# jac99/Egonn

Measured on AMD Instinct MI355X. Metric: LiDAR scans/sec (descriptor extraction), 50k-pt clouds @ 0.1m voxel, higher is better.
Workload: dtype f32

## Files before the change

egonn_amd/_lib.py:

```python
from __future__ import annotations

import ctypes as C
import os
from typing import List, Optional, Sequence

import numpy as np
import torch

_HERE = os.path.dirname(os.path.abspath(__file__))
LIB_PATH = os.path.join(_HERE, "lib", "libegonn_hip.so")

QUANT_CARTESIAN, QUANT_POLAR = 0, 1
FLAG_DISABLE_GLOBAL, FLAG_DISABLE_LOCAL, FLAG_IGNORE_KP_REGRESSOR, FLAG_BF16 = 1, 2, 4, 8
FLAG_POOL_SPOC, FLAG_POOL_MAC = 16, 32
MINKFPN_SPLIT_TOPDOWN = 1
MINKFPN_BLOCKS = {'BasicBlock': 0, 'ECABasicBlock': 1}
MINKFPN_POOLING = {None: 0, 'GeM': 1, 'MAC': 2, 'SPoC': 3}

_P = C.c_void_p
_SIGS = [
    ("egonn_ctx_create", C.c_int, [C.POINTER(_P), C.c_int, C.c_int]),
    ("egonn_ctx_destroy", None, [_P]),
    ("egonn_last_error", C.c_char_p, []),
    ("egonn_debug_set_naive_conv", C.c_int, [_P, C.c_int]),
    ("egonn_debug_set_ksplit", C.c_int, [_P, C.c_int, C.c_int, C.c_int, C.c_int, C.c_int]),
    ("egonn_debug_set_resident", C.c_int, [_P, C.c_int, C.c_int]),
    ("egonn_debug_keep_level_features", C.c_int, [_P, C.c_int]),
    ("egonn_debug_set_trace", C.c_int, [_P]),
    ("egonn_prepare_maps", C.c_int, [_P, C.c_int, _P]),
    ("egonn_debug_rowgroup_tables", C.c_int, [_P, C.c_int, C.c_int, _P, _P, C.c_int64, C.POINTER(C.c_int64), _P]),
    ("egonn_debug_rowgroup_perm", C.c_int, [_P, C.c_int, C.c_int, _P, C.c_int64, C.POINTER(C.c_int64), _P]),
    ("egonn_debug_radix_sort_scratch_bytes", C.c_int64, [C.c_int64, C.c_int]),
    ("egonn_debug_radix_sort", C.c_int, [_P, _P, _P, _P, C.c_int64, C.c_int, _P, _P, C.c_int, C.c_int, C.c_int,
                                         C.POINTER(C.c_int32), _P, C.c_int64, _P]),
    ("egonn_debug_dense_group3", C.c_int, [_P, _P, _P, _P, _P, _P, _P]),
    ("egonn_debug_global_tail_scratch_bytes", C.c_int64, [C.c_int64]),
    ("egonn_debug_global_tail", C.c_int, [_P, _P, C.c_int, C.c_int64, _P, _P, _P, _P, _P, _P, C.c_int, C.c_int, _P, _P, _P, C.c_int64, _P]),
    ("egonn_voxelize", C.c_int, [_P, _P, C.POINTER(C.c_int64), C.c_int, C.c_int, C.POINTER(C.c_float), _P]),
    ("egonn_ctx_reserve", C.c_int, [_P, C.c_int64, C.c_int, C.POINTER(C.c_int64)]),
    ("egonn_voxelize_device", C.c_int, [_P, _P, C.c_int64, _P, C.c_int, C.c_int, C.POINTER(C.c_float), _P]),
    ("egonn_plan_status", C.c_int, [_P, _P]),
    ("egonn_ctx_set_exact_fp32", C.c_int, [_P, C.c_int]),
    ("egonn_ctx_set_operand_autoscale", C.c_int, [_P, C.c_int]),
    ("egonn_level_capacity", C.c_int, [_P, C.c_int, C.POINTER(C.c_int64)]),
    ("egonn_graph_begin", C.c_int, [_P]),
    ("egonn_graph_end", C.c_int, [_P, C.POINTER(_P)]),
    ("egonn_graph_launch", C.c_int, [_P, _P]),
    ("egonn_graph_destroy", None, [_P]),
    ("egonn_coords_set", C.c_int, [_P, _P, C.c_int64, C.c_int, _P]),
    ("egonn_level_count", C.c_int, [_P, C.c_int, C.POINTER(C.c_int64)]),
    ("egonn_level_batch_offsets", C.c_int, [_P, C.c_int, C.POINTER(C.c_int64)]),
    ("egonn_level_coords", C.c_int, [_P, C.c_int, _P, _P]),
    ("egonn_input_index", C.c_int, [_P, _P, _P]),
    ("egonn_conv", C.c_int, [_P, C.c_int, C.c_int, C.c_int, _P, C.c_int, _P, C.c_int, _P, _P, C.c_int, _P, _P]),
    ("egonn_conv_transpose", C.c_int, [_P, C.c_int, _P, C.c_int, _P, C.c_int, _P, _P]),
    ("egonn_sparse_conv", C.c_int, [_P, C.c_int, C.c_int, _P, C.c_int, _P, C.c_int, C.c_int, _P, _P, C.c_int, _P, _P, _P]),
    ("egonn_map_groups", C.c_int, [_P, C.c_int, C.c_int, C.POINTER(C.c_int64), C.POINTER(C.c_int64), _P]),
    ("egonn_global_avg_pool", C.c_int, [_P, C.c_int, _P, C.c_int, _P, _P]),
    ("egonn_bn_fold", C.c_int, [_P, _P, _P, _P, C.c_float, C.c_int, _P, _P, _P]),
    ("egonn_block_tail", C.c_int, [_P, C.c_int, _P, _P, C.c_int, _P, C.c_int, _P, _P]),
    ("egonn_gem", C.c_int, [_P, C.c_int, _P, C.c_int, _P, _P, _P]),
    ("egonn_global_max_pool", C.c_int, [_P, C.c_int, _P, C.c_int, _P, _P]),
    ("egonn_netvlad", C.c_int, [_P, C.c_int, _P, C.c_int, _P, _P, _P, _P, _P, _P, _P, _P, _P, _P, C.c_int, C.c_int, _P, _P]),
    ("egonn_netvlad_train_forward", C.c_int, [_P, C.c_int, _P, C.c_int, C.c_int, _P, _P, _P, _P, C.c_float, C.c_float, _P, _P,
                                              _P, C.c_int, _P, _P, _P, _P, _P, _P, _P]),
    ("egonn_netvlad_train_backward", C.c_int, [_P, C.c_int, _P, C.c_int, C.c_int, _P, _P, _P, _P, C.c_int, _P, _P, _P, _P, _P,
                                               _P, _P, _P, _P, _P, _P, _P]),
    ("egonn_global_max_pool_argmax", C.c_int, [_P, C.c_int, _P, C.c_int, _P, _P, _P]),
    ("egonn_global_max_pool_backward", C.c_int, [_P, C.c_int, _P, _P, C.c_int, _P, _P]),
    ("egonn_sigmoid_gate", C.c_int, [_P, _P, _P, C.c_int64, _P, _P, _P, _P]),
    ("egonn_add", C.c_int, [_P, _P, C.c_int64, _P, _P]),
    ("egonn_gather_input", C.c_int, [_P, _P, C.c_int, _P, _P]),
    ("egonn_model_create", C.c_int, [C.POINTER(_P)]),
    ("egonn_model_destroy", None, [_P]),
    ("egonn_model_set_tensor", C.c_int, [_P, C.c_char_p, _P, C.c_int, C.POINTER(C.c_int64)]),
    ("egonn_model_finalize", C.c_int, [_P, _P]),
    ("egonn_forward", C.c_int, [_P, _P, _P, C.c_int, C.POINTER(C.c_float), C.c_int, _P, _P, _P, _P, _P]),
    ("egonn_forward_level_features", C.c_int, [_P, C.c_int, _P, C.c_int, _P]),
    ("egonn_minkfpn_finalize", C.c_int, [_P, C.c_int, C.POINTER(C.c_int), C.POINTER(C.c_int), C.c_int, C.c_int, C.c_int, C.c_int, _P]),
    ("egonn_minkfpn_out_level", C.c_int, [C.c_int, C.c_int, C.POINTER(C.c_int)]),
    ("egonn_minkfpn_forward", C.c_int, [_P, _P, C.c_int, _P, _P, _P]),
    ("egonn_topdown_step", C.c_int, [_P, C.c_int, _P, _P, _P, _P, C.c_int, C.c_int, _P, _P]),
    ("egonn_select_keypoints", C.c_int, [_P, _P, _P, _P, C.c_int, _P, _P, _P, _P, _P]),
    ("egonn_topk_rows", C.c_int, [_P, _P, C.c_int, C.c_int, _P, _P, _P]),
    ("egonn_triplet_loss_scratch_floats", C.c_int64, [C.c_int]),
    ("egonn_triplet_loss", C.c_int, [_P, C.c_int, C.c_int, _P, _P, C.c_float, _P, _P, _P, _P, _P]),
    ("egonn_nn_search", C.c_int, [_P, C.c_int64, _P, _P, C.c_int64, _P, _P, _P]),
    ("egonn_matrix_min", C.c_int, [_P, C.c_int64, C.c_int64, _P, _P, _P, _P, _P]),
    ("egonn_softmax_cross_entropy", C.c_int, [_P, C.c_int64, C.c_int64, _P, _P, _P, _P, _P]),
    ("egonn_local_loss_scratch_bytes", C.c_int64, [C.c_int, C.c_int64, C.c_int64, C.c_int]),
    ("egonn_local_loss", C.c_int, [C.c_int, C.c_int64, C.c_int64, C.c_int64, C.c_int64, C.c_int] + [_P] * 13 +
                                  [C.POINTER(C.c_float)] + [_P] * 9 + [C.c_int64, _P]),
    ("egonn_dense", C.c_int, [_P, C.c_int64, C.c_int, _P, C.c_int, _P, C.c_int, C.c_int, _P, _P]),
    ("egonn_dense_pack_fragments", C.c_int, [_P, C.c_int, C.c_int, C.c_int, _P, _P]),
    ("egonn_dense_pack_fragments_host", C.c_int, [_P, C.c_int, C.c_int, C.c_int, _P]),
    ("egonn_debug_dense", C.c_int, [_P, C.c_int, C.c_int64, _P, C.c_int, C.c_int, _P, C.c_int, _P, _P, _P, _P, C.c_int, _P, C.c_int,
                                    _P, _P, C.c_int, _P, C.c_int, C.c_int, _P]),
    ("egonn_debug_dense_route", C.c_int, [C.c_int64, C.c_int, C.c_int, C.c_int, C.c_int, C.POINTER(C.c_int32)]),
    ("egonn_debug_sconv_choice", C.c_int, [C.POINTER(C.c_int32), C.c_int64, C.POINTER(C.c_int32)]),
    ("egonn_dense_backward_weight", C.c_int, [_P, C.c_int, _P, C.c_int, C.c_int64, _P, _P, C.c_int64, _P]),
    ("egonn_conv_backward_weight", C.c_int, [_P, C.c_int, C.c_int, C.c_int, C.c_int, _P, C.c_int, _P, C.c_int, _P, _P,
                                             C.c_int64, _P]),
    ("egonn_col_stats", C.c_int, [C.c_int, _P, _P, _P, _P, C.c_int64, C.c_int, _P, _P, C.c_int64, _P]),
    ("egonn_bn_train_finalize", C.c_int, [_P, _P, C.c_double, C.c_int, _P, _P, C.c_float, C.c_float, _P, _P, _P, _P]),
    ("egonn_bn_backward_finalize", C.c_int, [_P, _P, C.c_double, C.c_int, _P, _P, _P, _P, _P]),
    ("egonn_affine_act", C.c_int, [_P, _P, _P, C.c_int64, C.c_int, C.c_int, _P, _P]),
    ("egonn_affine3", C.c_int, [_P, _P, _P, _P, _P, _P, C.c_int64, C.c_int, _P, _P]),
    ("egonn_relu_backward", C.c_int, [_P, _P, C.c_int64, C.c_int, _P, _P]),
    ("egonn_contrastive_loss_scratch_floats", C.c_int64, [C.c_int]),
    ("egonn_contrastive_loss", C.c_int, [_P, C.c_int, C.c_int, _P, _P, C.c_float, C.c_float, _P, _P, _P, _P, _P]),
    ("egonn_se_gate", C.c_int, [_P, _P, _P, _P, _P, C.c_int, C.c_int, C.c_int, _P, _P, _P]),
    ("egonn_se_gate_backward", C.c_int, [_P, _P, _P, _P, _P, _P, C.c_int, C.c_int, C.c_int, _P, _P, _P, _P, _P, _P]),
    ("egonn_eca_gate", C.c_int, [_P, _P, C.c_int, C.c_int, C.c_int, _P, _P]),
    ("egonn_eca_gate_backward", C.c_int, [_P, _P, _P, _P, C.c_int, C.c_int, C.c_int, _P, _P, _P]),
    ("egonn_act_backward", C.c_int, [C.c_int, _P, _P, C.c_int64, C.c_int, _P, _P]),
    ("egonn_l2_normalize", C.c_int, [_P, _P, C.c_int64, C.c_int, _P, _P]),
    ("egonn_gate_residual", C.c_int, [_P, C.c_int, _P, _P, _P, C.c_int, C.c_int, _P, _P]),
    ("egonn_gate_residual_backward", C.c_int, [_P, C.c_int, _P, _P, _P, C.c_int, _P, _P, _P]),
    ("egonn_segment_sums", C.c_int, [_P, C.c_int, C.c_int, _P, _P, _P, _P, C.c_int, _P, _P, C.c_int64, _P]),
    ("egonn_segment_broadcast", C.c_int, [_P, C.c_int, _P, C.c_int, C.c_int, _P, _P]),
    ("egonn_gem_backward", C.c_int, [_P, C.c_int, _P, _P, _P, C.c_int, _P, _P]),
    ("egonn_filter_points_scratch_ints", C.c_int64, [C.c_int64]),
    ("egonn_filter_points", C.c_int, [_P, C.c_int64, C.c_int, _P, C.c_int, C.c_int, C.c_int, C.c_float, _P, _P, _P,
                                      C.c_int64, _P]),
    ("egonn_knn", C.c_int, [_P, C.c_int64, _P, C.c_int64, C.c_int, C.c_int, _P, _P, _P, C.c_int64, _P]),
    ("egonn_recall_counts", C.c_int, [_P, _P, _P, C.c_int64, C.c_int, C.c_int, _P, C.c_int, _P, _P]),
    ("egonn_registration_scratch_bytes", C.c_int64, [C.c_int, C.c_int, C.c_int]),
    ("egonn_match_mutual_scratch_bytes", C.c_int64, [C.c_int, C.c_int]),
    ("egonn_match_mutual", C.c_int, [_P, _P, _P, _P, C.c_int, C.c_int, C.c_int, _P, _P, _P, C.c_int64, _P]),
    ("egonn_ransac_pairs", C.c_int, [_P, _P, _P, _P, _P, _P, _P, C.c_int, C.c_int, C.c_int, C.c_uint64, C.c_double, _P,
                                     C.c_int64, _P, _P, _P]),
    ("egonn_registration_finish", C.c_int, [_P, _P, _P, _P, _P, _P, _P, C.c_int, C.c_int, C.c_int, C.c_uint64, C.c_double, _P,
                                            C.c_int64, _P, C.c_double, _P, _P, _P, _P, _P, _P, _P, _P, _P, _P, _P, _P]),
    ("egonn_voxel_downsample_scratch_bytes", C.c_int64, [C.c_int64, C.c_int]),
    ("egonn_voxel_downsample", C.c_int, [_P, C.c_int64, _P, C.c_int, C.c_double, C.POINTER(C.c_float), _P, _P, _P, _P, _P,
                                         C.c_int64, _P]),
    ("egonn_icp_scratch_bytes", C.c_int64, [C.c_int64, C.c_int64, C.c_int]),
    ("egonn_icp_pairs", C.c_int, [_P, C.c_int64, _P, _P, C.c_int64, _P, C.c_int, _P, C.c_double, C.c_int, C.c_double, C.c_double,
                                  _P, _P, _P, _P, _P, _P, _P, _P, _P, C.c_int64, _P]),
    ("egonn_estimate_normals_scratch_bytes", C.c_int64, [C.c_int64, C.c_int]),
    ("egonn_estimate_normals", C.c_int, [_P, C.c_int64, _P, C.c_int, C.c_int, _P, _P, _P, _P, _P, C.c_int64, _P]),
    ("egonn_icp_plane_scratch_bytes", C.c_int64, [C.c_int64, C.c_int64, C.c_int]),
    ("egonn_icp_plane_pairs", C.c_int, [_P, C.c_int64, _P, _P, C.c_int64, _P, _P, C.c_int, _P, C.c_double, C.c_int, C.c_double,
                                        C.c_double, _P, _P, _P, _P, _P, _P, _P, _P, _P, C.c_int64, _P]),
    ("egonn_augment_scratch_bytes", C.c_int64, [C.c_int64, C.c_int]),
    ("egonn_augment_points", C.c_int, [_P, C.c_int64, _P, C.c_int, _P, _P, _P, _P, _P, _P, _P, _P, _P, C.c_int64, _P]),
    ("egonn_scan_context", C.c_int, [_P, C.c_int64, _P, C.c_int, C.c_int, C.c_int, C.c_double, C.c_double, _P, _P, _P]),
    ("egonn_scan_context_ringkey", C.c_int, [_P, C.c_int64, C.c_int, C.c_int, _P, _P]),
    ("egonn_scan_context_distance", C.c_int, [_P, C.c_int64, _P, C.c_int64, C.c_int, C.c_int, _P, C.c_int, _P, _P, _P]),
    ("egonn_scan_context_rerank", C.c_int, [_P, _P, _P, C.c_int64, C.c_int, _P, _P, _P, _P]),
    ("egonn_radius_count", C.c_int, [_P, C.c_int64, _P, C.c_int64, C.POINTER(C.c_double), C.c_int, C.c_int, _P, _P]),
    ("egonn_radius_fill", C.c_int, [_P, C.c_int64, _P, C.c_int64, C.c_double, C.c_int, _P, _P, C.c_int64, _P, _P]),
    ("egonn_pair_masks", C.c_int, [_P, C.c_int, _P, _P, C.c_int64, _P, _P, C.c_int64, C.c_int64, _P, _P, _P, _P]),
    ("egonn_relative_poses", C.c_int, [_P, C.c_int64, _P, _P, C.c_int64, C.c_int, _P, _P, _P]),
    ("egonn_gather_clouds", C.c_int, [_P, C.c_int64, _P, C.c_int64, _P, C.c_int, _P, C.c_int64, _P, _P, _P]),
    ("egonn_match_candidates_scratch_bytes", C.c_int64, [C.c_int, C.c_int, C.c_int]),
    ("egonn_match_candidates", C.c_int, [_P, _P, _P, _P, _P, C.c_int, C.c_int, C.c_int, C.c_int, C.c_int, _P, _P, _P, _P,
                                         C.c_int64, _P]),
    ("egonn_gather_candidates", C.c_int, [_P, _P, _P, _P, _P, _P, C.c_int, C.c_int, C.c_int, C.c_int, _P, _P, _P, _P, _P, _P]),
    ("egonn_pick_candidates", C.c_int, [_P, C.c_int, C.c_int, C.c_int, _P, _P, _P, _P, _P, _P, _P, _P, C.c_int] + [_P] * 12),
    ("egonn_profile_enable", C.c_int, [_P, C.c_int, C.c_char_p]),
    ("egonn_profile_fetch", C.c_int, [_P, C.c_int, C.POINTER(C.c_int), C.c_char_p, C.POINTER(C.c_float),
                                      C.POINTER(C.c_double), C.POINTER(C.c_double), _P]),
]
EXPORTED_SYMBOLS = [s[0] for s in _SIGS]

_lib = None


def load() -> C.CDLL:
    global _lib
    if _lib is not None:
        return _lib
    if not os.path.exists(LIB_PATH):
        raise RuntimeError(
            f"egonn_amd: HIP library not found at {LIB_PATH}. Build it with "
            f"`python -c 'import __graft_entry__ as g; g.build()'` (hipcc --offload-arch=gfx950). "
            f"There is no CPU fallback.")
    lib = C.CDLL(LIB_PATH)
    for name, res, args in _SIGS:
        fn = getattr(lib, name)
        fn.restype = res
        fn.argtypes = args
    _lib = lib
    return lib


def _err(lib) -> str:
    msg = lib.egonn_last_error()
    return msg.decode() if msg else "unknown error"


class EgonnError(RuntimeError):

    def __init__(self, msg: str, code: int):
        super().__init__(msg)
        self.code = int(code)


class CapacityError(EgonnError):
    """status 5: the batch did not fit the capacities of egonn_ctx_reserve (the exact-size eager path still works)"""


class Fp16RangeError(EgonnError):
    """status 6: a kernel on the fp16-split pipe (fp32 sparse convolution or local heads) met an operand fp16 cannot hold
    (|x| >= 65520) or a non-finite input: the batch's outputs are invalid; Context.set_exact_fp32(True) and run it again
    (on the same plan: every forward clears this flag)"""


def check(rc: int):
    if rc != 0:
        cls = CapacityError if rc == 5 else (Fp16RangeError if rc == 6 else EgonnError)
        raise cls(f"libegonn_hip: {_err(load())} (code {rc})", rc)


def _stream() -> int:
    return torch.cuda.current_stream().cuda_stream


def _ptr(t: Optional[torch.Tensor]) -> Optional[int]:
    return None if t is None else t.data_ptr()


def call(device: torch.device, fn, *args):
    idx = device.index
    if idx is None or torch.cuda.current_device() == idx:
        rc = fn(*args, _stream())
    else:
        with torch.cuda.device(device):
            rc = fn(*args, _stream())
    if rc != 0:
        check(rc)


def _dev_f32(t: torch.Tensor, device) -> torch.Tensor:
    return t.to(device=device, dtype=torch.float32).contiguous()


def as_dev(x, dev, dtype) -> torch.Tensor:
    return torch.as_tensor(x).to(device=dev, dtype=dtype).contiguous()


def scratch(nbytes: int, dev) -> torch.Tensor:
    return torch.empty((max(int(nbytes), 8) + 7) // 8, dtype=torch.int64, device=dev)


def check_cloud(name, x):
    shape = tuple(getattr(x, "shape", ()))
    if len(shape) != 2 or shape[1] != 3:
        raise ValueError(f"{name}: expected (n, 3) points, got shape {shape}")


def check_offsets(name, off) -> int:
    shape = tuple(getattr(off, "shape", (len(off),) if hasattr(off, "__len__") else ()))
    if len(shape) != 1 or shape[0] < 2:
        raise ValueError(f"{name}: offsets must be a 1-D sequence of n_clouds + 1 entries, got shape {shape}")
    return shape[0] - 1


def concat_clouds(clouds, dev):
    ts = [torch.as_tensor(c) for c in clouds]
    for c in ts:
        check_cloud("cloud", c)
    off = [0]
    for c in ts:
        off.append(off[-1] + c.shape[0])
    pts = torch.cat([c.to(device=dev, dtype=torch.float32) for c in ts]) if ts else torch.zeros((0, 3), device=dev)
    return pts, torch.tensor(off, dtype=torch.int64, device=dev)


def dense_pack_fragments(weight, out_in: bool):
    lib = load()
    co, ci = (weight.shape if out_in else weight.shape[::-1])
    if isinstance(weight, np.ndarray):
        w = np.ascontiguousarray(weight, dtype=np.float32)
        out = np.empty(ci * co, dtype=np.float32)
        check(lib.egonn_dense_pack_fragments_host(w.ctypes.data, int(bool(out_in)), int(ci), int(co), out.ctypes.data))
        return out
    w = weight.contiguous()
    out = torch.empty(ci * co, dtype=torch.float32, device=w.device)
    call(w.device, lib.egonn_dense_pack_fragments, w.data_ptr(), int(bool(out_in)), int(ci), int(co), out.data_ptr())
    return out


def debug_dense(x, weight, out_in: bool, out, form: int, n_dev=None, packed=None, bias=None, scale=None, shift=None, act: int = 0,
                residual=None, gate=None, boff=None):
    lib = load()
    cap, cin = x.shape
    cout = out.shape[1]
    B = 0 if boff is None else boff.numel() - 1
    bf = lambda t: int(t is not None and t.dtype == torch.bfloat16)
    call(x.device, lib.egonn_debug_dense, x.data_ptr(), bf(x), int(cap), _ptr(n_dev), int(cin), int(cout), weight.data_ptr(),
         int(bool(out_in)), _ptr(packed), _ptr(bias), _ptr(scale), _ptr(shift), int(act), _ptr(residual), bf(residual), _ptr(gate),
         _ptr(boff), B, out.data_ptr(), bf(out), int(form))
    return out


CONV_PRODUCT, CONV_PLAIN, CONV_RING, CONV_COOP, CONV_RING2, CONV_DMA, CONV_DMA3, CONV_TRACED = 0, 1, 2, 4, 8, 16, 32, 128
CONV_SPLIT = 1000
CFG_NW4, CFG_NW8, CFG_RESIDENT = 142, 182, 183
CFG_PARTS, CFG_TRACED = 400, 9000
SCONV_ROUTES = ("plain", "split", "tail_split", "wg", "dma", "rg")
SCONV_CHOICE_FIELDS = ("route", "kernel", "NW", "NSW", "KW", "KS", "GATED", "TRACE", "resident", "KSP", "D", "G", "SPLIT", "PIPE",
                       "gx", "gy", "gz", "block", "lds", "kparts")


def debug_sconv_choice(kind: int, level: int, cin: int, cout: int, cap_groups: int, *, code: int = 0, bf16: int = 0, gated: int = 0,
                       split_io: int = 0, residual: int = 0, split_max_level: int = 5, autoscale: int = 0, resident_mask: int = -1,
                       max_workgroups: int = 0, kparts: int = -1, kw: int = -1, col_parts: int = -1) -> dict:
    arg = (C.c_int32 * 16)(int(code), kind, level, cin, cout, int(bf16), int(gated), split_io, int(residual), split_max_level,
                           int(autoscale), resident_mask, max_workgroups, kparts, kw, col_parts)
    out = (C.c_int32 * 20)()
    check(load().egonn_debug_sconv_choice(arg, int(cap_groups), out))
    d = dict(zip(SCONV_CHOICE_FIELDS, out))
    d["route"], d["kernel"] = SCONV_ROUTES[d["route"]], SCONV_ROUTES[d["kernel"]]
    return d


DENSE_ROUTES = ("none", "stream", "lds", "small", "tile", "plain")


def debug_dense_route(rows: int, cin: int, cout: int, form: int = -1, gate_scans: int = 0):
    out = (C.c_int32 * 5)()
    check(load().egonn_debug_dense_route(int(rows), int(cin), int(cout), int(form), int(gate_scans), out))
    return (DENSE_ROUTES[out[0]],) + tuple(out[1:])


def debug_radix_sort(keys_in, vals_in, keys_out, vals_out, n: int, nbits: int, n_dev=None, seg_offsets=None, idx_bits: int = 0,
                     either_pair: bool = False, scratch_buf=None, scratch_bytes: Optional[int] = None) -> int:
    lib = load()
    B = 0 if seg_offsets is None else seg_offsets.numel() - 1
    need = lib.egonn_debug_radix_sort_scratch_bytes(int(n), B)
    if scratch_buf is None:
        scratch_buf = scratch(need, keys_in.device)
    pair = C.c_int32(-1)
    call(keys_in.device, lib.egonn_debug_radix_sort, keys_in.data_ptr(), vals_in.data_ptr(), keys_out.data_ptr(),
         vals_out.data_ptr(), int(n), int(nbits), _ptr(n_dev), _ptr(seg_offsets), B, int(idx_bits), int(bool(either_pair)),
         C.byref(pair), scratch_buf.data_ptr(), need if scratch_bytes is None else int(scratch_bytes))
    return pair.value


def debug_dense_group3(xs, capacities, counts, ws, packed: bool):
    lib = load()
    dev = xs[0].device
    arr = lambda ptrs: (C.c_void_p * 3)(*ptrs)
    nds = [torch.tensor([int(c)], dtype=torch.int32, device=dev) for c in counts]
    pks = [dense_pack_fragments(w, False) for w in ws] if packed else [None] * 3
    bufs = [torch.full((max(int(c), 1), 128), -12345.0, dtype=torch.float32, device=dev) for c in capacities]
    call(dev, lib.egonn_debug_dense_group3, arr([x.data_ptr() for x in xs]), (C.c_int64 * 3)(*[int(c) for c in capacities]),
         arr([n.data_ptr() for n in nds]), arr([w.data_ptr() for w in ws]), arr([_ptr(p) for p in pks]),
         arr([b.data_ptr() for b in bufs]))
    return [b[:int(c)] for b, c in zip(bufs, capacities)]


GLOBAL_TAIL_POOLING = {"GeM": 1, "MAC": 2, "SPoC": 3}


def debug_global_tail(g5, row_offsets, n_dev, w0, b0, w1, b1, p, pooling: str, form: int):
    lib = load()
    B = row_offsets.numel() - 1
    cap = g5.shape[0]
    need = lib.egonn_debug_global_tail_scratch_bytes(int(cap))
    buf = scratch(need, g5.device)
    partial = torch.empty((B, 32, 256), dtype=torch.float32, device=g5.device)
    out = torch.empty((B, 256), dtype=torch.float32, device=g5.device)
    call(g5.device, lib.egonn_debug_global_tail, g5.data_ptr(), row_offsets.data_ptr(), B, int(cap), n_dev.data_ptr(), w0.data_ptr(),
         b0.data_ptr(), w1.data_ptr(), b1.data_ptr(), _ptr(p), GLOBAL_TAIL_POOLING[pooling], int(form), partial.data_ptr(),
         out.data_ptr(), buf.data_ptr(), need)
    return partial, out


def require_gpu() -> torch.device:
    if not torch.cuda.is_available():
        raise RuntimeError("egonn_amd: no HIP device visible (torch.cuda.is_available() is False); "
                           "the descriptor-extraction path runs on MI355X only — there is no CPU fallback.")
    return torch.device("cuda", torch.cuda.current_device())


class Context:

    def __init__(self, device: Optional[torch.device] = None, coord_bits: int = 16):
        self.lib = load()
        self.device = torch.device(device) if device is not None else require_gpu()
        if self.device.type != "cuda":
            raise RuntimeError(f"egonn_amd: device {self.device} is not a HIP device; there is no CPU fallback.")
        if self.device.index is None:
            self.device = torch.device("cuda", torch.cuda.current_device())
        h = _P()
        check(self.lib.egonn_ctx_create(C.byref(h), self.device.index, coord_bits))
        self.h = h
        self.batch_size = 0
        self._keep = []

    def __del__(self):
        try:
            if getattr(self, "h", None):
                self.lib.egonn_ctx_destroy(self.h)
                self.h = None
        except Exception:
            pass

    def voxelize(self, points: torch.Tensor, scan_offsets: Sequence[int], mode: int, step: Sequence[float]):
        assert points.is_cuda and points.dtype == torch.float32 and points.is_contiguous()
        assert points.dim() == 2 and points.shape[1] == 3
        B = len(scan_offsets) - 1
        off = (C.c_int64 * (B + 1))(*[int(o) for o in scan_offsets])
        st = (C.c_float * 3)(*([float(s) for s in step] + [0.0, 0.0])[:3])
        self._call(self.lib.egonn_voxelize, self.h, points.data_ptr(), off, B, mode, st)
        self.batch_size = B

    def reserve(self, max_points: int, batch_size: int, level_capacity: Optional[Sequence[int]] = None):
        caps = None
        if level_capacity is not None:
            assert len(level_capacity) == 8
            caps = (C.c_int64 * 8)(*[int(v) for v in level_capacity])
        with torch.cuda.device(self.device):
            check(self.lib.egonn_ctx_reserve(self.h, int(max_points), int(batch_size), caps))
        self.batch_size = int(batch_size)

    def voxelize_device(self, points: torch.Tensor, scan_offsets: torch.Tensor, batch_size: int, mode: int,
                        step: Sequence[float]):
        assert points.is_cuda and points.dtype == torch.float32 and points.is_contiguous() and points.shape[1] == 3
        assert scan_offsets.is_cuda and scan_offsets.dtype == torch.int64 and scan_offsets.numel() == batch_size + 1
        st = (C.c_float * 3)(*([float(s) for s in step] + [0.0, 0.0])[:3])
        self._call(self.lib.egonn_voxelize_device, self.h, points.data_ptr(), points.shape[0], scan_offsets.data_ptr(),
                   int(batch_size), mode, st)
        self.batch_size = int(batch_size)

    def plan_status(self):
        self._call(self.lib.egonn_plan_status, self.h)

    def level_capacity(self, level: int) -> int:
        n = C.c_int64()
        check(self.lib.egonn_level_capacity(self.h, level, C.byref(n)))
        return n.value

    def coords_set(self, coords: torch.Tensor, batch_size: int):
        assert coords.is_cuda and coords.dtype == torch.int32 and coords.is_contiguous()
        assert coords.dim() == 2 and coords.shape[1] == 4
        self._call(self.lib.egonn_coords_set, self.h, coords.data_ptr(), coords.shape[0], int(batch_size))
        self.batch_size = int(batch_size)

    def level_count(self, level: int) -> int:
        n = C.c_int64()
        check(self.lib.egonn_level_count(self.h, level, C.byref(n)))
        return n.value

    def level_batch_offsets(self, level: int) -> List[int]:
        off = (C.c_int64 * (self.batch_size + 1))()
        check(self.lib.egonn_level_batch_offsets(self.h, level, off))
        return list(off)

    def level_coords(self, level: int) -> torch.Tensor:
        out = torch.empty((self.level_count(level), 4), dtype=torch.int32, device=self.device)
        self._call(self.lib.egonn_level_coords, self.h, level, out.data_ptr())
        return out

    def input_index(self) -> torch.Tensor:
        out = torch.empty((self.level_count(0),), dtype=torch.int64, device=self.device)
        self._call(self.lib.egonn_input_index, self.h, out.data_ptr())
        return out

    def conv(self, level_in: int, level_out: int, kernel_size: int, x: torch.Tensor, kernel: torch.Tensor,
             scale: Optional[torch.Tensor] = None, shift: Optional[torch.Tensor] = None, relu: bool = False):
        kernel = _dev_f32(kernel, self.device)
        cin, cout = kernel.shape[-2], kernel.shape[-1]
        if x is None:
            assert kernel_size == 5 and cin == 1, "x=None (all-ones features) is the k=5 input layer only"
        else:
            x = _dev_f32(x, self.device)
            assert x.shape == (self.level_count(level_in), cin), (x.shape, self.level_count(level_in), cin)
        out = torch.empty((self.level_count(level_out), cout), dtype=torch.float32, device=self.device)
        sc = None if scale is None else _dev_f32(scale, self.device)
        sh = None if shift is None else _dev_f32(shift, self.device)
        self._call(self.lib.egonn_conv, self.h, level_in, level_out, kernel_size, _ptr(x), cin, kernel.data_ptr(), cout,
                   _ptr(sc), _ptr(sh), int(relu), out.data_ptr())
        return out

    def conv_transpose(self, level_in: int, x: torch.Tensor, kernel: torch.Tensor):
        x = _dev_f32(x, self.device)
        kernel = _dev_f32(kernel, self.device)
        cin, cout = kernel.shape[-2], kernel.shape[-1]
        assert x.shape == (self.level_count(level_in), cin)
        out = torch.empty((self.level_count(level_in - 1), cout), dtype=torch.float32, device=self.device)
        self._call(self.lib.egonn_conv_transpose, self.h, level_in, x.data_ptr(), cin, kernel.data_ptr(), cout, out.data_ptr())
        return out

    def sparse_conv(self, map_kind: int, level_out: int, x: torch.Tensor, kernel: torch.Tensor, scale=None, shift=None,
                    relu: bool = False, group_sums: bool = False):
        assert x.is_cuda and x.dtype in (torch.float32, torch.bfloat16) and x.is_contiguous()
        kernel = _dev_f32(kernel, self.device)
        cin, cout = kernel.shape[-2], kernel.shape[-1]
        assert x.shape[1] == cin
        out = torch.empty((self.level_count(level_out), cout), dtype=x.dtype, device=self.device)
        sc = None if scale is None else _dev_f32(scale, self.device)
        sh = None if shift is None else _dev_f32(shift, self.device)
        sums = None
        if group_sums:
            sums = torch.zeros((self.map_groups(map_kind, level_out)[0], cout), dtype=torch.float32, device=self.device)
        self._call(self.lib.egonn_sparse_conv, self.h, map_kind, level_out, x.data_ptr(), cin, kernel.data_ptr(), cout,
                   int(x.dtype == torch.bfloat16), _ptr(sc), _ptr(sh), int(relu), out.data_ptr(), _ptr(sums))
        return (out, sums) if group_sums else out

    def prepare_maps(self, with_level0_transpose: bool = False):
        self._call(self.lib.egonn_prepare_maps, self.h, int(with_level0_transpose))

    def map_groups(self, map_kind: int, level_out: int):
        n = C.c_int64()
        first = (C.c_int64 * (self.batch_size + 1))()
        self._call(self.lib.egonn_map_groups, self.h, map_kind, level_out, C.byref(n), first)
        return n.value, list(first)

    def rowgroup_tables(self, map_kind: int, level_out: int, with_rows: bool = True):
        ng, _ = self.map_groups(map_kind, level_out)
        K = 27 if map_kind == 0 else 8
        gm = torch.empty(ng, dtype=torch.int32, device=self.device)
        sn = torch.empty((ng, K, 16), dtype=torch.int32, device=self.device) if with_rows else None
        n = C.c_int64()
        self._call(self.lib.egonn_debug_rowgroup_tables, self.h, map_kind, level_out, gm.data_ptr(),
                   sn.data_ptr() if with_rows else None, ng, C.byref(n))
        return gm, sn

    def rowgroup_perm(self, map_kind: int, level_out: int):
        ng, _ = self.map_groups(map_kind, level_out)
        pm = torch.empty((ng, 16), dtype=torch.int32, device=self.device)
        n = C.c_int64()
        self._call(self.lib.egonn_debug_rowgroup_perm, self.h, map_kind, level_out, pm.data_ptr(), ng, C.byref(n))
        return pm

    def set_naive_conv(self, on):
        check(self.lib.egonn_debug_set_naive_conv(self.h, int(on)))

    def keep_level_features(self, on: bool):
        check(self.lib.egonn_debug_keep_level_features(self.h, int(bool(on))))

    def set_exact_fp32(self, on: bool):
        check(self.lib.egonn_ctx_set_exact_fp32(self.h, int(bool(on))))

    def set_operand_autoscale(self, on: bool):
        check(self.lib.egonn_ctx_set_operand_autoscale(self.h, int(bool(on))))

    def set_ksplit(self, map_class: int, level: int, kparts: int = -1, kw: int = -1, col_parts: int = -1):
        check(self.lib.egonn_debug_set_ksplit(self.h, int(map_class), int(level), int(kparts), int(kw), int(col_parts)))

    def set_resident(self, mask: int = -1, max_workgroups: int = 0):
        check(self.lib.egonn_debug_set_resident(self.h, int(mask), int(max_workgroups)))

    def global_avg_pool(self, level: int, x: torch.Tensor):
        x = _dev_f32(x, self.device)
        out = torch.empty((self.batch_size, x.shape[1]), dtype=torch.float32, device=self.device)
        self._call(self.lib.egonn_global_avg_pool, self.h, level, x.data_ptr(), x.shape[1], out.data_ptr())
        return out

    def bn_fold(self, bn: torch.nn.BatchNorm1d):
        c = bn.num_features
        w, b, rm, rv = (_dev_f32(t.detach(), self.device) for t in (bn.weight, bn.bias, bn.running_mean, bn.running_var))
        scale = torch.empty(c, dtype=torch.float32, device=self.device)
        shift = torch.empty(c, dtype=torch.float32, device=self.device)
        self._call(self.lib.egonn_bn_fold, w.data_ptr(), b.data_ptr(), rm.data_ptr(), rv.data_ptr(), float(bn.eps), c,
                   scale.data_ptr(), shift.data_ptr())
        return scale, shift

    def block_tail(self, level: int, x: torch.Tensor, residual: torch.Tensor, eca_weight: Optional[torch.Tensor] = None):
        x, residual = _dev_f32(x, self.device), _dev_f32(residual, self.device)
        assert x.shape == residual.shape == (self.level_count(level), x.shape[1])
        out = torch.empty_like(x)
        ew = None if eca_weight is None else _dev_f32(eca_weight.detach().reshape(-1), self.device)
        self._call(self.lib.egonn_block_tail, self.h, level, x.data_ptr(), residual.data_ptr(), x.shape[1], _ptr(ew),
                   0 if ew is None else ew.numel(), out.data_ptr())
        return out

    def se_gate(self, mean: torch.Tensor, w1, b1, w2, b2, want_hidden: bool = False):
        mean = _dev_f32(mean, self.device)
        w1, b1, w2, b2 = (_dev_f32(t.detach(), self.device) for t in (w1, b1, w2, b2))
        B, c = mean.shape
        h = w1.shape[0]
        assert w1.shape == (h, c) and w2.shape == (c, h) and b1.shape == (h,) and b2.shape == (c,)
        gate = torch.empty_like(mean)
        hid = torch.empty((B, h), dtype=torch.float32, device=self.device) if want_hidden else None
        self._call(self.lib.egonn_se_gate, mean.data_ptr(), w1.data_ptr(), b1.data_ptr(), w2.data_ptr(), b2.data_ptr(), B, c, h,
                   gate.data_ptr(), _ptr(hid))
        return (gate, hid) if want_hidden else gate

    def add(self, a: torch.Tensor, b: torch.Tensor):
        a, b = _dev_f32(a, self.device), _dev_f32(b, self.device)
        assert a.shape == b.shape
        out = torch.empty_like(a)
        self._call(self.lib.egonn_add, a.data_ptr(), b.data_ptr(), a.numel(), out.data_ptr())
        return out

    def topdown_step(self, level_out: int, x_coarse: torch.Tensor, w_tconv: torch.Tensor, x_lateral: Optional[torch.Tensor] = None,
                     w_lateral: Optional[torch.Tensor] = None, rows: Optional[int] = None):
        x_coarse, w_tconv = _dev_f32(x_coarse, self.device), _dev_f32(w_tconv, self.device)
        c = w_tconv.shape[-1]
        cl = 0
        if x_lateral is not None:
            x_lateral, w_lateral = _dev_f32(x_lateral, self.device), _dev_f32(w_lateral, self.device)
            cl = w_lateral.shape[0]
        n = self.level_count(level_out) if rows is None else int(rows)
        out = torch.empty((n, c), dtype=torch.float32, device=self.device)
        self._call(self.lib.egonn_topdown_step, self.h, level_out, x_coarse.data_ptr(), w_tconv.data_ptr(), _ptr(x_lateral),
                   _ptr(w_lateral), c, cl, out.data_ptr())
        return out

    def gather_input(self, feats: torch.Tensor):
        feats = _dev_f32(feats, self.device)
        out = torch.empty((self.level_count(0), feats.shape[1]), dtype=torch.float32, device=self.device)
        self._call(self.lib.egonn_gather_input, self.h, feats.data_ptr(), feats.shape[1], out.data_ptr())
        return out

    def gem(self, level: int, x: torch.Tensor, p: torch.Tensor):
        x = _dev_f32(x, self.device)
        pp = _dev_f32(p.detach().reshape(-1), self.device)
        out = torch.empty((self.batch_size, x.shape[1]), dtype=torch.float32, device=self.device)
        self._call(self.lib.egonn_gem, self.h, level, x.data_ptr(), x.shape[1], pp.data_ptr(), out.data_ptr())
        return out

    def global_max_pool(self, level: int, x: torch.Tensor):
        x = _dev_f32(x, self.device)
        out = torch.empty((self.batch_size, x.shape[1]), dtype=torch.float32, device=self.device)
        self._call(self.lib.egonn_global_max_pool, self.h, level, x.data_ptr(), x.shape[1], out.data_ptr())
        return out

    def netvlad(self, level: int, x: torch.Tensor, cluster_weights: torch.Tensor, cluster_weights2: torch.Tensor,
                bn1: torch.nn.BatchNorm1d, hidden1_weights: torch.Tensor, bn2: torch.nn.BatchNorm1d,
                gating_weights: Optional[torch.Tensor] = None, gate_bn: Optional[torch.nn.BatchNorm1d] = None):
        x = _dev_f32(x, self.device)
        assert x.dim() == 2 and x.shape[0] >= self.level_count(level), "netvlad: x must hold every row of the level"
        w = [_dev_f32(t.detach(), self.device) for t in (cluster_weights, cluster_weights2, hidden1_weights)]
        d = w[2].shape[-1]
        sc1, sh1 = self.bn_fold(bn1)
        sc2, sh2 = self.bn_fold(bn2)
        gating = gating_weights is not None
        gw = scg = shg = None
        if gating:
            gw = _dev_f32(gating_weights.detach(), self.device)
            scg, shg = self.bn_fold(gate_bn)
        out = torch.empty((self.batch_size, d), dtype=torch.float32, device=self.device)
        self._call(self.lib.egonn_netvlad, self.h, level, x.data_ptr(), x.shape[1], w[0].data_ptr(), w[1].data_ptr(),
                   sc1.data_ptr(), sh1.data_ptr(), w[2].data_ptr(), sc2.data_ptr(), sh2.data_ptr(), _ptr(gw), _ptr(scg),
                   _ptr(shg), d, int(gating), out.data_ptr())
        return out

    def scratch(self, nfloats: int) -> torch.Tensor:
        buf = getattr(self, "_scratch", None)
        if buf is None or buf.numel() < nfloats:
            buf = torch.empty(max(int(nfloats), 1 << 24), dtype=torch.float32, device=self.device)
            self._scratch = buf
        return buf

    def _call(self, fn, *args):
        call(self.device, fn, *args)

    def dense(self, x, weight, out_in: bool, bias=None, act: int = 0):
        x, weight = _dev_f32(x, self.device), _dev_f32(weight, self.device)
        cin, cout = (weight.shape[1], weight.shape[0]) if out_in else (weight.shape[0], weight.shape[1])
        assert x.dim() == 2 and x.shape[1] == cin, (x.shape, weight.shape, out_in)
        b = None if bias is None else _dev_f32(bias, self.device)
        out = torch.empty((x.shape[0], cout), dtype=torch.float32, device=self.device)
        self._call(self.lib.egonn_dense, x.data_ptr(), x.shape[0], cin, weight.data_ptr(), int(out_in), _ptr(b), cout,
                   act, out.data_ptr())
        return out

    def netvlad_train_forward(self, level: int, x: torch.Tensor, nmax: int, cluster_weights, cluster_weights2,
                              bn1: torch.nn.BatchNorm1d, hidden1_weights):
        x = _dev_f32(x, self.device)
        n, c = x.shape
        assert n == self.level_count(level), "netvlad: x must hold exactly the rows of the level"
        B, d = self.batch_size, hidden1_weights.shape[-1]
        f = dict(dtype=torch.float32, device=self.device)
        out = torch.empty((B, d), **f)
        saved = (torch.empty((n, 64), **f), torch.empty((4, 64), **f), torch.empty((B, c, 64), **f),
                 torch.empty((B, c // 16, 64), **f), torch.empty((B, 64), **f))
        mom = bn1.momentum if bn1.momentum is not None else 1.0 / float(int(bn1.num_batches_tracked) + 1)
# ... 259 lines not shown
```

egonn_amd/csrc/common.h:

```cpp
#pragma once
#include <hip/hip_runtime.h>
#include <atomic>
#include <stdint.h>
#include <stdio.h>
#include <string.h>
#include <string>
#include <vector>

#define EGONN_MAX_LEVELS 10
#define EGONN_NUM_LEVELS 8
#define EGONN_MAX_BATCH 4096

#define API extern "C" __attribute__((visibility("default")))

namespace egonn {

void set_error(const char* fmt, ...);
#define EGONN_OK 0
#define EGONN_ERR_INVALID 1
#define EGONN_ERR_HIP 2
#define EGONN_ERR_RANGE 3
#define EGONN_ERR_STATE 4
#define EGONN_ERR_CAPACITY 5
#define EGONN_ERR_FP16_RANGE 6

#define HIP_CHECK(expr)                                                                   \
  do {                                                                                    \
    hipError_t _e = (expr);                                                               \
    if (_e != hipSuccess) {                                                               \
      ::egonn::set_error("%s:%d: %s failed: %s", __FILE__, __LINE__, #expr,               \
                         hipGetErrorString(_e));                                          \
      return EGONN_ERR_HIP;                                                               \
    }                                                                                     \
  } while (0)

#define EGONN_REQUIRE(cond, code, ...)                                                    \
  do {                                                                                    \
    if (!(cond)) {                                                                        \
      ::egonn::set_error(__VA_ARGS__);                                                    \
      return (code);                                                                      \
    }                                                                                     \
  } while (0)

#define EGONN_TRY(expr)                                                                   \
  do {                                                                                    \
    int _rc = (expr);                                                                     \
    if (_rc != EGONN_OK) return _rc;                                                      \
  } while (0)

static inline int64_t cdiv(int64_t a, int64_t b) { return (a + b - 1) / b; }
__host__ __device__ static inline int clipi(int v, int hi) { return v < 0 ? 0 : (v > hi ? hi : v); }
__host__ __device__ static inline int64_t clipi(int64_t v, int64_t hi) { return v < 0 ? 0 : (v > hi ? hi : v); }

struct AttrOnce {
  std::atomic<uint64_t> done{0};
  static int dev() { int d = 0; (void)hipGetDevice(&d); return d & 63; }
  bool need() const { return !((done.load(std::memory_order_acquire) >> dev()) & 1ull); }
  void mark() { done.fetch_or(1ull << dev(), std::memory_order_release); }
};
static inline size_t align_up(size_t v, size_t a) { return (v + a - 1) / a * a; }

struct Arena {
  char* base = nullptr;
  size_t cap = 0;
  size_t off = 0;
  bool borrowed = false;
  static Arena view(void* span, size_t bytes) {
    Arena a;
    a.base = static_cast<char*>(span);
    a.cap = bytes;
    a.borrowed = true;
    return a;
  }
  int ensure(size_t bytes) {
    if (bytes <= cap) return EGONN_OK;
    EGONN_REQUIRE(!borrowed, EGONN_ERR_INVALID, "scratch span of %zu bytes is %zu bytes short of the %zu needed", cap, bytes - cap,
                  bytes);
    size_t want = align_up(bytes + bytes / 4, size_t(1) << 20);
    if (base) {
      HIP_CHECK(hipDeviceSynchronize());
      HIP_CHECK(hipFree(base));
      base = nullptr;
      cap = 0;
    }
    HIP_CHECK(hipMalloc(reinterpret_cast<void**>(&base), want));
    cap = want;
    off = 0;
    return EGONN_OK;
  }
  void reset() { off = 0; }
  template <typename T>
  T* alloc(size_t n) {
    size_t o = align_up(off, 256);
    size_t end = o + n * sizeof(T);
    if (end > cap) return nullptr;
    off = end;
    return reinterpret_cast<T*>(base + o);
  }
  void release() {
    if (borrowed) return;
    if (base) (void)hipFree(base);
    base = nullptr;
    cap = off = 0;
  }
};

__host__ __device__ static inline uint64_t part1by2(uint32_t v) {
  uint64_t x = v & 0xFFFFull;
  x = (x | (x << 16)) & 0x0000FF0000FFull;
  x = (x | (x << 8)) & 0x00F00F00F00Full;
  x = (x | (x << 4)) & 0x0C30C30C30C3ull;
  x = (x | (x << 2)) & 0x249249249249ull;
  return x;
}
__host__ __device__ static inline uint32_t compact1by2(uint64_t x) {
  x &= 0x249249249249ull;
  x = (x | (x >> 2)) & 0x0C30C30C30C3ull;
  x = (x | (x >> 4)) & 0x00F00F00F00Full;
  x = (x | (x >> 8)) & 0x0000FF0000FFull;
  x = (x | (x >> 16)) & 0xFFFFull;
  return (uint32_t)x;
}
__host__ __device__ static inline uint64_t morton3(uint32_t x, uint32_t y, uint32_t z) {
  return part1by2(x) | (part1by2(y) << 1) | (part1by2(z) << 2);
}

static constexpr int RG_MAX_JOBS = 24;
static constexpr int RG_MAX_WIN = 512;
struct RowGroups {
  int K = 0;
  int win = 0;
  int cap_groups = 0;
  int32_t* perm = nullptr;
  int32_t* snbr = nullptr;
  uint32_t* gmask = nullptr;
  int32_t* meta = nullptr;
  int32_t* order4 = nullptr;
  bool built = false;
};
struct RGBuild {
  RowGroups* rg;
  const int32_t* nbr;
  const int32_t* n_dev;
  const int32_t* boff;
  int32_t cap_rows = 0;
};
int rowgroup_build(const RGBuild* jobs, int njobs, int B, hipStream_t stream);

struct Level {
  int64_t n = 0;
  uint64_t* keys = nullptr;
  int32_t* parent = nullptr;
  int32_t* cstart = nullptr;
  uint64_t* mask = nullptr;
  int32_t* bstart = nullptr;
  int32_t* boff = nullptr;
  int32_t* nbr27 = nullptr;
  int32_t* nbr8 = nullptr;
  int32_t* nbrT = nullptr;
  RowGroups rg27, rg8, rgT;
};

struct Plan {
  bool valid = false;
  bool built_reserved = false;
  bool exact = false;
  int64_t cap_points = 0;
  int64_t* scan_off = nullptr;
  int batch = 0;
  int coord_bits = 16;
  int64_t n_input = 0;
  Level lv[EGONN_MAX_LEVELS];
  int64_t cap[EGONN_MAX_LEVELS] = {};
  int32_t* perm0 = nullptr;
  int32_t* g0 = nullptr;
  uint64_t* t2m = nullptr;
  int32_t* t2s = nullptr;
  std::vector<int32_t> boff_host[EGONN_NUM_LEVELS];
};

enum ProfKind { PK_CONV0 = 0, PK_K3 = 1, PK_K2S2 = 2, PK_TCONV = 3, PK_OTHER = 4 };
struct ProfRec {
  char name[64];
  int kind, level, K, cin, cout;
  int es;
  hipEvent_t e0, e1;
};
struct Profiler {
  int mode = 0;
  char filter[64] = "";
  std::vector<ProfRec> recs;
  std::vector<ProfRec> graph_recs;
  std::vector<hipEvent_t> pool;
  hipEvent_t get();
};

struct Switches {
  bool debug_sync;
  bool no_presplit;
  bool no_fused_down;
  bool no_fused_lateral;
  bool no_gated_k2s2;
  bool no_fused_ghead;
  bool no_fused_gtail;
  bool no_packed_laterals;
  bool no_split_heads;
  bool no_tail_split;
  bool no_task_order;
  bool flat_sort, sort_pairs;
  bool no_search67;
  bool no_dense_stream;
  int split_max_level;
  int split_max_level_k8;
  int split_cfg;
  int rg_first_pass;
  const char* ksplit[5];
};
const Switches& switches();

struct KsRule {
  int8_t kparts[2][EGONN_NUM_LEVELS];
  int8_t kw[2][EGONN_NUM_LEVELS];
  int8_t col_parts[EGONN_NUM_LEVELS];
};

static constexpr int SCONV_RESIDENT_DEFAULT = 6;

enum SconvFamily {
  SCONV_AUTO = 0,
  SCONV_PLAIN,
  SCONV_RING,
  SCONV_RING2,
  SCONV_COOP,
  SCONV_DMA,
  SCONV_DMA3,
  SCONV_TRACED
};
struct SplitCfg {
  int code = 0;
  int nw = 0;
  int parts_sel = 0;
  bool trace = false;
  bool resident = false;
};
struct SconvSetting {
  SconvFamily family = SCONV_AUTO;
  bool split = false;
  SplitCfg cfg;
  bool product() const { return family == SCONV_AUTO && !split; }
};
struct SconvSettings {
  SconvSetting set;
  int split_max_level = 5;
  int operand_autoscale = 0;
  int resident_mask = SCONV_RESIDENT_DEFAULT;
  int resident_wgs = 0;
  KsRule ks_rule;
};

struct Ctx {
  Profiler prof;
  SconvSettings sconv;
  uint16_t* conv0_lut = nullptr;
  unsigned long long* dev_pairs = nullptr;
  int device = 0;
  int coord_bits = 16;
  float* ks_part = nullptr;
  size_t ks_part_floats = 0;
  const void* sort_prezeroed = nullptr;
  int keep_level_features = 0;
  Arena plan_arena;
  Arena work_arena;
  Arena sort_arena;
  Plan plan;
  int32_t* host_counts = nullptr;
  int32_t* dev_counts = nullptr;
  int32_t* dev_flags = nullptr;
  int32_t* dev_fp16_flag = nullptr;
  bool reserved = false;
  int64_t reserve_points = 0;
  int reserve_batch = 0;
  int64_t reserve_cap[EGONN_MAX_LEVELS] = {};
  hipEvent_t ev0 = nullptr, ev1 = nullptr;
};

hipEvent_t* prof_kernel_events();
struct ProfScope {
  Ctx* ctx;
  hipStream_t st;
  int idx = -1;
  bool exact = false;
  bool in_graph = false;
  ProfScope(Ctx* c, hipStream_t s, const char* name, int kind, int level, int K, int cin, int cout, int es);
  ~ProfScope();
};

int ensure_level0_parent_table(Ctx* ctx, hipStream_t stream);
int ensure_rowgroups(Ctx* ctx, const int* kinds, const int* levels, int count, hipStream_t stream);
int rowgroup_cap_groups(const Plan& P, int level);

static constexpr int KP_MAX_N = 256;
static constexpr int KP_MAX_D = 256;
static constexpr int KP_MAX_PAIRS = 1 << 20;
static constexpr int REL_MAX_K = 1024;
int reg_check_shape(const char* who, int P, int n_max);
int rel_check_shape(const char* who, int Q, int k, int M, int n_max);

int radix_sort_pairs(Arena& ws, uint64_t* keys_in, uint32_t* vals_in, uint64_t* keys_out, uint32_t* vals_out,
                     int64_t n, int nbits, hipStream_t stream, const int64_t* n_dev = nullptr, uint64_t** keys_res = nullptr,
                     uint32_t** vals_res = nullptr);
size_t radix_sort_scratch_bytes(int64_t n);
int radix_sort_segments(Arena& ws, uint64_t* keys_in, uint32_t* vals_in, uint64_t* keys_out, uint32_t* vals_out, int64_t n,
                        const int64_t* off_dev, int B, int nbits, hipStream_t stream, uint64_t** keys_res, uint32_t** vals_res,
                        int idx_bits = 0, const void* prezeroed = nullptr);
size_t radix_sort_segments_scratch_bytes(int64_t n, int B);
int radix_sort_segments_layout(Arena& ws, int64_t n, int B, int32_t** tilehist, int32_t** scanhist);
int radix_sort_segments_passes(int nbits);
int radix_sort_segments_digits();

int plan_from_points(Ctx* ctx, const float* points, const int64_t* scan_offsets, int64_t n_cap, int offsets_on_device,
                     int B, int mode, const float* step, hipStream_t stream);
int plan_reserve(Ctx* ctx, int64_t max_points, int B, const int64_t* level_caps);
int plan_sync(Ctx* ctx, hipStream_t stream);
int plan_from_coords(Ctx* ctx, const int32_t* coords, int64_t n, int B, hipStream_t stream);
int plan_level_coords(Ctx* ctx, int level, int32_t* out, hipStream_t stream);
int count_map_pairs(Ctx* ctx, hipStream_t stream);

}
```

egonn_amd/csrc/coords.hip:

```cpp
#include "common.h"

#include <algorithm>
#include <stdarg.h>

namespace egonn {

static thread_local char g_err[1024] = "";
void set_error(const char* fmt, ...) {
  va_list ap;
  va_start(ap, fmt);
  vsnprintf(g_err, sizeof(g_err), fmt, ap);
  va_end(ap);
}
const char* last_error() { return g_err; }

const Switches& switches() {
  static const Switches sw = [] {
    auto on = [](const char* name) { return getenv(name) != nullptr; };
    auto num = [](const char* name, int unset) { const char* e = getenv(name); return e ? atoi(e) : unset; };
    const char* ds = getenv("EGONN_DEBUG_SYNC");
    return Switches{.debug_sync = ds && ds[0] == '1', .no_presplit = on("EGONN_NO_PRESPLIT"), .no_fused_down = on("EGONN_NO_FUSED_DOWN"),
                    .no_fused_lateral = on("EGONN_NO_FUSED_LATERAL"), .no_gated_k2s2 = on("EGONN_NO_GATED_K2S2"),
                    .no_fused_ghead = on("EGONN_NO_FUSED_GHEAD"), .no_fused_gtail = on("EGONN_NO_FUSED_GTAIL"),
                    .no_packed_laterals = on("EGONN_NO_PACKED_LATERALS"), .no_split_heads = on("EGONN_NO_SPLIT_HEADS"),
                    .no_tail_split = on("EGONN_NO_TAIL_SPLIT"), .no_task_order = on("EGONN_NO_TASK_ORDER"),
                    .flat_sort = on("EGONN_FLAT_SORT"), .sort_pairs = on("EGONN_SORT_PAIRS"), .no_search67 = on("EGONN_NO_SEARCH67"),
                    .no_dense_stream = on("EGONN_NO_DENSE_STREAM"),
                    .split_max_level = num("EGONN_SPLIT_MAX_LEVEL", -1), .split_max_level_k8 = num("EGONN_SPLIT_MAX_LEVEL_K8", -1),
                    .split_cfg = num("EGONN_SPLIT_CFG", 0), .rg_first_pass = num("EGONN_RG_FIRST_PASS", 0),
                    .ksplit = {getenv("EGONN_KSPLIT"), getenv("EGONN_KSPLIT8"), getenv("EGONN_KSPLIT_KW"), getenv("EGONN_KSPLIT_KW8"),
                               getenv("EGONN_KSPLIT_PARTS")}};
  }();
  return sw;
}

hipEvent_t Profiler::get() {
  if (!pool.empty()) {
    hipEvent_t e = pool.back();
    pool.pop_back();
    return e;
  }
  hipEvent_t e = nullptr;
  (void)hipEventCreate(&e);
  return e;
}
ProfScope::ProfScope(Ctx* c, hipStream_t s, const char* name, int kind, int level, int K, int cin, int cout, int es)
    : ctx(c), st(s) {
  if (!c || c->prof.mode == 0) return;
  if (c->prof.mode >= 2 && !strstr(name, c->prof.filter)) return;
  hipStreamCaptureStatus cs = hipStreamCaptureStatusNone;
  (void)hipStreamIsCapturing(s, &cs);
  in_graph = cs == hipStreamCaptureStatusActive;
  if (in_graph && c->prof.mode != 3) return;
  ProfRec r;
  snprintf(r.name, sizeof(r.name), "%s", name);
  r.kind = kind; r.level = level; r.K = K; r.cin = cin; r.cout = cout; r.es = es;
  r.e0 = c->prof.get();
  r.e1 = c->prof.get();
  exact = c->prof.mode == 2 && (kind == PK_K3 || kind == PK_K2S2 || kind == PK_TCONV);
  if (exact) {
    prof_kernel_events()[0] = r.e0;
    prof_kernel_events()[1] = r.e1;
  } else {
    (void)hipEventRecord(r.e0, s);
  }
  std::vector<ProfRec>& dst = in_graph ? c->prof.graph_recs : c->prof.recs;
  idx = (int)dst.size();
  dst.push_back(r);
}
ProfScope::~ProfScope() {
  if (idx < 0) return;
  if (exact) {
    prof_kernel_events()[0] = prof_kernel_events()[1] = nullptr;
  } else {
    (void)hipEventRecord((in_graph ? ctx->prof.graph_recs : ctx->prof.recs)[idx].e1, st);
  }
}
hipEvent_t* prof_kernel_events() {
  static thread_local hipEvent_t ev[2] = {nullptr, nullptr};
  return ev;
}

struct QuantParams {
  int mode;
  float s0, s1, s2;
};

__device__ static inline void quantize_point(const QuantParams& qp, float x, float y, float z, int32_t& cx,
                                             int32_t& cy, int32_t& cz) {
  if (qp.mode == 0) {
    cx = (int32_t)floorf(qp.s0 == 1.0f ? x : __fdiv_rn(x, qp.s0));
    cy = (int32_t)floorf(qp.s0 == 1.0f ? y : __fdiv_rn(y, qp.s0));
    cz = (int32_t)floorf(qp.s0 == 1.0f ? z : __fdiv_rn(z, qp.s0));
  } else {
    const float at = (float)atan2((double)y, (double)x);
    const float theta = __fadd_rn(180.0f, __fdiv_rn(__fmul_rn(at, 180.0f), 3.14159265358979323846f));
    const float dist = sqrtf(__fadd_rn(__fmul_rn(x, x), __fmul_rn(y, y)));
    cx = (int32_t)floorf(__fdiv_rn(theta, qp.s0));
    cy = (int32_t)floorf(__fdiv_rn(dist, qp.s1));
    cz = (int32_t)floorf(__fdiv_rn(z, qp.s2));
  }
}

__device__ static inline bool encode_key(int32_t b, int32_t cx, int32_t cy, int32_t cz, int cb, uint64_t& key) {
  const int32_t bias = 1 << (cb - 1);
  const int32_t lim = 1 << cb;
  const int32_t ux = cx + bias, uy = cy + bias, uz = cz + bias;
  const bool ok = (ux >= 0) & (ux < lim) & (uy >= 0) & (uy < lim) & (uz >= 0) & (uz < lim) & (b >= 0);
  key = ((uint64_t)(uint32_t)b << (3 * cb)) | morton3((uint32_t)ux, (uint32_t)uy, (uint32_t)uz);
  return ok;
}

__global__ void points_to_keys_kernel(const float* __restrict__ pts, int64_t n_cap, const int64_t* __restrict__ scan_off,
                                      int B, QuantParams qp, int cb, uint64_t* __restrict__ keys,
                                      uint32_t* __restrict__ vals, int32_t* __restrict__ flags, int idx_bits,
                                      int64_t* __restrict__ off_copy, int32_t* __restrict__ zero_ptr, int zero_words) {
  const int64_t i = (int64_t)blockIdx.x * blockDim.x + threadIdx.x;
  const int64_t stride = (int64_t)gridDim.x * blockDim.x;
  if (off_copy)
    for (int64_t b = i; b <= B; b += stride) off_copy[b] = scan_off[b];
  for (int64_t w = i; w < zero_words; w += stride) zero_ptr[w] = 0;
  const int64_t nn = scan_off[B];
  if (i == 0 && nn > n_cap) atomicOr(flags, 2);
  for (int64_t b = i; b <= B; b += stride)
    if ((b == 0 && scan_off[0] != 0) || (b > 0 && scan_off[b] < scan_off[b - 1])) atomicOr(flags, 1);
  if (i >= (nn < n_cap ? nn : n_cap)) return;
  int lo = 0, hi = B;
  while (hi - lo > 1) {
    const int mid = (lo + hi) >> 1;
    if (scan_off[mid] <= i) lo = mid; else hi = mid;
  }
  const float x = pts[3 * i + 0], y = pts[3 * i + 1], z = pts[3 * i + 2];
  int32_t cx, cy, cz;
  quantize_point(qp, x, y, z, cx, cy, cz);
  uint64_t key;
  const bool finite = isfinite(x) & isfinite(y) & isfinite(z);
  if (!encode_key(lo, cx, cy, cz, cb, key) || !finite) {
    atomicOr(flags, 1);
    const int32_t hi = (1 << (cb - 1)) - 1, lo_c = -(1 << (cb - 1));
    const int32_t qx = finite ? min(max(cx, lo_c), hi) : 0, qy = finite ? min(max(cy, lo_c), hi) : 0,
                  qz = finite ? min(max(cz, lo_c), hi) : 0;
    encode_key(lo, qx, qy, qz, cb, key);
  }
  if (idx_bits > 0) {
    keys[i] = ((key & ((1ull << (3 * cb)) - 1)) << idx_bits) | (uint64_t)(i - scan_off[lo]);
  } else {
    keys[i] = key;
    vals[i] = (uint32_t)i;
  }
}

__global__ void coords_to_keys_kernel(const int32_t* __restrict__ c4, int64_t n, int cb, int Bmax,
                                      uint64_t* __restrict__ keys, uint32_t* __restrict__ vals,
                                      int32_t* __restrict__ flags) {
  const int64_t i = (int64_t)blockIdx.x * blockDim.x + threadIdx.x;
  if (i >= n) return;
  const int4 c = reinterpret_cast<const int4*>(c4)[i];
  uint64_t key;
  if (!encode_key(c.x, c.y, c.z, c.w, cb, key) || c.x >= Bmax) {
    atomicOr(flags, 1);
    key = ~0ull >> 1;
  }
  keys[i] = key;
  vals[i] = (uint32_t)i;
}

static constexpr int PYR_BLOCK = 256;
static constexpr int PYR_ROUNDS = 4;
static constexpr int PYR_TILE = PYR_BLOCK * PYR_ROUNDS;
static constexpr int NL = EGONN_MAX_LEVELS;

__device__ static inline int head_levels(const uint64_t* __restrict__ keys, int64_t i) {
  if (i == 0) return NL;
  const uint64_t d = keys[i] ^ keys[i - 1];
  if (d == 0) return 0;
  const int t = (63 - __clzll(d)) / 3;
  return (t >= NL - 1) ? NL : t + 1;
}

__device__ static inline int64_t clip_count(int64_t cap, const int64_t* __restrict__ n_dev) {
  if (!n_dev) return cap;
  const int64_t v = *n_dev;
  return v < cap ? v : cap;
}
__global__ __launch_bounds__(PYR_BLOCK) void pyramid_count_kernel(const uint64_t* __restrict__ keys, int64_t n_cap,
                                                                  const int64_t* __restrict__ n_dev,
                                                                  int32_t* __restrict__ tilecnt) {
  __shared__ int32_t cnt[PYR_BLOCK / 64][NL];
  const int64_t n = clip_count(n_cap, n_dev);
  const int tid = threadIdx.x, lane = tid & 63, wave = tid >> 6;
  const int64_t wbase = (int64_t)blockIdx.x * PYR_TILE + (int64_t)wave * 64 * PYR_ROUNDS;
  int32_t c[NL];
#pragma unroll
  for (int l = 0; l < NL; ++l) c[l] = 0;
  for (int r = 0; r < PYR_ROUNDS; ++r) {
    const int64_t i = wbase + r * 64 + lane;
    const int h = (i < n) ? head_levels(keys, i) : 0;
#pragma unroll
    for (int l = 0; l < NL; ++l) c[l] += __popcll(__ballot(h > l));
  }
  if (lane == 0) {
#pragma unroll
    for (int l = 0; l < NL; ++l) cnt[wave][l] = c[l];
  }
  __syncthreads();
  if (tid < NL) {
    int32_t s = 0;
    for (int w = 0; w < PYR_BLOCK / 64; ++w) s += cnt[w][tid];
    tilecnt[(int64_t)blockIdx.x * NL + tid] = s;
  }
}

struct PyramidOut {
  uint64_t* keys[NL];
  int32_t* parent[NL];
  int32_t* cstart[NL];
  int32_t* boff[EGONN_NUM_LEVELS];
  int32_t* perm0;
  int32_t* counts;
  int32_t* flags;
  int32_t cap[NL];
};

__global__ __launch_bounds__(PYR_BLOCK) void pyramid_apply_kernel(const uint64_t* __restrict__ keys,
                                                                  const uint32_t* __restrict__ vals, int64_t n_cap,
                                                                  const int64_t* __restrict__ n_dev,
                                                                  const int32_t* __restrict__ tilecnt, int ntiles,
                                                                  int cb, int B, PyramidOut out) {
  __shared__ int32_t red[PYR_BLOCK / 64][NL];
  const int64_t n = clip_count(n_cap, n_dev);
  __shared__ int32_t tilebase[NL];
  __shared__ int32_t wavecnt[PYR_BLOCK / 64][NL];
  const int tid = threadIdx.x, lane = tid & 63, wave = tid >> 6;
  const int tile = blockIdx.x;

  {
    int32_t p[NL];
#pragma unroll
    for (int l = 0; l < NL; ++l) p[l] = 0;
    for (int t = tid; t < tile; t += PYR_BLOCK) {
#pragma unroll
      for (int l = 0; l < NL; ++l) p[l] += tilecnt[(int64_t)t * NL + l];
    }
#pragma unroll
    for (int l = 0; l < NL; ++l) {
      int32_t v = p[l];
#pragma unroll
      for (int o = 32; o > 0; o >>= 1) v += __shfl_down(v, o, 64);
      if (lane == 0) red[wave][l] = v;
    }
    __syncthreads();
    if (tid < NL) {
      int32_t s = 0;
      for (int w = 0; w < PYR_BLOCK / 64; ++w) s += red[w][tid];
      tilebase[tid] = s;
    }
  }

  const int64_t wbase = (int64_t)tile * PYR_TILE + (int64_t)wave * 64 * PYR_ROUNDS;
  int hreg[PYR_ROUNDS];
  int32_t wc[NL];
#pragma unroll
  for (int l = 0; l < NL; ++l) wc[l] = 0;
#pragma unroll
  for (int r = 0; r < PYR_ROUNDS; ++r) {
    const int64_t i = wbase + r * 64 + lane;
    hreg[r] = (i < n) ? head_levels(keys, i) : 0;
#pragma unroll
    for (int l = 0; l < NL; ++l) wc[l] += __popcll(__ballot(hreg[r] > l));
  }
  if (lane == 0) {
#pragma unroll
    for (int l = 0; l < NL; ++l) wavecnt[wave][l] = wc[l];
  }
  __syncthreads();
  int32_t run[NL];
#pragma unroll
  for (int l = 0; l < NL; ++l) {
    int32_t s = tilebase[l];
    for (int w = 0; w < wave; ++w) s += wavecnt[w][l];
    run[l] = s;
  }

  const uint64_t lt = (lane == 0) ? 0ull : (~0ull >> (64 - lane));
  const int bshift = 3 * cb;
#pragma unroll
  for (int r = 0; r < PYR_ROUNDS; ++r) {
    const int64_t i = wbase + r * 64 + lane;
    const int h = hreg[r];
    const uint64_t key = (i < n) ? keys[i] : 0ull;
    int32_t excl[NL];
#pragma unroll
    for (int l = 0; l < NL; ++l) {
      const uint64_t m = __ballot(h > l);
      excl[l] = run[l] + __popcll(m & lt);
      run[l] += __popcll(m);
    }
    if (i < n && h > 0) {
      if (excl[0] < out.cap[0]) out.perm0[excl[0]] = (int32_t)vals[i];
#pragma unroll
      for (int l = 0; l < NL; ++l) {
        if (l < h && excl[l] < out.cap[l]) {
          out.keys[l][excl[l]] = key >> (3 * l);
          if (l >= 1) out.cstart[l][excl[l]] = min(excl[l - 1], out.cap[l - 1]);
          if (l + 1 < NL) {
            const int32_t g = (l + 1 < h) ? excl[l + 1] : excl[l + 1] - 1;
            out.parent[l][excl[l]] = min(g, out.cap[l + 1] - 1);
          }
        }
      }
      const int32_t b = (int32_t)(key >> bshift);
      const int32_t bprev = (i == 0) ? -1 : (int32_t)(keys[i - 1] >> bshift);
      if (b != bprev) {
        for (int32_t bb = bprev + 1; bb <= b && bb <= B; ++bb) {
#pragma unroll
          for (int l = 0; l < EGONN_NUM_LEVELS; ++l) out.boff[l][bb] = min(excl[l], out.cap[l]);
        }
      }
    }
    if (i == n - 1) {
      const int32_t blast = (int32_t)(key >> bshift);
#pragma unroll
      for (int l = 0; l < NL; ++l) {
        const int32_t total = excl[l] + (h > l ? 1 : 0);
        out.counts[l] = total;
        if (total > out.cap[l]) atomicOr(out.flags, 2);
        if (l >= 1) {
          const int32_t below = excl[l - 1] + (h > l - 1 ? 1 : 0);
          out.cstart[l][min(total, out.cap[l])] = min(below, out.cap[l - 1]);
        }
        if (l < EGONN_NUM_LEVELS) {
          for (int32_t bb = blast + 1; bb <= B; ++bb) out.boff[l][bb] = min(total, out.cap[l]);
// ... 747 lines not shown
```

egonn_amd/csrc/global_tail.hip:

```cpp
#include "common.h"
#include "kernels.h"
#include "rowmath.h"

namespace egonn {

constexpr int GT_KS0 = GTAIL_CIN / 16, GT_KS1 = GTAIL_MID / 16;
constexpr int GT_NT0 = GTAIL_MID / 16 / 4, GT_NT1 = GTAIL_OUT / 16 / 4;
constexpr int GT_HS = GTAIL_MID + 4, GT_OS = GTAIL_OUT + 4;

__global__ __launch_bounds__(256, 2) void global_tail_kernel(const float* __restrict__ g5, int64_t ncap, const int32_t* __restrict__ boff,
                                                             const f32x4* __restrict__ wf0, const float* __restrict__ b0,
                                                             const f32x4* __restrict__ wf1, const float* __restrict__ b1, int pow_mode,
                                                             const float* __restrict__ pexp, float* __restrict__ partial) {
  __shared__ __attribute__((aligned(16))) float s_hid[16 * GT_HS];
  __shared__ __attribute__((aligned(16))) float s_out[16 * GT_OS];
  const int b = blockIdx.y, ch = blockIdx.x;
  const int32_t s = boff[b], e = boff[b + 1];
  const int64_t len = e - s;
  const int32_t r0 = s + (int32_t)(len * ch / SEG_CHUNKS);
  const int32_t r1 = ncap > 0 ? s + (int32_t)(len * (ch + 1) / SEG_CHUNKS) : r0;
  const int tid = threadIdx.x, lane = tid & 63, wave = tid >> 6;
  const int l15 = lane & 15, g4 = lane >> 4;
  const float p = pow_mode == 1 ? pexp[0] : 1.f;
  float run = pow_mode == 2 ? -INFINITY : 0.f;
#pragma unroll 1
  for (int32_t base = r0; base < r1; base += 16) {
    int zero = 0;
    asm volatile("" : "+s"(zero));
    const f32x4* const w0p = wf0 + (int64_t)wave * GT_NT0 * GT_KS0 * 64 + lane + zero;
    const f32x4* const w1p = wf1 + (int64_t)wave * GT_NT1 * GT_KS1 * 64 + lane + zero;
    const int64_t row = max(min((int64_t)min(base + l15, r1 - 1), ncap - 1), (int64_t)0);
    f32x4 a[GT_KS0], w0[GT_NT0][GT_KS0], w1[2][GT_KS1];
    float bh[GT_NT0];
#pragma unroll
    for (int t = 0; t < GT_KS0; ++t) a[t] = *reinterpret_cast<const f32x4*>(g5 + row * GTAIL_CIN + 16 * t + 4 * g4);
#pragma unroll
    for (int j = 0; j < GT_NT0; ++j) {
#pragma unroll
      for (int t = 0; t < GT_KS0; ++t) w0[j][t] = w0p[(j * GT_KS0 + t) * 64];
      bh[j] = b0[16 * (wave * GT_NT0 + j) + l15];
    }
#pragma unroll
    for (int t = 0; t < GT_KS1; ++t) w1[0][t] = w1p[t * 64];
    __builtin_amdgcn_sched_barrier(0);
#pragma unroll
    for (int j = 0; j < GT_NT0; ++j) {
      f32x4 acc = {0.f, 0.f, 0.f, 0.f};
#pragma unroll
      for (int t = 0; t < GT_KS0; ++t) {
#pragma unroll
        for (int u = 0; u < 4; ++u) acc = __builtin_amdgcn_mfma_f32_16x16x4f32(a[t][u], w0[j][t][u], acc, 0, 0, 0);
      }
#pragma unroll
      for (int r = 0; r < 4; ++r) s_hid[(4 * g4 + r) * GT_HS + 16 * (wave * GT_NT0 + j) + l15] = fmaxf(acc[r] + bh[j], 0.f);
      __builtin_amdgcn_sched_barrier(0);
    }
    __syncthreads();
    f32x4 h[GT_KS1];
#pragma unroll
    for (int t = 0; t < GT_KS1; ++t) h[t] = *reinterpret_cast<const f32x4*>(s_hid + l15 * GT_HS + 16 * t + 4 * g4);
    __builtin_amdgcn_sched_barrier(0);
#pragma unroll
    for (int j = 0; j < GT_NT1; ++j) {
      const int c0 = 16 * (wave * GT_NT1 + j) + 4 * g4;
      const f32x4 bo = *reinterpret_cast<const f32x4*>(b1 + c0);
      if (j + 1 < GT_NT1) {
#pragma unroll
        for (int t = 0; t < GT_KS1; ++t) w1[(j + 1) & 1][t] = w1p[((j + 1) * GT_KS1 + t) * 64];
      }
      f32x4 acc = {0.f, 0.f, 0.f, 0.f};
#pragma unroll
      for (int t = 0; t < GT_KS1; ++t) {
#pragma unroll
        for (int u = 0; u < 4; ++u) acc = __builtin_amdgcn_mfma_f32_16x16x4f32(w1[j & 1][t][u], h[t][u], acc, 0, 0, 0);
      }
      f32x4 v = acc + bo;
      v = v * 1.f + 0.f;
      *reinterpret_cast<f32x4*>(s_out + l15 * GT_OS + c0) = v;
      __builtin_amdgcn_sched_barrier(0);
    }
    __syncthreads();
    const int nrows = min(16, r1 - base);
    for (int r = 0; r < nrows; ++r) {
      float v = s_out[r * GT_OS + tid];
      if (pow_mode == 1) v = powf(fmaxf(v, 1e-6f), p);
      run = pow_mode == 2 ? fmaxf(run, v) : run + v;
    }
  }
  float sum = pow_mode == 2 ? -INFINITY : 0.f;
  sum = pow_mode == 2 ? fmaxf(sum, run) : sum + run;
  partial[((int64_t)b * SEG_CHUNKS + ch) * GTAIL_OUT + tid] = sum;
}

int global_tail_fused(const float* g5, int64_t ncap, const int32_t* boff, int B, const float* wf0, const float* b0, const float* wf1,
                      const float* b1, int pow_mode, const float* p, float* partial, hipStream_t stream) {
  EGONN_REQUIRE(g5 && boff && wf0 && b0 && wf1 && b1 && partial && B >= 1 && ncap >= 0 && pow_mode >= 0 && pow_mode <= 2 &&
                    (pow_mode != 1 || p),
                EGONN_ERR_INVALID, "global tail: bad arguments");
  hipLaunchKernelGGL(global_tail_kernel, dim3(SEG_CHUNKS, B), dim3(256), 0, stream, g5, ncap, boff, reinterpret_cast<const f32x4*>(wf0),
                     b0, reinterpret_cast<const f32x4*>(wf1), b1, pow_mode, p, partial);
  HIP_CHECK(hipGetLastError());
  return EGONN_OK;
}

}
```

egonn_amd/csrc/kernels.h:

```cpp
#pragma once
#include "common.h"

namespace egonn {

const char* last_error();

bool sconv_rg_supported(int cin, int cout);
int pack_rg_weights(const float* W, int K, int cin, int cout, int bf16, int flip, int transpose, void* out,
                    hipStream_t stream);
extern unsigned long long* g_sconv_trace;
struct PackedKernel {
  const void* rg32 = nullptr;
  const void* rg16 = nullptr;
  const void* split = nullptr;
};
struct ConvCall {
  int kind = 0, level = 0;
  const void* in = nullptr; void* out = nullptr;
  int cin = 0, cout = 0, bf16 = 0;
  const float *scale = nullptr, *shift = nullptr;
  int relu = 0;
  float* psum = nullptr;
  const PackedKernel* packed = nullptr;
  const float* W = nullptr; float* scratch = nullptr; size_t scratch_floats = 0;
  int split_io = 0;
  const float *in2 = nullptr, *gate = nullptr;
  const float* residual = nullptr;
};
enum SconvRoute {
  ROUTE_PLAIN,
  ROUTE_SPLIT,
  ROUTE_TAIL_SPLIT,
  ROUTE_WG,
  ROUTE_DMA,
  ROUTE_RG
};
struct SconvLayer {
  int kind = 0, level = 0, cin = 0, cout = 0, bf16 = 0;
  bool gated = false;
  int split_io = 0;
  bool residual = false;
};
struct SconvChoice {
  SconvRoute route = ROUTE_RG;
  SconvRoute kernel = ROUTE_RG;
  int NW = 0, NSW = 0, KW = 0, KS = 0, GATED = 0, TRACE = 0, resident = 0;
  int KSP = 0, D = 0, G = 0, SPLIT = 0, PIPE = 0;
  unsigned gx = 0, gy = 1, gz = 1, block = 0;
  size_t lds = 0;
  int kparts = 1;
  int err = 0;
};
template <auto Kernel, class Args>
static int launch_sconv(const SconvChoice& ch, hipStream_t stream, const Args& a, hipEvent_t* stop_later = nullptr) {
  static AttrOnce attr_done;
  if (ch.lds > 48 * 1024 && attr_done.need()) {
    HIP_CHECK(hipFuncSetAttribute(reinterpret_cast<const void*>(Kernel), hipFuncAttributeMaxDynamicSharedMemorySize, 160 * 1024));
    attr_done.mark();
  }
  const dim3 grid(ch.gx, ch.gy, ch.gz), block(ch.block);
  hipEvent_t* pev = prof_kernel_events();
  if (pev[0]) {
    if (stop_later) *stop_later = pev[1];
    hipExtLaunchKernelGGL(Kernel, grid, block, ch.lds, stream, pev[0], stop_later ? nullptr : pev[1], 0, a);
    pev[0] = pev[1] = nullptr;
  } else {
    hipLaunchKernelGGL(Kernel, grid, block, ch.lds, stream, a);
  }
  HIP_CHECK(hipGetLastError());
  return EGONN_OK;
}
SconvChoice sconv_choose(const SconvSettings& s, const SconvLayer& l, int64_t cap_groups);
SconvSetting sconv_decode(int code);
SplitCfg sconv_decode_cfg(int cfg);
SconvRoute sconv_route(const Ctx* ctx, int kind, int level, int cin, int cout, int bf16);
bool sconv_split_arithmetic(const Ctx* ctx);
const char* sconv_kernel_name(const Ctx* ctx, int kind, int level, int cin, int cout, int bf16);
struct SconvLaunch {
  SconvChoice ch;
  const RowGroups* rg = nullptr;
  int64_t n_in_cap = 0;
  const void* Wp = nullptr;
  int32_t* flags = nullptr;
  int B = 0;
  float* part = nullptr; size_t part_floats = 0;
  uint32_t* in_absmax = nullptr; int64_t in_elems = 0;
};
int sconv_rg_forward(const ConvCall& c, const SconvLaunch& l, hipStream_t stream);
int sconv_map(Ctx* ctx, const ConvCall& c, hipStream_t stream);
bool sconv_split_supported(int cin, int cout);
int pack_split_weights(const float* W, int K, int cin, int cout, int flip, int transpose, void* out, hipStream_t stream);
size_t split_weights_bytes(int K, int cin, int cout);
int sconv_split_forward(const ConvCall& c, const SconvLaunch& l, hipStream_t stream);
size_t sconv_split_part_floats(const RowGroups& rg, int cout, int kparts);
struct KsChoice { int kparts, col_parts, kw; };
KsChoice sconv_ksplit_rule(const KsRule& rule, int kind, int level);
void sconv_ksplit_defaults(KsRule* r);
size_t sconv_ksplit_scratch_floats(const Ctx* ctx);
static constexpr size_t SCONV_SCRATCH_FLOATS = (size_t)2 << 20;
int sconv_naive(const float* in, const int32_t* nbr, const float* W, const float* scale, const float* shift, int relu,
                float* out, int64_t n_out, int K, int cin, int cout, hipStream_t stream);
int conv0_lut_init(Ctx* ctx);
int conv0_k5_forward(Ctx* ctx, const float* feat, const float* W, int cout, const float* scale,
                     const float* shift, int relu, void* out, int out_bf16, hipStream_t stream, const void* wpk = nullptr);
int conv0_pack_unit(const float* W, void* wpk, hipStream_t stream);

enum Act { ACT_NONE = 0, ACT_RELU = 1, ACT_TANH = 2, ACT_SOFTPLUS = 3, ACT_SIGMOID = 4 };
struct DenseCall {
  const void* in = nullptr; int in_bf16 = 0;
  int64_t n = 0;
  const int32_t* n_dev = nullptr;
  int cin = 0, cout = 0;
  const float* W = nullptr;
  int w_out_in = 0;
  const float* wfrag = nullptr;
  const float* bias = nullptr;
  const float *scale = nullptr, *shift = nullptr;
  int act = 0;
  const void* residual = nullptr; int res_bf16 = 0;
  const float* gate = nullptr;
  const int32_t* boff = nullptr;
  int B = 0;
  void* out = nullptr; int out_bf16 = 0;
  int form = -1;
};
enum DenseRoute {
  DENSE_INVALID = -1,
  DENSE_NONE = 0,
  DENSE_STREAM,
  DENSE_LDS,
  DENSE_SMALL,
  DENSE_TILE,
  DENSE_PLAIN
};
struct DenseLaunch {
  DenseRoute route = DENSE_NONE;
  unsigned gx = 0, gy = 0;
  size_t lds = 0;
  int colblk = 0;
};
DenseRoute dense_route(int64_t n, int cin, int cout, int form);
DenseLaunch dense_launch(int64_t n, int cin, int cout, int form, int gate_scans);
int dense_forward(const DenseCall& c, hipStream_t stream);
bool dense_gate_fusable(int64_t n, int cin, int cout);
bool dense_group3_rows(int64_t n);
int dense_small_group3(const float* const* in, const int64_t* n, const int32_t* const* n_dev, const float* const* W,
                       const float* const* wfrag, float* const* out, hipStream_t stream);
int dense_pack_frags(const float* W, int w_out_in, int cin, int cout, float* out, hipStream_t stream);

constexpr int GTAIL_CIN = 128, GTAIL_MID = 192, GTAIL_OUT = 256;
int global_tail_fused(const float* g5, int64_t ncap, const int32_t* boff, int B, const float* wf0, const float* b0, const float* wf1,
                      const float* b1, int pow_mode, const float* p, float* partial, hipStream_t stream);

int bn_fold(const float* w, const float* b, const float* rm, const float* rv, float eps, int c, float* scale,
            float* shift, hipStream_t stream);
int gather_rows(const float* in, const int32_t* perm, int64_t n, int c, float* out, hipStream_t stream,
                const int32_t* n_dev = nullptr);
static constexpr int SEG_CHUNKS = 32;
int segment_partial_sums(const float* in, const int32_t* boff, int B, int c, int pow_mode, const float* p,
                         float* partial, hipStream_t stream);
int eca_apply(const float* x, const float* res, const float* partial, const int32_t* boff, int B, int64_t n, int c,
              const float* wconv, int ksize, float* out, hipStream_t stream);
int eca_gate_groups(const float* psum, const RowGroups& rg, const int32_t* boff, int B, int c, const float* wconv, int ksize,
                    float* gate, hipStream_t stream);
int eca_apply_gate(const void* x, const void* res, const float* gate, const int32_t* boff, int B, int64_t n, int c,
                   void* out, int bf16, hipStream_t stream);
int convert_bf16_to_f32(const void* in, int64_t n, float* out, hipStream_t stream);
int gem_finish(const float* partial, const int32_t* boff, int B, int c, const float* p, float* out,
               hipStream_t stream);
int pool_finish(const float* partial, const int32_t* boff, int B, int c, int mode, float* out, hipStream_t stream);
int l2_normalize_rows(float* x, int64_t n, int c, hipStream_t stream, const int32_t* n_dev = nullptr);
int add_act(const float* a, const float* b, int64_t n, int relu, float* out, hipStream_t stream);

constexpr int LH_WAVES = 8;
int keypoint_positions(const uint64_t* keys, int64_t n, int level, int cb, const float* offsets, int mode,
                       const float* step, int ignore_offsets, float* out, hipStream_t stream, const int32_t* n_dev = nullptr);
int local_heads_forward(const float* x, int64_t n, const int32_t* n_dev, const float* const* w, const uint64_t* keys,
                        int level, int cb, int mode, const float* step, int ignore_offsets, float* out_desc, float* out_kp,
                        float* out_sigma, hipStream_t stream, const float* lateral_w = nullptr, const float* lateral_res = nullptr,
                        int in_bf16 = 0, const void* split_pack = nullptr, int32_t* flags = nullptr);
size_t local_heads_pack_bytes();
int local_heads_pack(const float* const* w6_dev, void* out, hipStream_t stream);
int select_topk(const float* sigma, const int32_t* boff_dev, int B, int k, const float* kp, const float* desc, int dc,
                int32_t* sel_rows , int32_t* sel_count , float* out_kp, float* out_desc, hipStream_t stream);

static constexpr int NV_K = 64;
static constexpr int NV_MAX_CHUNKS = 32;
static constexpr int NV_CHUNK_ROWS = 128;
__host__ __device__ static inline int nv_chunks(int32_t len) {
  if (len <= 0) return 0;
  const int n = (len + NV_CHUNK_ROWS - 1) / NV_CHUNK_ROWS;
  return n < NV_MAX_CHUNKS ? n : NV_MAX_CHUNKS;
}
size_t netvlad_workspace_floats(int B, int C, int D);
void netvlad_workspace_carve(float* ws, int B, int C, float** part, float** vraw, float** sq, float** pp);
int netvlad_forward(const float* x, const int32_t* boff, int B, int C, const float* wc, const float* w2, const float* sc1,
                    const float* sh1, const float* H, int D, const float* sc2, const float* sh2, const float* wg,
                    const float* scg, const float* shg, int gating, float* out, float* ws, hipStream_t stream);

constexpr int LL_CLOUD_CHUNK = 1024;
constexpr int LL_STATS = 16;

}
```

egonn_amd/csrc/model.h:

```cpp
#pragma once
#include <map>
#include <string>
#include <vector>

#include "../../include/egonn_hip.h"
#include "common.h"
#include "kernels.h"

struct egonn_ctx : public egonn::Ctx {
  hipStream_t plan_stream = nullptr;

  void* level_feat[EGONN_NUM_LEVELS] = {};
  int level_ch[EGONN_NUM_LEVELS] = {};
  int level_bf16 = 0;
  bool from_points = false;
};

#define REQUIRE_PLAN(c)                                                                               \
  EGONN_REQUIRE((c) && (c)->plan.valid, EGONN_ERR_STATE, "no coordinate plan (call egonn_voxelize / " \
                                                         "egonn_coords_set first)")
#define REQUIRE_LEVEL(c, level)                                                                              \
  REQUIRE_PLAN(c);                                                                                           \
  HIP_CHECK(hipSetDevice((c)->device));                                                                      \
  EGONN_REQUIRE((level) >= 0 && (level) < EGONN_NUM_LEVELS, EGONN_ERR_INVALID, "level %d out of range", (level))

#define DBG_SYNC(...)                                                 \
  do {                                                                \
    if (switches().debug_sync) {                                      \
      fprintf(stderr, "[egonn] " __VA_ARGS__);                        \
      fprintf(stderr, "\n");                                          \
      fflush(stderr);                                                 \
      HIP_CHECK(hipStreamSynchronize(st));                            \
    }                                                                 \
  } while (0)

#define WALLOC(T, var, count)                                                      \
  T* var = A->alloc<T>((size_t)(count));                                           \
  EGONN_REQUIRE(var != nullptr, EGONN_ERR_STATE, "work arena too small (" #var ")")

namespace egonn {

int claim_work(egonn_ctx* c, size_t bytes, bool with_ksplit, Arena** A);

struct TensorRef {
  const float* p = nullptr;
  std::vector<int64_t> shape;
};

struct BnRef {
  const float *w = nullptr, *b = nullptr, *rm = nullptr, *rv = nullptr;
  float *scale = nullptr, *shift = nullptr;
  int c = 0;
};

struct BlockRef {
  const float *conv1 = nullptr, *conv2 = nullptr, *down = nullptr, *eca = nullptr;
  BnRef n1, n2, dn;
  int cin = 0, cout = 0, eca_k = 0;
};

struct MlpRef {
  const float *w0 = nullptr, *b0 = nullptr, *w1 = nullptr, *b1 = nullptr;
  int cin = 0, mid = 0, cout = 0;
};

struct ModelStore {
  enum Form { RG32, RG16, SPLIT, DENSE, DENSE_OI };
  struct Pack { Form form; const float* w; int K, ci, co; size_t off; const void** dst; };
  std::vector<BnRef*> bns;
  std::vector<Pack> packs;
  size_t bn_bytes = 0, pack_bytes = 0;
  char *folded = nullptr, *packed = nullptr;
  size_t folded_cap = 0, packed_cap = 0;

  void begin();
  void add_bn(BnRef* bn);
  void add_pack(Form form, const float* w, int K, int ci, int co, const void** dst);
  void add_kernel(const float* w, int K, int ci, int co, bool bf16, PackedKernel* dst);
  int commit(hipStream_t st);
  void release();
};

struct MinkFpnModel;
void minkfpn_model_free(MinkFpnModel* f);
void minkfpn_model_invalidate(MinkFpnModel* f);

}

struct egonn_model {
  std::map<std::string, egonn::TensorRef> t;
  bool ready = false;
  egonn::ModelStore store;
  const float* conv0 = nullptr;
  egonn::BnRef bn[8];
  const float* convs[8] = {};
  egonn::BlockRef blk[8];
  const float *g1x1[8] = {}, *gt[8] = {}, *l1x1[8] = {}, *lt[8] = {};
  const float* gem_p = nullptr;
  egonn::MlpRef gdec, ldec, kp, sg;
  void* conv0_unit = nullptr;
  void* lh_pack = nullptr;
  const float** lh_ptrs = nullptr;
  egonn::PackedKernel pk_convs[8], pk_c1[8], pk_c2[8], pk_gt[8], pk_lt[8];
  const void *pk_down[8] = {}, *pk_l1x1[8] = {};
  const void *pk_g1x1[8] = {}, *pk_gdec[2] = {};
  egonn::MinkFpnModel* fpn = nullptr;
};

namespace egonn {

int get_tensor(egonn_model* m, const std::string& key, std::initializer_list<int64_t> want, const float** out);
int get_bn(egonn_model* m, const std::string& prefix, int c, BnRef* bn, ModelStore* store);
int get_block(egonn_model* m, const std::string& prefix, int ci, int co, bool eca, BlockRef* b, ModelStore* store);
int eca_ksize(int c);
int conv_layer(egonn_ctx* c, hipStream_t st, const ConvCall& cc, const char* what);
ConvCall conv_call(int kind, int level, const void* in, const PackedKernel& pk, int cin, int cout, int bf16, const BnRef* bn, int relu,
                   void* out);
int ensure_graph_rowgroups(egonn_ctx* c, int L, const int* tlevels, int nt, hipStream_t st);
int block_convs(egonn_ctx* c, hipStream_t st, Arena* A, int level, const BlockRef& b, const PackedKernel& pk1, const PackedKernel& pk2,
                int bf16, const void* in, float* psum, void** t2);
DenseCall down_call(const BlockRef& b, const void* in, int bf16, int64_t n, const int32_t* n_dev, const void* wfrag);
int block_tail(const float* x, const float* res, const int32_t* boff, int B, int64_t n, int ch, const float* eca, int eca_k,
               float* partial, float* out, hipStream_t st);
enum Pooling { POOL_GEM = 1, POOL_MAC = 2, POOL_SPOC = 3 };
int global_pool(Pooling method, const float* x, const int32_t* boff, int B, int C, const float* p, float* partial, float* out,
                hipStream_t st);
bool global_tail_fusable(const MlpRef& r);
int global_tail(const MlpRef& r, const void* const* pk, const float* g5, int64_t ncap, const int32_t* n_dev, const int32_t* boff, int B,
                Pooling method, const float* p, bool fused, float* gh, float* gd, float* partial, float* out, hipStream_t st);

bool topdown_split_supported(int C, int Cl);
int topdown_split_forward(Ctx* ctx, int level_out, const float* x_coarse, const void* sp_tconv, const float* x_lateral,
                          const void* sp_lateral, int C, int Cl, float* out, hipStream_t stream);

}
```

egonn_amd/csrc/model.hip:

```cpp
#include "model.h"

using namespace egonn;

namespace {

const int PLANES[7] = {32, 64, 64, 128, 128, 128, 128};
const int GLOBAL_CH = 128, GLOBAL_DIM = 256, LOCAL_CH = 64, LOCAL_DIM = 128;

}

API const char* egonn_last_error(void) { return last_error(); }

API int egonn_debug_set_naive_conv(egonn_ctx* c, int on) {
  EGONN_REQUIRE(c, EGONN_ERR_INVALID, "debug_set_naive_conv: null context");
  c->sconv.set = sconv_decode(on);
  return EGONN_OK;
}

API int egonn_debug_set_ksplit(egonn_ctx* c, int map_class, int level, int kparts, int kw, int col_parts) {
  EGONN_REQUIRE(c && (map_class == 0 || map_class == 1) && level >= 0 && level < EGONN_NUM_LEVELS, EGONN_ERR_INVALID,
                "debug_set_ksplit: bad argument");
  EGONN_REQUIRE(kparts <= 27 && kw <= 4 && col_parts <= 4, EGONN_ERR_INVALID, "debug_set_ksplit: kparts <= 27, kw <= 4, col_parts <= 4");
  if (kparts >= 0) c->sconv.ks_rule.kparts[map_class][level] = (int8_t)std::max(kparts, 1);
  if (kw >= 0) c->sconv.ks_rule.kw[map_class][level] = (int8_t)kw;
// ... 448 lines not shown
API int egonn_model_set_tensor(egonn_model* m, const char* key, const float* data, int ndim, const int64_t* shape) {
  EGONN_REQUIRE(m && key && data && ndim >= 0 && ndim <= 4, EGONN_ERR_INVALID, "model_set_tensor: bad argument");
  TensorRef r;
  r.p = data;
  r.shape.assign(shape, shape + ndim);
  m->t[key] = r;
  m->ready = false;
  if (m->fpn) minkfpn_model_invalidate(m->fpn);
  return EGONN_OK;
}

namespace egonn {

int get_tensor(egonn_model* m, const std::string& key, std::initializer_list<int64_t> want, const float** out) {
  auto it = m->t.find(key);
  EGONN_REQUIRE(it != m->t.end(), EGONN_ERR_STATE, "model: missing state_dict tensor '%s'", key.c_str());
  const std::vector<int64_t>& s = it->second.shape;
  bool ok = s.size() == want.size();
  size_t i = 0;
  for (int64_t w : want) {
    if (ok && s[i] != w) ok = false;
    ++i;
  }
  if (!ok) {
    std::string got = "(", exp = "(";
    for (int64_t v : s) got += std::to_string(v) + ",";
    for (int64_t v : want) exp += std::to_string(v) + ",";
    set_error("model: tensor '%s' has shape %s), expected %s)", key.c_str(), got.c_str(), exp.c_str());
    return EGONN_ERR_INVALID;
  }
  *out = it->second.p;
  return EGONN_OK;
}

int get_bn(egonn_model* m, const std::string& prefix, int c, BnRef* bn, ModelStore* store) {
  bn->c = c;
  EGONN_TRY(get_tensor(m, prefix + ".bn.weight", {c}, &bn->w));
  EGONN_TRY(get_tensor(m, prefix + ".bn.bias", {c}, &bn->b));
  EGONN_TRY(get_tensor(m, prefix + ".bn.running_mean", {c}, &bn->rm));
  EGONN_TRY(get_tensor(m, prefix + ".bn.running_var", {c}, &bn->rv));
  store->add_bn(bn);
  return EGONN_OK;
}

int eca_ksize(int c) {
  int lg = 0;
  while ((1 << lg) < c) ++lg;
  const int t = (lg + 1) / 2;
  return (t % 2) ? t : t + 1;
}

int get_block(egonn_model* m, const std::string& prefix, int ci, int co, bool eca, BlockRef* b, ModelStore* store) {
  *b = BlockRef();
  b->cin = ci;
  b->cout = co;
  EGONN_TRY(get_tensor(m, prefix + ".conv1.kernel", {27, ci, co}, &b->conv1));
  EGONN_TRY(get_bn(m, prefix + ".norm1", co, &b->n1, store));
  EGONN_TRY(get_tensor(m, prefix + ".conv2.kernel", {27, co, co}, &b->conv2));
  EGONN_TRY(get_bn(m, prefix + ".norm2", co, &b->n2, store));
  if (ci != co) {
    EGONN_TRY(get_tensor(m, prefix + ".downsample.0.kernel", {ci, co}, &b->down));
    EGONN_TRY(get_bn(m, prefix + ".downsample.1", co, &b->dn, store));
  }
  if (eca) {
    b->eca_k = eca_ksize(co);
    EGONN_TRY(get_tensor(m, prefix + ".eca.conv.weight", {1, 1, b->eca_k}, &b->eca));
  }
  return EGONN_OK;
}

void ModelStore::begin() {
  bns.clear();
  packs.clear();
  bn_bytes = pack_bytes = 0;
}
void ModelStore::add_bn(BnRef* bn) {
  bns.push_back(bn);
  bn_bytes += align_up((size_t)2 * bn->c * sizeof(float), 256);
}
void ModelStore::add_pack(Form form, const float* w, int K, int ci, int co, const void** dst) {
  packs.push_back({form, w, K, ci, co, pack_bytes, dst});
  const size_t n = (size_t)K * ci * co;
  pack_bytes += align_up(form == SPLIT ? split_weights_bytes(K, ci, co) : form == RG16 ? n * 2 : n * 4, 256);
}
void ModelStore::add_kernel(const float* w, int K, int ci, int co, bool bf16, PackedKernel* dst) {
  *dst = PackedKernel();
  add_pack(RG32, w, K, ci, co, &dst->rg32);
  if (bf16) add_pack(RG16, w, K, ci, co, &dst->rg16);
  if (sconv_split_supported(ci, co)) add_pack(SPLIT, w, K, ci, co, &dst->split);
}
int ModelStore::commit(hipStream_t st) {
  auto grow = [](char** buf, size_t* cap, size_t need) -> int {
    if (*cap >= need) return EGONN_OK;
    if (*buf) HIP_CHECK(hipFree(*buf));
    *buf = nullptr;
    *cap = 0;
    HIP_CHECK(hipMalloc(reinterpret_cast<void**>(buf), need));
    *cap = need;
    return EGONN_OK;
  };
  EGONN_TRY(grow(&folded, &folded_cap, bn_bytes));
  EGONN_TRY(grow(&packed, &packed_cap, pack_bytes));
  for (const Pack& k : packs) {
    char* out = packed + k.off;
    switch (k.form) {
      case RG32: EGONN_TRY(pack_rg_weights(k.w, k.K, k.ci, k.co, 0, 0, 0, out, st)); break;
      case RG16: EGONN_TRY(pack_rg_weights(k.w, k.K, k.ci, k.co, 1, 0, 0, out, st)); break;
      case SPLIT: EGONN_TRY(pack_split_weights(k.w, k.K, k.ci, k.co, 0, 0, out, st)); break;
      case DENSE: EGONN_TRY(dense_pack_frags(k.w, 0, k.ci, k.co, reinterpret_cast<float*>(out), st)); break;
      case DENSE_OI: EGONN_TRY(dense_pack_frags(k.w, 1, k.ci, k.co, reinterpret_cast<float*>(out), st)); break;
    }
    *k.dst = out;
  }
  char* cur = folded;
  for (BnRef* bn : bns) {
    bn->scale = reinterpret_cast<float*>(cur);
    bn->shift = bn->scale + bn->c;
    cur += align_up((size_t)2 * bn->c * sizeof(float), 256);
    EGONN_TRY(bn_fold(bn->w, bn->b, bn->rm, bn->rv, 1e-5f, bn->c, bn->scale, bn->shift, st));
  }
  return EGONN_OK;
}
void ModelStore::release() {
  if (folded) (void)hipFree(folded);
  if (packed) (void)hipFree(packed);
  folded = packed = nullptr;
  folded_cap = packed_cap = 0;
}

}

namespace {

int get_mlp(egonn_model* m, const std::string& prefix, int cin, int mid, int cout, MlpRef* r) {
  r->cin = cin; r->mid = mid; r->cout = cout;
  EGONN_TRY(get_tensor(m, prefix + ".net.0.linear.weight", {mid, cin}, &r->w0));
  EGONN_TRY(get_tensor(m, prefix + ".net.0.linear.bias", {mid}, &r->b0));
  EGONN_TRY(get_tensor(m, prefix + ".net.2.linear.weight", {cout, mid}, &r->w1));
  EGONN_TRY(get_tensor(m, prefix + ".net.2.linear.bias", {cout}, &r->b1));
  return EGONN_OK;
}

}

API int egonn_model_finalize(egonn_model* m, void* stream) {
  EGONN_REQUIRE(m, EGONN_ERR_INVALID, "model_finalize: null model");
  hipStream_t st = (hipStream_t)stream;
  ModelStore& S = m->store;
  S.begin();
  auto dense = [&](const float* w, int ci, int co, const void** dst, ModelStore::Form form = ModelStore::DENSE) {
    *dst = nullptr;
    if (ci % 16 == 0 && co % 16 == 0) S.add_pack(form, w, 1, ci, co, dst);
  };
  EGONN_TRY(get_tensor(m, "trunk.convs.0.kernel", {125, 1, 32}, &m->conv0));
  EGONN_TRY(get_bn(m, "trunk.bn.0", 32, &m->bn[0], &S));
  int inpl = PLANES[0];
  for (int i = 1; i <= 7; ++i) {
    const std::string si = std::to_string(i);
    const int cout = PLANES[i - 1];
    EGONN_TRY(get_tensor(m, "trunk.convs." + si + ".kernel", {8, inpl, inpl}, &m->convs[i]));
    EGONN_TRY(get_bn(m, "trunk.bn." + si, inpl, &m->bn[i], &S));
    BlockRef& b = m->blk[i];
    EGONN_TRY(get_block(m, "trunk.blocks." + si + ".0", inpl, cout, true, &b, &S));
    S.add_kernel(m->convs[i], 8, inpl, inpl, true, &m->pk_convs[i]);
    S.add_kernel(b.conv1, 27, inpl, cout, true, &m->pk_c1[i]);
    S.add_kernel(b.conv2, 27, cout, cout, true, &m->pk_c2[i]);
    m->pk_down[i] = nullptr;
    if (b.down) dense(b.down, inpl, cout, &m->pk_down[i]);
    inpl = cout;
  }
  for (int l : {5, 6, 7}) {
    EGONN_TRY(get_tensor(m, "global_head.conv1x1." + std::to_string(l) + ".kernel", {PLANES[l - 1], GLOBAL_CH}, &m->g1x1[l]));
    dense(m->g1x1[l], PLANES[l - 1], GLOBAL_CH, &m->pk_g1x1[l]);
  }
  for (int l : {6, 7}) {
    EGONN_TRY(get_tensor(m, "global_head.tconv." + std::to_string(l) + ".kernel", {8, GLOBAL_CH, GLOBAL_CH}, &m->gt[l]));
    S.add_kernel(m->gt[l], 8, GLOBAL_CH, GLOBAL_CH, true, &m->pk_gt[l]);
  }
  for (int l : {3, 4}) {
    EGONN_TRY(get_tensor(m, "local_head.conv1x1." + std::to_string(l) + ".kernel", {PLANES[l - 1], LOCAL_CH}, &m->l1x1[l]));
    dense(m->l1x1[l], PLANES[l - 1], LOCAL_CH, &m->pk_l1x1[l]);
  }
  EGONN_TRY(get_tensor(m, "local_head.tconv.4.kernel", {8, LOCAL_CH, LOCAL_CH}, &m->lt[4]));
  S.add_kernel(m->lt[4], 8, LOCAL_CH, LOCAL_CH, true, &m->pk_lt[4]);
  m->gem_p = nullptr;
  if (m->t.count("global_pooling.pooling.p")) EGONN_TRY(get_tensor(m, "global_pooling.pooling.p", {1}, &m->gem_p));
  EGONN_TRY(get_mlp(m, "global_descriptor_decoder", GLOBAL_CH, GLOBAL_DIM + (GLOBAL_CH - GLOBAL_DIM) / 2, GLOBAL_DIM, &m->gdec));
  m->pk_gdec[0] = m->pk_gdec[1] = nullptr;
  if (global_tail_fusable(m->gdec)) {
    dense(m->gdec.w0, m->gdec.cin, m->gdec.mid, &m->pk_gdec[0], ModelStore::DENSE_OI);
    dense(m->gdec.w1, m->gdec.mid, m->gdec.cout, &m->pk_gdec[1], ModelStore::DENSE_OI);
  }
  EGONN_TRY(get_mlp(m, "local_descriptor_decoder", LOCAL_CH, LOCAL_DIM + (LOCAL_CH - LOCAL_DIM) / 2, LOCAL_DIM, &m->ldec));
  EGONN_TRY(get_mlp(m, "local_keypoint_regressor", LOCAL_CH, LOCAL_CH / 2, 3, &m->kp));
  EGONN_TRY(get_mlp(m, "local_sigma_regressor", LOCAL_CH, LOCAL_CH / 2, 1, &m->sg));

  EGONN_TRY(S.commit(st));
  if (!m->conv0_unit) HIP_CHECK(hipMalloc(&m->conv0_unit, 2 * 4 * 3 * 64 * 16));
  EGONN_TRY(conv0_pack_unit(m->conv0, m->conv0_unit, st));
  if (m->ldec.cin == 64 && m->ldec.mid == 96 && m->ldec.cout == 128 && m->kp.mid == 32 && m->sg.mid == 32 && m->kp.cin == 64 &&
      m->sg.cin == 64) {
    if (!m->lh_pack) HIP_CHECK(hipMalloc(&m->lh_pack, local_heads_pack_bytes()));
    if (!m->lh_ptrs) HIP_CHECK(hipMalloc(reinterpret_cast<void**>(&m->lh_ptrs), 6 * sizeof(float*)));
    const float* hp[6] = {m->ldec.w0, m->ldec.w1, m->kp.w0, m->kp.w1, m->sg.w0, m->sg.w1};
    HIP_CHECK(hipMemcpyAsync(m->lh_ptrs, hp, sizeof(hp), hipMemcpyHostToDevice, st));
    HIP_CHECK(hipStreamSynchronize(st));
    EGONN_TRY(local_heads_pack(m->lh_ptrs, m->lh_pack, st));
  }
  m->ready = true;
  return EGONN_OK;
}

namespace {

int run_mlp(const MlpRef& r, const float* x, int64_t n, int act_out, float* hidden, float* out, hipStream_t st,
            const int32_t* n_dev) {
  EGONN_TRY(dense_forward({.in = x, .n = n, .n_dev = n_dev, .cin = r.cin, .cout = r.mid, .W = r.w0, .w_out_in = 1, .bias = r.b0,
                           .act = ACT_RELU, .out = hidden},
                          st));
  return dense_forward({.in = hidden, .n = n, .n_dev = n_dev, .cin = r.mid, .cout = r.cout, .W = r.w1, .w_out_in = 1, .bias = r.b1,
                        .act = act_out, .out = out},
                       st);
}

}

namespace egonn {

int claim_work(egonn_ctx* c, size_t bytes, bool with_ksplit, Arena** A) {
  for (int l = 0; l < EGONN_NUM_LEVELS; ++l) c->level_feat[l] = nullptr;
  c->ks_part = nullptr;
  c->ks_part_floats = 0;
  EGONN_TRY(c->work_arena.ensure(bytes));
  c->work_arena.reset();
  *A = &c->work_arena;
  const size_t ks = with_ksplit ? sconv_ksplit_scratch_floats(c) : 0;
  if (ks) {
    c->ks_part = (*A)->alloc<float>(ks);
    EGONN_REQUIRE(c->ks_part, EGONN_ERR_STATE, "work arena too small (ks_part)");
    c->ks_part_floats = ks;
  }
  return EGONN_OK;
}

int conv_layer(egonn_ctx* c, hipStream_t st, const ConvCall& cc, const char* what) {
  static const int pk[3] = {PK_K3, PK_K2S2, PK_TCONV};
  char tag[64];
  snprintf(tag, sizeof(tag), "%s<%d,%d>/L%d/%s", sconv_kernel_name(c, cc.kind, cc.level, cc.cin, cc.cout, cc.bf16), cc.cin, cc.cout,
           cc.level, what);
  ProfScope ps(c, st, tag, pk[cc.kind], cc.level, cc.kind == 0 ? 27 : 8, cc.cin, cc.cout, cc.bf16 ? 2 : 4);
  return sconv_map(c, cc, st);
}
ConvCall conv_call(int kind, int level, const void* in, const PackedKernel& pk, int cin, int cout, int bf16, const BnRef* bn, int relu,
                   void* out) {
  return ConvCall{.kind = kind, .level = level, .in = in, .out = out, .cin = cin, .cout = cout, .bf16 = bf16,
                  .scale = bn ? bn->scale : nullptr, .shift = bn ? bn->shift : nullptr, .relu = relu, .packed = &pk};
}

int ensure_graph_rowgroups(egonn_ctx* c, int L, const int* tlevels, int nt, hipStream_t st) {
  int kinds[RG_MAX_JOBS], levels[RG_MAX_JOBS], n = 0;
  for (int l = 1; l <= L; ++l) { kinds[n] = 0; levels[n++] = l; }
  for (int l = 1; l <= L; ++l) { kinds[n] = 1; levels[n++] = l; }
  for (int i = 0; i < nt; ++i) { kinds[n] = 2; levels[n++] = tlevels[i]; }
  return ensure_rowgroups(c, kinds, levels, n, st);
}

int block_convs(egonn_ctx* c, hipStream_t st, Arena* A, int level, const BlockRef& b, const PackedKernel& pk1, const PackedKernel& pk2,
                int bf16, const void* in, float* psum, void** t2_out) {
  const size_t bytes = (size_t)c->plan.cap[level] * b.cout * (bf16 ? 2 : 4);
  WALLOC(char, t1, bytes);
  WALLOC(char, t2, bytes);
  const bool t1_split = !switches().no_presplit && sconv_route(c, 0, level, b.cin, b.cout, bf16) == ROUTE_SPLIT &&
                        sconv_route(c, 0, level, b.cout, b.cout, bf16) == ROUTE_SPLIT;
  ConvCall c1 = conv_call(0, level, in, pk1, b.cin, b.cout, bf16, &b.n1, 1, t1);
  c1.split_io = t1_split ? 2 : 0;
  EGONN_TRY(conv_layer(c, st, c1, "k3.conv1"));
  ConvCall c2 = conv_call(0, level, t1, pk2, b.cout, b.cout, bf16, &b.n2, 0, t2);
  c2.split_io = t1_split ? 1 : 0;
  c2.psum = psum;
  EGONN_TRY(conv_layer(c, st, c2, "k3.conv2"));
  *t2_out = t2;
  return EGONN_OK;
}

DenseCall down_call(const BlockRef& b, const void* in, int bf16, int64_t n, const int32_t* n_dev, const void* wfrag) {
  return DenseCall{.in = in, .in_bf16 = bf16, .n = n, .n_dev = n_dev, .cin = b.cin, .cout = b.cout, .W = b.down,
                   .wfrag = static_cast<const float*>(wfrag), .scale = b.dn.scale, .shift = b.dn.shift, .out_bf16 = bf16};
}

static int pool_pow_mode(Pooling method) { return method == POOL_GEM ? 1 : method == POOL_MAC ? 2 : 0; }
static int global_pool_finish(Pooling method, const float* partial, const int32_t* boff, int B, int C, const float* p, float* out,
                              hipStream_t st) {
  if (method == POOL_GEM) return gem_finish(partial, boff, B, C, p, out, st);
  return pool_finish(partial, boff, B, C, pool_pow_mode(method), out, st);
}
int global_pool(Pooling method, const float* x, const int32_t* boff, int B, int C, const float* p, float* partial, float* out,
                hipStream_t st) {
  EGONN_TRY(segment_partial_sums(x, boff, B, C, pool_pow_mode(method), method == POOL_GEM ? p : nullptr, partial, st));
  return global_pool_finish(method, partial, boff, B, C, p, out, st);
}

bool global_tail_fusable(const MlpRef& r) { return r.cin == GTAIL_CIN && r.mid == GTAIL_MID && r.cout == GTAIL_OUT; }
int global_tail(const MlpRef& r, const void* const* pk, const float* g5, int64_t ncap, const int32_t* n_dev, const int32_t* boff, int B,
                Pooling method, const float* p, bool fused, float* gh, float* gd, float* partial, float* out, hipStream_t st) {
  if (fused) {
    EGONN_REQUIRE(global_tail_fusable(r) && pk && pk[0] && pk[1], EGONN_ERR_STATE, "global tail: no fused form for %d->%d->%d", r.cin,
                  r.mid, r.cout);
    EGONN_TRY(global_tail_fused(g5, ncap, boff, B, static_cast<const float*>(pk[0]), r.b0, static_cast<const float*>(pk[1]), r.b1,
                                pool_pow_mode(method), method == POOL_GEM ? p : nullptr, partial, st));
    return global_pool_finish(method, partial, boff, B, r.cout, p, out, st);
  }
  EGONN_TRY(run_mlp(r, g5, ncap, ACT_NONE, gh, gd, st, n_dev));
  return global_pool(method, gd, boff, B, r.cout, p, partial, out, st);
}

int block_tail(const float* x, const float* res, const int32_t* boff, int B, int64_t n, int ch, const float* eca, int eca_k,
               float* partial, float* out, hipStream_t st) {
  if (!eca) return add_act(x, res, n * ch, 1, out, st);
  EGONN_TRY(segment_partial_sums(x, boff, B, ch, 0, nullptr, partial, st));
  return eca_apply(x, res, partial, boff, B, n, ch, eca, eca_k, out, st);
}

}

API int egonn_forward(egonn_ctx* c, egonn_model* m, const float* features, int quant_mode, const float* step, int flags,
                      float* out_global, float* out_desc, float* out_kp, float* out_sigma, void* stream) {
  REQUIRE_PLAN(c);
  EGONN_REQUIRE(m && m->ready, EGONN_ERR_STATE, "model not finalized (call egonn_model_finalize)");
  EGONN_REQUIRE(step, EGONN_ERR_INVALID, "forward: null argument");
  HIP_CHECK(hipSetDevice(c->device));
  hipStream_t st = (hipStream_t)stream;
  Plan& P = c->plan;
  const int B = P.batch;
  const int32_t* cnt = c->dev_counts;
  const int bf16 = (flags & EGONN_FLAG_BF16) ? 1 : 0;
  const size_t es = bf16 ? 2 : 4;
  const bool do_global = !(flags & EGONN_FLAG_DISABLE_GLOBAL);
  const bool do_local = !(flags & EGONN_FLAG_DISABLE_LOCAL);
  EGONN_REQUIRE(!do_global || out_global, EGONN_ERR_INVALID, "forward: out_global is null");
  EGONN_REQUIRE(!do_local || (out_desc && out_kp && out_sigma), EGONN_ERR_INVALID, "forward: local outputs are null");
  HIP_CHECK(hipMemsetAsync(c->dev_fp16_flag, 0, sizeof(int32_t), st));

  {
    const int tlevels[3] = {6, 5, 3};
    EGONN_TRY(ensure_graph_rowgroups(c, 7, tlevels + (do_global ? 0 : 2), (do_global ? 2 : 0) + (do_local ? 1 : 0), st));
    DBG_SYNC("row groups");
  }

  size_t need = (size_t)P.cap[0] * (1 + 32) * 4;
  for (int i = 1; i <= 7; ++i) need += (size_t)P.cap[i] * 128 * 4 * 6 + (size_t)P.lv[i].rg27.cap_groups * 128 * 4;
  need += (size_t)P.cap[5] * (192 + 256 + 128 * 2) * 4 + (size_t)P.cap[3] * (96 + 32 + 32 + 3 + 64 * 2) * 4;
  need += (size_t)B * SEG_CHUNKS * 256 * 4 * 10 + (size_t)P.cap[3] * 32 + (4u << 20);
  need += sconv_ksplit_scratch_floats(c) * 4 + 4096;
  Arena* A;
  EGONN_TRY(claim_work(c, need, true, &A));

  const int64_t n0 = P.cap[0];
  const float* f0 = features;
  if (features && !c->from_points) {
    WALLOC(float, fg, n0);
    EGONN_TRY(gather_rows(features, P.perm0, n0, 1, fg, st, cnt));
    f0 = fg;
  }
  WALLOC(char, x0, n0 * 32 * es);
  {
    ProfScope ps(c, st, "conv0_k5_kernel/L0", PK_CONV0, 0, 125, 1, 32, (int)es);
    EGONN_TRY(conv0_k5_forward(c, f0, m->conv0, 32, m->bn[0].scale, m->bn[0].shift, 1, x0, bf16, st, m->conv0_unit));
  }
  DBG_SYNC("conv0");
  const void* x[8] = {x0};
  c->level_feat[0] = x0;
  c->level_ch[0] = 32;
  c->level_bf16 = bf16;
  auto local_head = [&](hipStream_t st) -> int {
    const int64_t n3 = P.cap[3], n4 = P.cap[4];
    WALLOC(char, l4, n4 * LOCAL_CH * es);
    EGONN_TRY(dense_forward({.in = x[4], .in_bf16 = bf16, .n = n4, .n_dev = cnt + 4, .cin = 128, .cout = LOCAL_CH, .W = m->l1x1[4],
                             .wfrag = static_cast<const float*>(m->pk_l1x1[4]), .out = l4, .out_bf16 = bf16},
                            st));
    WALLOC(char, u3, n3 * LOCAL_CH * es);
    EGONN_TRY(conv_layer(c, st, conv_call(2, 3, l4, m->pk_lt[4], LOCAL_CH, LOCAL_CH, bf16, nullptr, 0, u3), "tconv"));
    EGONN_REQUIRE(m->ldec.cin == 64 && m->ldec.mid == 96 && m->ldec.cout == 128 && m->kp.mid == 32 && m->sg.mid == 32,
                  EGONN_ERR_STATE, "local heads: unexpected layer sizes");
    const float* hw[12] = {m->ldec.w0, m->ldec.b0, m->ldec.w1, m->ldec.b1, m->kp.w0, m->kp.b0, m->kp.w1, m->kp.b1,
                           m->sg.w0, m->sg.b0, m->sg.w1, m->sg.b1};
    const void* lh_pack = (!switches().no_split_heads && sconv_split_arithmetic(c)) ? m->lh_pack : nullptr;
    if (!switches().no_fused_lateral && LOCAL_CH == 64) {
      EGONN_TRY(local_heads_forward(reinterpret_cast<const float*>(x[3]), n3, cnt + 3, hw, P.lv[3].keys, 3, P.coord_bits, quant_mode,
                                    step, (flags & EGONN_FLAG_IGNORE_KP_REGRESSOR) ? 1 : 0, out_desc, out_kp, out_sigma, st,
                                    m->l1x1[3], reinterpret_cast<const float*>(u3), bf16, lh_pack, c->dev_fp16_flag));
      return EGONN_OK;
    }
    WALLOC(float, l3, n3 * LOCAL_CH);
    EGONN_TRY(dense_forward({.in = x[3], .in_bf16 = bf16, .n = n3, .n_dev = cnt + 3, .cin = 64, .cout = LOCAL_CH, .W = m->l1x1[3],
                             .wfrag = static_cast<const float*>(m->pk_l1x1[3]), .residual = u3, .res_bf16 = bf16, .out = l3},
                            st));
    EGONN_TRY(local_heads_forward(l3, n3, cnt + 3, hw, P.lv[3].keys, 3, P.coord_bits, quant_mode, step,
                                  (flags & EGONN_FLAG_IGNORE_KP_REGRESSOR) ? 1 : 0, out_desc, out_kp, out_sigma, st, nullptr, nullptr, 0,
                                  lh_pack, c->dev_fp16_flag));
    return EGONN_OK;
  };
  const float *gated_t2 = nullptr, *gated_res = nullptr, *gated_gate = nullptr;
  for (int i = 1; i <= 7; ++i) {
    const BlockRef& b = m->blk[i];
    const Level& L = P.lv[i];
    const int64_t n = P.cap[i];
    WALLOC(char, y, n * b.cin * es);
    {
      ConvCall cc = conv_call(1, i, x[i - 1], m->pk_convs[i], b.cin, b.cin, bf16, &m->bn[i], 1, y);
      if (gated_t2 && i == 2) {
        cc.in = gated_t2;
        cc.in2 = gated_res;
        cc.gate = gated_gate;
      }
      EGONN_TRY(conv_layer(c, st, cc, "k2s2"));
    }
    DBG_SYNC("L%d k2s2", i);
    WALLOC(float, psum, (size_t)L.rg27.cap_groups * b.cout);
    void* t2 = nullptr;
    EGONN_TRY(block_convs(c, st, A, i, b, m->pk_c1[i], m->pk_c2[i], bf16, y, psum, &t2));
    WALLOC(float, gate, (size_t)B * b.cout);
    DBG_SYNC("L%d convs", i);
    EGONN_TRY(eca_gate_groups(psum, L.rg27, L.boff, B, b.cout, b.eca, b.eca_k, gate, st));
    DBG_SYNC("L%d eca gate", i);
    const void* res = y;
    if (i == 1 && !switches().no_gated_k2s2 && !c->keep_level_features && !bf16 && !b.down && c->sconv.set.product() && b.cout == 32 &&
        m->blk[2].cin == 32 && sconv_route(c, 1, 2, 32, 32, 0) == ROUTE_SPLIT) {
      gated_t2 = reinterpret_cast<const float*>(t2);
      gated_res = reinterpret_cast<const float*>(y);
      gated_gate = gate;
      x[i] = nullptr;
      c->level_feat[i] = nullptr;
      c->level_ch[i] = b.cout;
      continue;
    }
    WALLOC(char, xo, n * b.cout * es);
    const DenseCall down = down_call(b, y, bf16, n, cnt + i, m->pk_down[i]);
    if (b.down && !switches().no_fused_down && dense_gate_fusable(n, b.cin, b.cout)) {
      DenseCall dc = down;
      dc.residual = t2; dc.res_bf16 = bf16;
      dc.gate = gate; dc.boff = L.boff; dc.B = B;
      dc.out = xo;
      EGONN_TRY(dense_forward(dc, st));
    } else {
      if (b.down) {
        WALLOC(char, rd, n * b.cout * es);
        DenseCall dc = down;
        dc.out = rd;
        EGONN_TRY(dense_forward(dc, st));
        res = rd;
      }
      EGONN_TRY(eca_apply_gate(t2, res, gate, L.boff, B, n, b.cout, xo, bf16, st));
    }
    DBG_SYNC("L%d eca apply", i);
    x[i] = xo;
    c->level_feat[i] = xo;
    c->level_ch[i] = b.cout;
  }
  if (do_local) EGONN_TRY(local_head(st));
  DBG_SYNC("local head");

  void* g5_fused = nullptr;
  if (do_global && !switches().no_fused_ghead && !bf16 && c->sconv.set.product() && dense_group3_rows(P.cap[5]) &&
      dense_group3_rows(P.cap[6]) && dense_group3_rows(P.cap[7])) {
    WALLOC(float, l7, P.cap[7] * GLOBAL_CH);
    WALLOC(float, l6, P.cap[6] * GLOBAL_CH);
    WALLOC(float, l5, P.cap[5] * GLOBAL_CH);
    WALLOC(float, g6f, P.cap[6] * GLOBAL_CH);
    WALLOC(float, g5f, P.cap[5] * GLOBAL_CH);
    const float* gin[3] = {reinterpret_cast<const float*>(x[7]), reinterpret_cast<const float*>(x[6]), reinterpret_cast<const float*>(x[5])};
    const int64_t gn[3] = {P.cap[7], P.cap[6], P.cap[5]};
    const int32_t* gnd[3] = {cnt + 7, cnt + 6, cnt + 5};
    const float* gw[3] = {m->g1x1[7], m->g1x1[6], m->g1x1[5]};
    float* gout[3] = {l7, l6, l5};
    const float* gpk[3] = {static_cast<const float*>(m->pk_g1x1[7]), static_cast<const float*>(m->pk_g1x1[6]),
                           static_cast<const float*>(m->pk_g1x1[5])};
    EGONN_TRY(dense_small_group3(gin, gn, gnd, gw, switches().no_packed_laterals ? nullptr : gpk, gout, st));
    for (int lv = 6; lv >= 5; --lv) {
      ConvCall cc = conv_call(2, lv, lv == 6 ? l7 : g6f, m->pk_gt[lv + 1], GLOBAL_CH, GLOBAL_CH, 0, nullptr, 0, lv == 6 ? g6f : g5f);
      cc.residual = lv == 6 ? l6 : l5;
      EGONN_TRY(conv_layer(c, st, cc, "tconv"));
    }
    g5_fused = g5f;
    DBG_SYNC("global head (fused)");
  }
  if (do_global) {
    const float* g5 = reinterpret_cast<const float*>(g5_fused);
    if (!g5) {
    auto lateral = [&](int l, const void* up, void* out, int out_bf16) {
      return dense_forward({.in = x[l], .in_bf16 = bf16, .n = P.cap[l], .n_dev = cnt + l, .cin = 128, .cout = GLOBAL_CH, .W = m->g1x1[l],
                            .residual = up, .res_bf16 = up ? bf16 : 0, .out = out, .out_bf16 = out_bf16},
                           st);
    };
    WALLOC(char, g7, P.cap[7] * GLOBAL_CH * es);
    EGONN_TRY(lateral(7, nullptr, g7, bf16));
    WALLOC(char, u6, P.cap[6] * GLOBAL_CH * es);
    EGONN_TRY(conv_layer(c, st, conv_call(2, 6, g7, m->pk_gt[7], GLOBAL_CH, GLOBAL_CH, bf16, nullptr, 0, u6), "tconv"));
    WALLOC(char, g6, P.cap[6] * GLOBAL_CH * es);
    EGONN_TRY(lateral(6, u6, g6, bf16));
    WALLOC(char, u5, P.cap[5] * GLOBAL_CH * es);
    EGONN_TRY(conv_layer(c, st, conv_call(2, 5, g6, m->pk_gt[6], GLOBAL_CH, GLOBAL_CH, bf16, nullptr, 0, u5), "tconv"));
    WALLOC(float, g5u, P.cap[5] * GLOBAL_CH);
    EGONN_TRY(lateral(5, u5, g5u, 0));
    g5 = g5u;
    DBG_SYNC("global head");
    }
    WALLOC(float, gh, P.cap[5] * m->gdec.mid);
    WALLOC(float, gd, P.cap[5] * GLOBAL_DIM);
    WALLOC(float, gp, (size_t)B * SEG_CHUNKS * GLOBAL_DIM);
    const Pooling pool = (flags & EGONN_FLAG_POOL_MAC) ? POOL_MAC : (flags & EGONN_FLAG_POOL_SPOC) ? POOL_SPOC : POOL_GEM;
    EGONN_REQUIRE(pool != POOL_GEM || m->gem_p, EGONN_ERR_STATE, "forward: GeM pooling needs the tensor 'global_pooling.pooling.p'");
    const bool fused_tail = !switches().no_fused_gtail && global_tail_fusable(m->gdec) && m->pk_gdec[0] && m->pk_gdec[1];
    EGONN_TRY(global_tail(m->gdec, m->pk_gdec, g5, P.cap[5], cnt + 5, P.lv[5].boff, B, pool, m->gem_p, fused_tail, gh, gd, gp, out_global, st));
  }

  DBG_SYNC("global decoder + pooling");
  return EGONN_OK;
}

static size_t debug_tail_span(int64_t ncap) {
  return align_up((size_t)ncap * GTAIL_MID * 4, 256) + align_up((size_t)ncap * GTAIL_OUT * 4, 256) +
         align_up((size_t)GTAIL_CIN * GTAIL_MID * 4, 256) + align_up((size_t)GTAIL_MID * GTAIL_OUT * 4, 256) + 1024;
}
API int64_t egonn_debug_global_tail_scratch_bytes(int64_t rows_capacity) {
  if (rows_capacity < 0 || rows_capacity >= (1ll << 31) / GTAIL_OUT) return -1;
  return (int64_t)debug_tail_span(rows_capacity);
}
API int egonn_debug_global_tail(const float* g5, const int32_t* row_offsets, int batch_size, int64_t rows_capacity, const int32_t* n_dev,
                                const float* w0, const float* b0, const float* w1, const float* b1, const float* p, int pooling, int form,
                                float* partial, float* out, void* scratch, int64_t scratch_bytes, void* stream) {
  EGONN_REQUIRE(g5 && row_offsets && n_dev && w0 && b0 && w1 && b1 && partial && out && scratch, EGONN_ERR_INVALID,
                "debug_global_tail: null pointer");
  EGONN_REQUIRE(batch_size >= 1 && batch_size <= EGONN_MAX_BATCH, EGONN_ERR_INVALID, "debug_global_tail: batch_size=%d outside [1, %d]",
                batch_size, EGONN_MAX_BATCH);
  EGONN_REQUIRE(rows_capacity >= 0 && rows_capacity < (1ll << 31) / GTAIL_OUT, EGONN_ERR_INVALID,
                "debug_global_tail: rows_capacity=%lld outside [0, 2^31 / %d)", (long long)rows_capacity, GTAIL_OUT);
  EGONN_REQUIRE(pooling >= POOL_GEM && pooling <= POOL_SPOC && (pooling != POOL_GEM || p), EGONN_ERR_INVALID,
                "debug_global_tail: pooling=%d (1 GeM with its exponent, 2 MAC, 3 SPoC)", pooling);
  EGONN_REQUIRE(form == 0 || form == 1, EGONN_ERR_INVALID, "debug_global_tail: form=%d (0 three launches, 1 the fused launch)", form);
  const size_t need = debug_tail_span(rows_capacity);
  EGONN_REQUIRE(scratch_bytes >= (int64_t)need && ((uintptr_t)scratch & 255) == 0, EGONN_ERR_INVALID,
                "debug_global_tail: scratch needs %lld bytes, 256-byte aligned", (long long)need);
  hipStream_t st = (hipStream_t)stream;
  Arena ws = Arena::view(scratch, need);
  float* gh = ws.alloc<float>((size_t)rows_capacity * GTAIL_MID);
  float* gd = ws.alloc<float>((size_t)rows_capacity * GTAIL_OUT);
  float* pk0 = ws.alloc<float>((size_t)GTAIL_CIN * GTAIL_MID);
  float* pk1 = ws.alloc<float>((size_t)GTAIL_MID * GTAIL_OUT);
  EGONN_REQUIRE(gh && gd && pk0 && pk1, EGONN_ERR_STATE, "debug_global_tail: scratch span too small");
  const MlpRef r{.w0 = w0, .b0 = b0, .w1 = w1, .b1 = b1, .cin = GTAIL_CIN, .mid = GTAIL_MID, .cout = GTAIL_OUT};
  const void* pk[2] = {pk0, pk1};
  if (form == 1) {
    EGONN_TRY(dense_pack_frags(w0, 1, r.cin, r.mid, pk0, st));
    EGONN_TRY(dense_pack_frags(w1, 1, r.mid, r.cout, pk1, st));
  }
  return global_tail(r, pk, g5, rows_capacity, n_dev, row_offsets, batch_size, (Pooling)pooling, p, form == 1, gh, gd, partial, out, st);
}

API int egonn_forward_level_features(egonn_ctx* c, int level, float* out, int channels, void* stream) {
  REQUIRE_PLAN(c);
  EGONN_REQUIRE(level >= 0 && level < EGONN_NUM_LEVELS && c->level_feat[level], EGONN_ERR_STATE,
                "no features for level %d (run egonn_forward first; level 1 of fp32 maps is materialised only after "
                "egonn_debug_keep_level_features(ctx, 1))", level);
  EGONN_REQUIRE(channels == c->level_ch[level], EGONN_ERR_INVALID, "level %d has %d channels, caller expects %d", level,
                c->level_ch[level], channels);
  const int64_t cnt = c->plan.lv[level].n * channels;
  if (c->level_bf16) return convert_bf16_to_f32(c->level_feat[level], cnt, out, (hipStream_t)stream);
  HIP_CHECK(hipMemcpyAsync(out, c->level_feat[level], sizeof(float) * cnt, hipMemcpyDeviceToDevice, (hipStream_t)stream));
  return EGONN_OK;
}

API int egonn_select_keypoints(egonn_ctx* c, const float* sigma, const float* keypoints, const float* descriptors,
                               int n_k, float* sel_kp, float* sel_desc, int32_t* sel_rows, int32_t* sel_count,
                               void* stream) {
  REQUIRE_PLAN(c);
  EGONN_REQUIRE(sigma && keypoints && descriptors && sel_kp && sel_desc && sel_rows && sel_count, EGONN_ERR_INVALID,
                "select_keypoints: null argument");
  HIP_CHECK(hipSetDevice(c->device));
  return select_topk(sigma, c->plan.lv[3].boff, c->plan.batch, n_k, keypoints, descriptors, LOCAL_DIM, sel_rows, sel_count,
                     sel_kp, sel_desc, (hipStream_t)stream);
}


API int egonn_topk_rows(const float* sigma, const int32_t* row_offsets, int batch_size, int n_k, int32_t* sel_rows,
                        int32_t* sel_count, void* stream) {
  EGONN_REQUIRE(sigma && row_offsets && sel_rows && sel_count && batch_size >= 1, EGONN_ERR_INVALID, "topk_rows: bad argument");
  return select_topk(sigma, row_offsets, batch_size, n_k, nullptr, nullptr, 0, sel_rows, sel_count, nullptr, nullptr,
                     (hipStream_t)stream);
}

API int egonn_profile_enable(egonn_ctx* c, int mode, const char* filter) {
  EGONN_REQUIRE(c && mode >= 0 && mode <= 3, EGONN_ERR_INVALID, "profile_enable: bad argument");
  c->prof.mode = mode;
  snprintf(c->prof.filter, sizeof(c->prof.filter), "%s", filter ? filter : "");
  return EGONN_OK;
}

API int egonn_profile_fetch(egonn_ctx* c, int cap, int* n, char* names, float* ms, double* bytes, double* flops,
                            void* stream) {
  EGONN_REQUIRE(c && n && names && ms && bytes && flops, EGONN_ERR_INVALID, "profile_fetch: null argument");
  HIP_CHECK(hipSetDevice(c->device));
  Plan& P = c->plan;
  if (P.valid) {
    if (P.built_reserved) P.exact = false;
    EGONN_TRY(plan_sync(c, (hipStream_t)stream));
    EGONN_TRY(count_map_pairs(c, (hipStream_t)stream));
  }
  HIP_CHECK(hipStreamSynchronize((hipStream_t)stream));
  unsigned long long pairs[16];
  HIP_CHECK(hipMemcpy(pairs, c->dev_pairs, sizeof(pairs), hipMemcpyDeviceToHost));
  int w = 0;
  std::vector<ProfRec> all(c->prof.recs);
  all.insert(all.end(), c->prof.graph_recs.begin(), c->prof.graph_recs.end());
  const size_t n_plain = c->prof.recs.size();
  size_t ri = 0;
  for (auto& r : all) {
    const bool plain = ri++ < n_plain;
    float t = 0.f;
    if (hipEventSynchronize(r.e1) != hipSuccess || hipEventElapsedTime(&t, r.e0, r.e1) != hipSuccess) {
      (void)hipGetLastError();
      if (plain) { c->prof.pool.push_back(r.e0); c->prof.pool.push_back(r.e1); }
      continue;
    }
    if (w < cap) {
      const double n_out = (double)P.lv[r.level].n;
      double Pn = 0;
      switch (r.kind) {
        case PK_CONV0: Pn = (double)pairs[0]; break;
        case PK_K3: Pn = (double)pairs[r.level]; break;
        case PK_K2S2: Pn = (double)P.lv[r.level - 1].n; break;
        case PK_TCONV: Pn = n_out; break;
        default: Pn = n_out; break;
      }
      snprintf(names + (size_t)w * 64, 64, "%s", r.name);
      ms[w] = t;
      bytes[w] = Pn * r.cin * r.es + n_out * r.cout * r.es + (double)r.K * r.cin * r.cout * r.es + 8.0 * Pn;
      flops[w] = 2.0 * Pn * r.cin * r.cout;
      ++w;
    }
    if (plain) { c->prof.pool.push_back(r.e0); c->prof.pool.push_back(r.e1); }
  }
  c->prof.recs.clear();
  *n = w;
  return EGONN_OK;
}
```

egonn_amd/csrc/rowwise.hip:

```cpp
#include "common.h"
#include "kernels.h"
#include "rowmath.h"

namespace egonn {

__global__ void bn_fold_kernel(const float* __restrict__ w, const float* __restrict__ b,
                               const float* __restrict__ rm, const float* __restrict__ rv, float eps, int c,
                               float* __restrict__ scale, float* __restrict__ shift) {
  const int i = blockIdx.x * blockDim.x + threadIdx.x;
  if (i >= c) return;
  const float s = w[i] / sqrtf(rv[i] + eps);
  scale[i] = s;
  shift[i] = b[i] - rm[i] * s;
}
int bn_fold(const float* w, const float* b, const float* rm, const float* rv, float eps, int c, float* scale,
            float* shift, hipStream_t stream) {
  hipLaunchKernelGGL(bn_fold_kernel, dim3((unsigned)cdiv(c, 128)), dim3(128), 0, stream, w, b, rm, rv, eps, c, scale,
                     shift);
  HIP_CHECK(hipGetLastError());
  return EGONN_OK;
}

__global__ void gather_rows_kernel(const float* __restrict__ in, const int32_t* __restrict__ perm, int64_t n, int c,
                                   float* __restrict__ out, const int32_t* __restrict__ n_dev) {
  const int64_t t = (int64_t)blockIdx.x * blockDim.x + threadIdx.x;
  if (n_dev) n = min((int64_t)*n_dev, n);
  if (t >= n * c) return;
  const int64_t r = t / c;
  const int ch = (int)(t - r * c);
  out[t] = in[(int64_t)perm[r] * c + ch];
}
int gather_rows(const float* in, const int32_t* perm, int64_t n, int c, float* out, hipStream_t stream, const int32_t* n_dev) {
  if (n == 0) return EGONN_OK;
  hipLaunchKernelGGL(gather_rows_kernel, dim3((unsigned)cdiv(n * c, 256)), dim3(256), 0, stream, in, perm, n, c, out, n_dev);
  HIP_CHECK(hipGetLastError());
  return EGONN_OK;
}

__global__ __launch_bounds__(256) void segment_partial_kernel(const float* __restrict__ in,
                                                               const int32_t* __restrict__ boff, int c, int pow_mode,
                                                               const float* __restrict__ pexp,
                                                               float* __restrict__ partial) {
  __shared__ float red[256];
  const int b = blockIdx.y, ch = blockIdx.x;
  const int32_t s = boff[b], e = boff[b + 1];
  const int64_t len = e - s;
  const int32_t r0 = s + (int32_t)(len * ch / SEG_CHUNKS), r1 = s + (int32_t)(len * (ch + 1) / SEG_CHUNKS);
  const int tid = threadIdx.x;
  const float p = pow_mode == 1 ? pexp[0] : 1.f;
  const int rl = tid / c, cidx = tid - rl * c, nrl = 256 / c;
  float acc = pow_mode == 2 ? -INFINITY : 0.f;
  if (rl < nrl) {
    for (int32_t r = r0 + rl; r < r1; r += nrl) {
      float v = in[(int64_t)r * c + cidx];
      if (pow_mode == 1) v = powf(fmaxf(v, 1e-6f), p);
      acc = pow_mode == 2 ? fmaxf(acc, v) : acc + v;
    }
  }
  red[tid] = acc;
  __syncthreads();
  if (tid < c) {
    float sum = pow_mode == 2 ? -INFINITY : 0.f;
    for (int k = 0; k < nrl; ++k) sum = pow_mode == 2 ? fmaxf(sum, red[k * c + tid]) : sum + red[k * c + tid];
    partial[((int64_t)b * SEG_CHUNKS + ch) * c + tid] = sum;
  }
}
int segment_partial_sums(const float* in, const int32_t* boff, int B, int c, int pow_mode, const float* p,
                         float* partial, hipStream_t stream) {
  EGONN_REQUIRE(c >= 1 && c <= 256 && 256 % c == 0, EGONN_ERR_INVALID, "segment sums: %d channels unsupported", c);
  hipLaunchKernelGGL(segment_partial_kernel, dim3(SEG_CHUNKS, B), dim3(256), 0, stream, in, boff, c, pow_mode, p,
                     partial);
  HIP_CHECK(hipGetLastError());
  return EGONN_OK;
}

__global__ void eca_gate_kernel(const float* __restrict__ partial, const int32_t* __restrict__ boff, int c,
                                const float* __restrict__ wconv, int ksize, float* __restrict__ gate) {
  extern __shared__ float mean[];
  const int b = blockIdx.x, t = threadIdx.x;
  const int32_t cntr = boff[b + 1] - boff[b];
  if (t < c) {
    float s = 0.f;
    for (int ch = 0; ch < SEG_CHUNKS; ++ch) s += partial[((int64_t)b * SEG_CHUNKS + ch) * c + t];
    mean[t] = cntr > 0 ? s / (float)cntr : 0.f;
  }
  __syncthreads();
  if (t < c) {
    const int pad = (ksize - 1) / 2;
    float y = 0.f;
    for (int j = 0; j < ksize; ++j) {
      const int q = t + j - pad;
      if (q >= 0 && q < c) y += wconv[j] * mean[q];
    }
    gate[(int64_t)b * c + t] = 1.f / (1.f + expf(-y));
  }
}


template <bool BF16>
__global__ void eca_apply_kernel(const void* __restrict__ x, const void* __restrict__ res,
                                 const float* __restrict__ gate, const int32_t* __restrict__ boff, int B, int64_t n,
                                 int cq_shift, void* __restrict__ out) {
  constexpr int CPT = BF16 ? 8 : 4;
  const int64_t t = (int64_t)blockIdx.x * blockDim.x + threadIdx.x;
  n = min((int64_t)boff[B], n);
  if (t >= (n << cq_shift)) return;
  const int32_t r = (int32_t)(t >> cq_shift);
  const int q = (int)(t - ((int64_t)r << cq_shift));
  const int b = sample_of_row(boff, B, r);
  const float* gp = gate + (((int64_t)b << cq_shift) + q) * CPT;
  float xv[CPT], rv[CPT], g[CPT];
  if constexpr (BF16) {
    const uint4 xh = reinterpret_cast<const uint4*>(x)[t], rh = reinterpret_cast<const uint4*>(res)[t];
    const uint32_t xw[4] = {xh.x, xh.y, xh.z, xh.w}, rw[4] = {rh.x, rh.y, rh.z, rh.w};
#pragma unroll
    for (int i = 0; i < 4; ++i) {
      xv[2 * i] = bf2f(xw[i] & 0xFFFFu); xv[2 * i + 1] = bf2f(xw[i] >> 16);
      rv[2 * i] = bf2f(rw[i] & 0xFFFFu); rv[2 * i + 1] = bf2f(rw[i] >> 16);
    }
    const float4 g0 = reinterpret_cast<const float4*>(gp)[0], g1 = reinterpret_cast<const float4*>(gp)[1];
    g[0] = g0.x; g[1] = g0.y; g[2] = g0.z; g[3] = g0.w; g[4] = g1.x; g[5] = g1.y; g[6] = g1.z; g[7] = g1.w;
  } else {
    const float4 xf = reinterpret_cast<const float4*>(x)[t], rf = reinterpret_cast<const float4*>(res)[t];
    const float4 g0 = reinterpret_cast<const float4*>(gp)[0];
    xv[0] = xf.x; xv[1] = xf.y; xv[2] = xf.z; xv[3] = xf.w;
    rv[0] = rf.x; rv[1] = rf.y; rv[2] = rf.z; rv[3] = rf.w;
    g[0] = g0.x; g[1] = g0.y; g[2] = g0.z; g[3] = g0.w;
  }
  float o[CPT];
#pragma unroll
  for (int i = 0; i < CPT; ++i) o[i] = fmaxf(xv[i] * g[i] + rv[i], 0.f);
  if constexpr (BF16) {
    uint4 oh;
    oh.x = f2bf_rn(o[0]) | (f2bf_rn(o[1]) << 16);
    oh.y = f2bf_rn(o[2]) | (f2bf_rn(o[3]) << 16);
    oh.z = f2bf_rn(o[4]) | (f2bf_rn(o[5]) << 16);
    oh.w = f2bf_rn(o[6]) | (f2bf_rn(o[7]) << 16);
    reinterpret_cast<uint4*>(out)[t] = oh;
  } else {
    reinterpret_cast<float4*>(out)[t] = make_float4(o[0], o[1], o[2], o[3]);
  }
}
__global__ void bf16_to_f32_kernel(const uint16_t* __restrict__ in, int64_t n, float* __restrict__ out) {
  const int64_t t = (int64_t)blockIdx.x * blockDim.x + threadIdx.x;
  if (t < n) out[t] = bf2f(in[t]);
}
int convert_bf16_to_f32(const void* in, int64_t n, float* out, hipStream_t stream) {
  if (n == 0) return EGONN_OK;
  hipLaunchKernelGGL(bf16_to_f32_kernel, dim3((unsigned)cdiv(n, 256)), dim3(256), 0, stream,
                     reinterpret_cast<const uint16_t*>(in), n, out);
  HIP_CHECK(hipGetLastError());
  return EGONN_OK;
}

int eca_apply(const float* x, const float* res, const float* partial, const int32_t* boff, int B, int64_t n, int c,
              const float* wconv, int ksize, float* out, hipStream_t stream) {
  EGONN_REQUIRE(c >= 4 && c <= 256 && c % 4 == 0, EGONN_ERR_INVALID, "eca: %d channels unsupported (4..256, multiple of 4)", c);
  if (n == 0) return EGONN_OK;
  float* gate = const_cast<float*>(partial) + (int64_t)B * SEG_CHUNKS * c;
  hipLaunchKernelGGL(eca_gate_kernel, dim3(B), dim3(256), c * sizeof(float), stream, partial, boff, c, wconv, ksize,
                     gate);
  const int c4 = c / 4;
  EGONN_REQUIRE((c4 & (c4 - 1)) == 0, EGONN_ERR_INVALID, "eca_apply: %d channels (a power of two expected)", c);
  hipLaunchKernelGGL(eca_apply_kernel<false>, dim3((unsigned)cdiv(n * c4, 256)), dim3(256), 0, stream, x, res, gate, boff, B,
                     n, __builtin_ctz(c4), out);
  HIP_CHECK(hipGetLastError());
  return EGONN_OK;
}

__global__ __launch_bounds__(1024) void eca_gate_groups_kernel(const float* __restrict__ psum,
                                                                const uint32_t* __restrict__ gmask,
                                                                const int32_t* __restrict__ meta,
                                                                const int32_t* __restrict__ boff, int c,
                                                                const float* __restrict__ wconv, int ksize,
                                                                float* __restrict__ gate) {
  __shared__ float red[1024];
  __shared__ float mean[256];
  const int b = blockIdx.x, tid = threadIdx.x;
  const int g0 = meta[1 + b], g1 = meta[2 + b];
  const int32_t cntr = boff[b + 1] - boff[b];
  const int nsl = 1024 / c, sl = tid / c, ch = tid - sl * c;
  float acc = 0.f;
  {
    constexpr int U = 8;
    int g = g0 + sl;
    for (; g + (U - 1) * nsl < g1; g += U * nsl) {
      float v[U];
      uint32_t m[U];
#pragma unroll
      for (int u = 0; u < U; ++u) {
        m[u] = gmask[g + u * nsl];
        v[u] = psum[(int64_t)(g + u * nsl) * c + ch];
      }
#pragma unroll
      for (int u = 0; u < U; ++u) acc += (m[u] >> 31) ? v[u] : 0.f;
    }
    for (; g < g1; g += nsl) {
      const uint32_t m = gmask[g];
      const float v = psum[(int64_t)g * c + ch];
      acc += (m >> 31) ? v : 0.f;
    }
  }
  red[tid] = acc;
  __syncthreads();
  if (tid < c) {
    float s = 0.f;
    for (int k = 0; k < nsl; ++k) s += red[k * c + tid];
    mean[tid] = cntr > 0 ? s / (float)cntr : 0.f;
  }
  __syncthreads();
  if (tid < c) {
    const int pad = (ksize - 1) / 2;
    float y = 0.f;
    for (int j = 0; j < ksize; ++j) {
      const int q = tid + j - pad;
      if (q >= 0 && q < c) y += wconv[j] * mean[q];
    }
    gate[(int64_t)b * c + tid] = 1.f / (1.f + expf(-y));
  }
}
int eca_gate_groups(const float* psum, const RowGroups& rg, const int32_t* boff, int B, int c, const float* wconv, int ksize,
                    float* gate, hipStream_t stream) {
  EGONN_REQUIRE(c >= 32 && c <= 256 && 256 % c == 0, EGONN_ERR_INVALID, "eca gate: %d channels unsupported", c);
  hipLaunchKernelGGL(eca_gate_groups_kernel, dim3(B), dim3(1024), 0, stream, psum, rg.gmask, rg.meta, boff, c, wconv, ksize,
                     gate);
  HIP_CHECK(hipGetLastError());
  return EGONN_OK;
}
int eca_apply_gate(const void* x, const void* res, const float* gate, const int32_t* boff, int B, int64_t n, int c,
                   void* out, int bf16, hipStream_t stream) {
  if (n == 0) return EGONN_OK;
  const int cq = bf16 ? c / 8 : c / 4;
  EGONN_REQUIRE(cq >= 1 && (cq & (cq - 1)) == 0, EGONN_ERR_INVALID, "eca_apply: %d channels (a power of two expected)", c);
  if (bf16)
    hipLaunchKernelGGL(eca_apply_kernel<true>, dim3((unsigned)cdiv(n * cq, 256)), dim3(256), 0, stream, x, res, gate, boff, B, n,
                       __builtin_ctz(cq), out);
  else
    hipLaunchKernelGGL(eca_apply_kernel<false>, dim3((unsigned)cdiv(n * cq, 256)), dim3(256), 0, stream, x, res, gate, boff, B, n,
                       __builtin_ctz(cq), out);
  HIP_CHECK(hipGetLastError());
  return EGONN_OK;
}

__global__ void add_act_kernel(const float* __restrict__ a, const float* __restrict__ b, int64_t n, int relu,
                               float* __restrict__ out) {
  const int64_t t = (int64_t)blockIdx.x * blockDim.x + threadIdx.x;
  if (t >= n) return;
  const float v = a[t] + b[t];
  out[t] = relu ? fmaxf(v, 0.f) : v;
}
int add_act(const float* a, const float* b, int64_t n, int relu, float* out, hipStream_t stream) {
  if (n == 0) return EGONN_OK;
  hipLaunchKernelGGL(add_act_kernel, dim3((unsigned)cdiv(n, 256)), dim3(256), 0, stream, a, b, n, relu, out);
  HIP_CHECK(hipGetLastError());
  return EGONN_OK;
}

__global__ void gem_finish_kernel(const float* __restrict__ partial, const int32_t* __restrict__ boff, int c,
                                  const float* __restrict__ pexp, int mode, float* __restrict__ out) {
  const int b = blockIdx.x, t = threadIdx.x;
  if (t >= c) return;
  const int32_t cntr = boff[b + 1] - boff[b];
  if (mode == 2) {
    float s = -INFINITY;
    for (int ch = 0; ch < SEG_CHUNKS; ++ch) s = fmaxf(s, partial[((int64_t)b * SEG_CHUNKS + ch) * c + t]);
    out[(int64_t)b * c + t] = cntr > 0 ? s : 0.f;
    return;
  }
  float s = 0.f;
  for (int ch = 0; ch < SEG_CHUNKS; ++ch) s += partial[((int64_t)b * SEG_CHUNKS + ch) * c + t];
  const float m = cntr > 0 ? s / (float)cntr : 0.f;
  out[(int64_t)b * c + t] = pexp ? powf(m, 1.f / pexp[0]) : m;
}
int gem_finish(const float* partial, const int32_t* boff, int B, int c, const float* p, float* out,
               hipStream_t stream) {
  EGONN_REQUIRE(c >= 1 && c <= 256, EGONN_ERR_INVALID, "gem: %d channels unsupported (1..256)", c);
  hipLaunchKernelGGL(gem_finish_kernel, dim3(B), dim3(256), 0, stream, partial, boff, c, p, 0, out);
  HIP_CHECK(hipGetLastError());
  return EGONN_OK;
}

int pool_finish(const float* partial, const int32_t* boff, int B, int c, int mode, float* out, hipStream_t stream) {
  EGONN_REQUIRE(c >= 1 && c <= 256 && (mode == 0 || mode == 2), EGONN_ERR_INVALID, "pooling: bad arguments");
  hipLaunchKernelGGL(gem_finish_kernel, dim3(B), dim3(256), 0, stream, partial, boff, c, (const float*)nullptr, mode, out);
  HIP_CHECK(hipGetLastError());
  return EGONN_OK;
}

__global__ void l2norm_kernel(float* __restrict__ x, int64_t n, int c, const int32_t* __restrict__ n_dev) {
  const int lane = threadIdx.x & 63;
  const int64_t row = (int64_t)blockIdx.x * (blockDim.x >> 6) + (threadIdx.x >> 6);
  if (n_dev) n = min((int64_t)*n_dev, n);
  if (row >= n) return;
  float* p = x + row * c;
  float ss = 0.f;
  for (int i = lane; i < c; i += 64) ss += p[i] * p[i];
#pragma unroll
  for (int o = 32; o > 0; o >>= 1) ss += __shfl_xor(ss, o, 64);
  const float inv = 1.f / fmaxf(sqrtf(ss), 1e-12f);
  for (int i = lane; i < c; i += 64) p[i] *= inv;
}
int l2_normalize_rows(float* x, int64_t n, int c, hipStream_t stream, const int32_t* n_dev) {
  if (n == 0) return EGONN_OK;
  hipLaunchKernelGGL(l2norm_kernel, dim3((unsigned)cdiv(n, 4)), dim3(256), 0, stream, x, n, c, n_dev);
  HIP_CHECK(hipGetLastError());
  return EGONN_OK;
}

}
```

include/egonn_hip.h:

```cpp
#ifndef EGONN_HIP_H
#define EGONN_HIP_H

#include <stdint.h>

#ifdef __cplusplus
extern "C" {
#endif

typedef struct egonn_ctx egonn_ctx;
typedef struct egonn_model egonn_model;

enum { EGONN_QUANT_CARTESIAN = 0, EGONN_QUANT_POLAR = 1 };
enum { EGONN_STATUS_OK = 0, EGONN_STATUS_INVALID = 1, EGONN_STATUS_HIP = 2, EGONN_STATUS_RANGE = 3, EGONN_STATUS_STATE = 4,
       EGONN_STATUS_CAPACITY = 5,
       EGONN_STATUS_FP16_RANGE = 6 };
enum { EGONN_FLAG_DISABLE_GLOBAL = 1, EGONN_FLAG_DISABLE_LOCAL = 2, EGONN_FLAG_IGNORE_KP_REGRESSOR = 4,
       EGONN_FLAG_BF16 = 8,
       EGONN_FLAG_POOL_SPOC = 16, EGONN_FLAG_POOL_MAC = 32 };

int egonn_ctx_create(egonn_ctx** ctx, int device, int coord_bits);
void egonn_ctx_destroy(egonn_ctx* ctx);
const char* egonn_last_error(void);
int egonn_debug_set_naive_conv(egonn_ctx* ctx, int on);
int egonn_debug_set_ksplit(egonn_ctx* ctx, int map_class, int level, int kparts, int kw, int col_parts);
int egonn_debug_set_resident(egonn_ctx* ctx, int mask, int max_workgroups);
int egonn_debug_keep_level_features(egonn_ctx* ctx, int on);
int egonn_debug_set_trace(void* device_buffer);
int egonn_debug_rowgroup_tables(egonn_ctx* ctx, int map_kind, int level_out, uint32_t* gmask_out, int32_t* snbr_out,
                                int64_t capacity_groups, int64_t* n_groups, void* stream);
int egonn_debug_rowgroup_perm(egonn_ctx* ctx, int map_kind, int level_out, int32_t* perm_out, int64_t capacity_groups,
                              int64_t* n_groups, void* stream);
int64_t egonn_debug_radix_sort_scratch_bytes(int64_t n, int n_segments);
int egonn_debug_radix_sort(uint64_t* keys_in, uint32_t* vals_in, uint64_t* keys_out, uint32_t* vals_out, int64_t n, int nbits,
                           const int64_t* n_dev, const int64_t* seg_offsets, int n_segments, int idx_bits, int either_pair,
                           int32_t* result_pair, void* scratch, int64_t scratch_bytes, void* stream);
int egonn_debug_dense_group3(const float* const in[3], const int64_t rows_capacity[3], const int32_t* const n_dev[3],
                             const float* const weight[3], const float* const packed[3], float* const out[3], void* stream);
int64_t egonn_debug_global_tail_scratch_bytes(int64_t rows_capacity);
int egonn_debug_global_tail(const float* g5, const int32_t* row_offsets, int batch_size, int64_t rows_capacity, const int32_t* n_dev,
                            const float* w0, const float* b0, const float* w1, const float* b1, const float* p, int pooling, int form,
                            float* partial, float* out, void* scratch, int64_t scratch_bytes, void* stream);

int egonn_voxelize(egonn_ctx* ctx, const float* points, const int64_t* scan_offsets, int batch_size, int quant_mode,
                   const float* step, void* stream);
int egonn_ctx_reserve(egonn_ctx* ctx, int64_t max_points, int batch_size, const int64_t* level_capacity);
int egonn_voxelize_device(egonn_ctx* ctx, const float* points, int64_t n_rows, const int64_t* scan_offsets_dev,
                          int batch_size, int quant_mode, const float* step, void* stream);
int egonn_plan_status(egonn_ctx* ctx, void* stream);
int egonn_ctx_set_exact_fp32(egonn_ctx* ctx, int on);
int egonn_ctx_set_operand_autoscale(egonn_ctx* ctx, int on);
int egonn_level_capacity(egonn_ctx* ctx, int level, int64_t* capacity);
typedef struct egonn_graph egonn_graph;
int egonn_graph_begin(void* stream);
int egonn_graph_end(void* stream, egonn_graph** graph);
int egonn_graph_launch(egonn_graph* graph, void* stream);
void egonn_graph_destroy(egonn_graph* graph);
int egonn_coords_set(egonn_ctx* ctx, const int32_t* coords, int64_t n, int batch_size, void* stream);

int egonn_level_count(egonn_ctx* ctx, int level, int64_t* n_rows);
int egonn_level_batch_offsets(egonn_ctx* ctx, int level, int64_t* offsets );
int egonn_level_coords(egonn_ctx* ctx, int level, int32_t* out, void* stream);
int egonn_input_index(egonn_ctx* ctx, int64_t* out , void* stream);

int egonn_conv(egonn_ctx* ctx, int level_in, int level_out, int kernel_size, const float* in, int cin,
               const float* kernel, int cout, const float* scale, const float* shift, int relu, float* out,
               void* stream);
int egonn_conv_transpose(egonn_ctx* ctx, int level_in, const float* in, int cin, const float* kernel, int cout,
                         float* out, void* stream);
int egonn_sparse_conv(egonn_ctx* ctx, int map_kind, int level_out, const void* in, int cin, const float* kernel, int cout,
                      int bf16, const float* scale, const float* shift, int relu, void* out, float* group_sums,
                      void* stream);
int egonn_prepare_maps(egonn_ctx* ctx, int with_level0_transpose, void* stream);
int egonn_map_groups(egonn_ctx* ctx, int map_kind, int level_out, int64_t* n_groups, int64_t* first_group, void* stream);
int egonn_global_avg_pool(egonn_ctx* ctx, int level, const float* in, int channels, float* out, void* stream);

int egonn_bn_fold(const float* weight, const float* bias, const float* running_mean, const float* running_var,
                  float eps, int channels, float* scale, float* shift, void* stream);
int egonn_block_tail(egonn_ctx* ctx, int level, const float* x, const float* residual, int channels,
                     const float* eca_weight, int eca_ksize, float* out, void* stream);
int egonn_add(const float* a, const float* b, int64_t n, float* out, void* stream);
int egonn_gather_input(egonn_ctx* ctx, const float* features, int channels, float* out, void* stream);
int egonn_gem(egonn_ctx* ctx, int level, const float* x, int channels, const float* p, float* out, void* stream);
int egonn_global_max_pool(egonn_ctx* ctx, int level, const float* in, int channels, float* out, void* stream);
int egonn_netvlad(egonn_ctx* ctx, int level, const float* x, int channels, const float* cluster_weights,
                  const float* cluster_weights2, const float* bn1_scale, const float* bn1_shift,
                  const float* hidden1_weights, const float* bn2_scale, const float* bn2_shift,
                  const float* gating_weights, const float* gate_scale, const float* gate_shift, int out_dim, int gating,
                  float* out, void* stream);
int egonn_netvlad_train_forward(egonn_ctx* ctx, int level, const float* x, int channels, int nmax,
                                const float* cluster_weights, const float* cluster_weights2, const float* bn1_weight,
                                const float* bn1_bias, float bn1_eps, float bn1_momentum, float* bn1_running_mean,
                                float* bn1_running_var, const float* hidden1_weights, int out_dim, float* out, float* save_z,
                                float* save_bn1, float* save_v, float* save_sq, float* save_asum, void* stream);
int egonn_netvlad_train_backward(egonn_ctx* ctx, int level, const float* x, int channels, int nmax,
                                 const float* cluster_weights, const float* cluster_weights2, const float* bn1_weight,
                                 const float* hidden1_weights, int out_dim, const float* grad_out, const float* save_z,
                                 const float* save_bn1, const float* save_v, const float* save_sq, const float* save_asum,
                                 float* grad_x, float* grad_cluster_weights, float* grad_cluster_weights2, float* out_bn1,
                                 float* grad_hidden1_weights, void* stream);
int egonn_global_max_pool_argmax(egonn_ctx* ctx, int level, const float* in, int channels, float* out, int32_t* out_rows,
                                 void* stream);
int egonn_global_max_pool_backward(egonn_ctx* ctx, int level, const float* grad_out, const int32_t* rows, int channels,
                                   float* grad_in, void* stream);
int egonn_sigmoid_gate(const float* y, const float* t, const float* grad_out, int64_t n, float* out, float* grad_y,
                       float* grad_t, void* stream);

int egonn_model_create(egonn_model** model);
void egonn_model_destroy(egonn_model* model);
int egonn_model_set_tensor(egonn_model* model, const char* key, const float* data, int ndim, const int64_t* shape);
int egonn_model_finalize(egonn_model* model, void* stream);

int egonn_forward(egonn_ctx* ctx, egonn_model* model, const float* features, int quant_mode, const float* step,
                  int flags, float* out_global, float* out_descriptors, float* out_keypoints, float* out_sigma,
                  void* stream);
int egonn_forward_level_features(egonn_ctx* ctx, int level, float* out, int channels, void* stream);

int egonn_minkfpn_finalize(egonn_model* model, int n_levels, const int* planes, const int* layers, int num_top_down,
                           int feature_size, int block, int pooling, void* stream);
int egonn_minkfpn_out_level(int n_levels, int num_top_down, int* level);
enum { EGONN_MINKFPN_SPLIT_TOPDOWN = 1 };
int egonn_minkfpn_forward(egonn_ctx* ctx, egonn_model* model, int flags, float* out_global, float* out_map, void* stream);
int egonn_topdown_step(egonn_ctx* ctx, int level_out, const float* x_coarse, const float* w_tconv, const float* x_lateral,
                       const float* w_lateral, int C, int Cl, float* out, void* stream);

int egonn_select_keypoints(egonn_ctx* ctx, const float* sigma, const float* keypoints, const float* descriptors,
                           int n_k, float* sel_keypoints, float* sel_descriptors, int32_t* sel_rows,
                           int32_t* sel_count, void* stream);

int egonn_topk_rows(const float* sigma, const int32_t* row_offsets, int batch_size, int n_k, int32_t* sel_rows,
                    int32_t* sel_count, void* stream);

int64_t egonn_triplet_loss_scratch_floats(int n);
int egonn_triplet_loss(const float* embeddings, int n, int d, const uint8_t* positives_mask,
                       const uint8_t* negatives_mask, float margin, float* out_stats, int32_t* out_triplets,
                       float* out_grad, float* scratch, void* stream);

int64_t egonn_contrastive_loss_scratch_floats(int n);
int egonn_contrastive_loss(const float* embeddings, int n, int d, const uint8_t* positives_mask,
                           const uint8_t* negatives_mask, float pos_margin, float neg_margin, float* out_stats,
                           int32_t* out_triplets, float* out_grad, float* scratch, void* stream);

int egonn_nn_search(const float* a, int64_t n, const float* transform, const float* b, int64_t m, float* out_dist,
                    int32_t* out_index, void* stream);
int egonn_matrix_min(const float* d, int64_t n, int64_t m, float* row_min, int32_t* row_index, float* col_min,
                     int32_t* col_index, void* stream);
int egonn_softmax_cross_entropy(const float* logits, int64_t n, int64_t m, const int32_t* target, float* out_loss,
                                int32_t* out_argmax, float* out_dlogits, void* stream);

#define EGONN_LOCAL_LOSS_STATS 16
enum { EGONN_LL_LOSS = 0, EGONN_LL_KP_PER_CLOUD = 1, EGONN_LL_REPEATABILITY = 2, EGONN_LL_CHAMFER_PURE = 3,
       EGONN_LL_CHAMFER_WEIGHTED = 4, EGONN_LL_MEAN_SIGMA = 5, EGONN_LL_LOSS_CHAMFER = 6, EGONN_LL_LOSS_P2P = 7,
       EGONN_LL_KEYPOINT_LOSS = 8, EGONN_LL_CORRESPONDENCE_LOSS = 9, EGONN_LL_MATCHING_KEYPOINTS = 10,
       EGONN_LL_MATCHING_DESCRIPTORS = 11, EGONN_LL_POS_SIMILARITY = 12, EGONN_LL_NEG_SIMILARITY = 13  };
int64_t egonn_local_loss_scratch_bytes(int pairs, int64_t n_kp1, int64_t n_kp2, int dim);
int egonn_local_loss(int pairs, int64_t n_cloud1, int64_t n_cloud2, int64_t n_kp1, int64_t n_kp2, int dim,
                     const float* clouds1, const int32_t* cloud_off1, const float* clouds2, const int32_t* cloud_off2,
                     const float* kp1, const float* sigma1, const float* desc1, const int32_t* kp_off1,
                     const float* kp2, const float* sigma2, const float* desc2, const int32_t* kp_off2,
                     const float* transforms, const float* params, float* out_pair, float* out_batch,
                     float* g_kp1, float* g_sigma1, float* g_desc1, float* g_kp2, float* g_sigma2, float* g_desc2,
                     void* scratch, int64_t scratch_bytes, void* stream);

enum { EGONN_ACT_NONE = 0, EGONN_ACT_RELU = 1, EGONN_ACT_TANH = 2, EGONN_ACT_SOFTPLUS = 3, EGONN_ACT_SIGMOID = 4 };
int egonn_dense(const float* x, int64_t n, int cin, const float* weight, int weight_out_in, const float* bias, int cout,
                int act, float* out, void* stream);
int egonn_dense_pack_fragments(const float* weight, int weight_out_in, int cin, int cout, float* packed, void* stream);
int egonn_dense_pack_fragments_host(const float* weight, int weight_out_in, int cin, int cout, float* packed);
int egonn_debug_dense(const void* in, int in_bf16, int64_t rows_capacity, const int32_t* n_dev, int cin, int cout, const float* weight,
                      int weight_out_in, const float* packed, const float* bias, const float* scale, const float* shift, int act,
                      const void* residual, int res_bf16, const float* gate, const int32_t* boff, int B, void* out, int out_bf16,
                      int form, void* stream);
int egonn_debug_dense_route(int64_t rows, int cin, int cout, int form, int gate_scans, int32_t out[5]);
int egonn_debug_sconv_choice(const int32_t in[16], int64_t cap_groups, int32_t out[20]);
int egonn_dense_backward_weight(const float* a, int ca, const float* b, int cb, int64_t n, float* out, float* scratch,
                                int64_t scratch_floats, void* stream);
int egonn_conv_backward_weight(egonn_ctx* ctx, int level_in, int level_out, int kernel_size, int transposed,
                               const float* in, int cin, const float* grad_out, int cout, float* grad_kernel,
                               float* scratch, int64_t scratch_floats, void* stream);
int egonn_col_stats(int mode, const float* a, const float* b, const float* mask, const float* mean, int64_t n, int c,
                    double* out, float* scratch, int64_t scratch_floats, void* stream);
int egonn_bn_train_finalize(const double* sums, const float* shift_point, double count, int c, const float* weight,
                            const float* bias, float eps, float momentum, float* running_mean, float* running_var,
                            float* out_mean_invstd_scale_shift, void* stream);
int egonn_bn_backward_finalize(const double* local_sums, const double* global_sums, double count, int c, const float* weight,
                               const float* mean, const float* invstd, float* out_abc_dgamma_dbeta, void* stream);
int egonn_affine_act(const float* x, const float* scale, const float* shift, int64_t n, int c, int relu, float* out,
                     void* stream);
int egonn_affine3(const float* g, const float* mask, const float* x, const float* A, const float* B, const float* C,
                  int64_t n, int c, float* out, void* stream);
int egonn_relu_backward(const float* grad_out, const float* out, int64_t n, int c, float* grad_in, void* stream);
int egonn_act_backward(int act, const float* grad_out, const float* out, int64_t n, int c, float* grad_in, void* stream);
int egonn_l2_normalize(const float* x, const float* grad_out, int64_t n, int c, float* out, void* stream);
int egonn_eca_gate(const float* mean, const float* conv_weight, int kernel_size, int batch_size, int channels, float* gate,
                   void* stream);
int egonn_eca_gate_backward(const float* grad_gate, const float* gate, const float* mean, const float* conv_weight,
                            int kernel_size, int batch_size, int channels, float* grad_mean, float* grad_weight,
                            void* stream);
int egonn_se_gate(const float* mean, const float* w1, const float* b1, const float* w2, const float* b2, int batch_size,
                  int channels, int hidden, float* gate, float* hidden_out, void* stream);
int egonn_se_gate_backward(const float* grad_gate, const float* gate, const float* hidden_act, const float* mean,
                           const float* w1, const float* w2, int batch_size, int channels, int hidden, float* grad_mean,
                           float* grad_w1, float* grad_b1, float* grad_w2, float* grad_b2, void* stream);
int egonn_gate_residual(egonn_ctx* ctx, int level, const float* x, const float* gate, const float* residual, int channels,
                        int relu, float* out, void* stream);
int egonn_gate_residual_backward(egonn_ctx* ctx, int level, const float* grad_out, const float* out, const float* gate,
                                 int channels, float* grad_x, float* grad_residual, void* stream);
int egonn_segment_sums(egonn_ctx* ctx, int level, int mode, const float* a, const float* b, const float* x2,
                       const float* p, int channels, float* out, float* scratch, int64_t scratch_floats, void* stream);
int egonn_segment_broadcast(egonn_ctx* ctx, int level, const float* v, int channels, int mean, float* out, void* stream);
int egonn_gem_backward(egonn_ctx* ctx, int level, const float* x, const float* coef, const float* p, int channels,
                       float* grad_x, void* stream);

int64_t egonn_filter_points_scratch_ints(int64_t n);
int egonn_filter_points(const float* raw, int64_t n, int floats_per_point, const int64_t* scan_offsets, int batch_size,
                        int remove_zero_points, int remove_ground_plane, float ground_plane_level, float* out_points,
                        int64_t* out_scan_offsets, int32_t* scratch, int64_t scratch_ints, void* stream);

int egonn_knn(const float* query, int64_t n_query, const float* database, int64_t n_database, int dim, int k,
              int32_t* out_index, float* out_distance, float* scratch, int64_t scratch_floats, void* stream);
int egonn_recall_counts(const int32_t* nn_index, const float* query_positions, const float* map_positions,
                        int64_t n_query, int k, int position_dim, const float* radius, int n_radius,
                        int32_t* out_true_positives, void* stream);

enum { EGONN_REG_STATUS_CLIPPED = 1,
       EGONN_REG_STATUS_FEW_CORR = 2,
       EGONN_REG_STATUS_NO_MODEL = 4,
       EGONN_REG_STATUS_BAD_INDEX = 8 };
int64_t egonn_registration_scratch_bytes(int n_pairs, int n_max, int n_hypotheses);
int64_t egonn_match_mutual_scratch_bytes(int n_pairs, int n_max);
int egonn_match_mutual(const float* feat1, const float* feat2, const int32_t* n1, const int32_t* n2, int n_pairs, int n_max,
                       int dim, int32_t* corr, int32_t* n_corr, void* scratch, int64_t scratch_bytes, void* stream);
int egonn_ransac_pairs(const float* kp1, const float* kp2, const int32_t* n1, const int32_t* n2, const int32_t* corr,
                       const int32_t* n_corr, const int32_t* pair_id, int n_pairs, int n_max, int n_hypotheses, uint64_t seed,
                       double dist_th, void* scratch, int64_t scratch_bytes, int32_t* hyp_count, double* hyp_err2, void* stream);
int egonn_registration_finish(const float* kp1, const float* kp2, const int32_t* n1, const int32_t* n2, const int32_t* corr,
                              const int32_t* n_corr, const int32_t* pair_id, int n_pairs, int n_max, int n_hypotheses,
                              uint64_t seed, double dist_th, const void* scratch, int64_t scratch_bytes, const double* T_gt,
                              double repeat_th, double* T, int32_t* inliers, double* fitness, double* inlier_rmse,
                              int32_t* corr_set, int32_t* best_t, double* rte, double* rre, int32_t* success,
                              double* repeatability, int32_t* status, void* stream);

enum { EGONN_ICP_STATUS_FEW_CORR = 1,
       EGONN_ICP_STATUS_MAX_ITER = 2,
       EGONN_ICP_STATUS_EMPTY = 4,
       EGONN_ICP_STATUS_RANGE = 8 };
int64_t egonn_voxel_downsample_scratch_bytes(int64_t n, int n_clouds);
int egonn_voxel_downsample(const float* points, int64_t n, const int64_t* offsets, int n_clouds, double voxel_size,
                           const float* crop, double* out_points, int64_t* out_offsets, int32_t* out_counts, int32_t* status,
                           void* scratch, int64_t scratch_bytes, void* stream);
int64_t egonn_icp_scratch_bytes(int64_t n_src, int64_t n_tgt, int n_pairs);
int egonn_icp_pairs(const double* src, int64_t n_src, const int64_t* src_offsets, const double* tgt, int64_t n_tgt,
                    const int64_t* tgt_offsets, int n_pairs, const double* T_init, double max_dist, int max_iteration,
                    double eps_fitness, double eps_rmse, double* T, double* fitness, double* inlier_rmse, int32_t* iterations,
                    int32_t* status, double* T_trace, double* eval_trace, int32_t* corr, void* scratch, int64_t scratch_bytes,
                    void* stream);

enum { EGONN_ICP_STATUS_SINGULAR = 16 };
enum { EGONN_NORMALS_STATUS_FEW_POINTS = 1,
       EGONN_NORMALS_STATUS_RANGE = 2 };
int64_t egonn_estimate_normals_scratch_bytes(int64_t n, int n_clouds);
int egonn_estimate_normals(const double* points, int64_t n, const int64_t* offsets, int n_clouds, int knn, double* normals,
                           int32_t* status, int32_t* neighbors, double* eigenvalues, void* scratch, int64_t scratch_bytes,
                           void* stream);
int64_t egonn_icp_plane_scratch_bytes(int64_t n_src, int64_t n_tgt, int n_pairs);
int egonn_icp_plane_pairs(const double* src, int64_t n_src, const int64_t* src_offsets, const double* tgt, int64_t n_tgt,
                          const int64_t* tgt_offsets, const double* tgt_normals, int n_pairs, const double* T_init, double max_dist,
                          int max_iteration, double eps_fitness, double eps_rmse, double* T, double* fitness, double* inlier_rmse,
                          int32_t* iterations, int32_t* status, double* T_trace, double* eval_trace, int32_t* corr, void* scratch,
                          int64_t scratch_bytes, void* stream);

enum { EGONN_AUG_JITTER = 1, EGONN_AUG_REMOVE_POINTS = 2, EGONN_AUG_TRANSLATE = 4, EGONN_AUG_ROTATE = 8, EGONN_AUG_BLOCK = 16,
       EGONN_AUG_SET_ROTATE = 32, EGONN_AUG_FLIP = 64, EGONN_AUG_RIGID = 128, EGONN_AUG_JITTER_CLIP = 256, EGONN_AUG_ALL = 511 };
enum { EGONN_AUG_STATUS_BAD_ID = 1 };
typedef struct egonn_augment_params {
  uint64_t seed;
  uint32_t draw;
  uint32_t set_id;
  uint32_t stages;
  uint32_t reserved;
  double sigma, clip;
  double r_min, r_max;
  double max_delta;
  double max_theta;
  double block_p, scale_lo, scale_hi, ratio_lo, ratio_hi;
  double set_max_theta;
  double flip_cum[3];
  double rot_max, trans_max;
} egonn_augment_params;
int64_t egonn_augment_scratch_bytes(int64_t n, int batch_size);
int egonn_augment_points(const float* points, int64_t n, const int64_t* scan_offsets, int batch_size, const int32_t* scan_ids,
                         const egonn_augment_params* params, const float* T_in, float* out_points, float* T_out,
                         int32_t* rec_i, double* rec_d, uint8_t* flags, void* scratch, int64_t scratch_bytes, void* stream);

int egonn_scan_context(const float* points, int64_t n, const int64_t* scan_offsets, int batch_size, int num_sector,
                       int num_ring, double max_length, double lidar_height, float* out_sc, float* out_ringkey, void* stream);
int egonn_scan_context_ringkey(const float* sc, int64_t n, int num_ring, int num_sector, float* out_ringkey, void* stream);
int egonn_scan_context_distance(const float* query_sc, int64_t n_query, const float* map_sc, int64_t n_map, int num_ring,
                                int num_sector, const int32_t* candidates, int k, float* out_dist, int32_t* out_yaw,
                                void* stream);
int egonn_scan_context_rerank(const float* dist, const int32_t* yaw, const int32_t* candidates, int64_t n_query, int k,
                              int32_t* out_index, float* out_dist, int32_t* out_yaw, void* stream);

enum { EGONN_TUPLES_STATUS_CAPACITY = 1,
       EGONN_TUPLES_STATUS_BAD_OFFSETS = 2,
       EGONN_TUPLES_STATUS_BAD_INDEX = 4 };
enum { EGONN_POSE_STATUS_BAD_ROW = 1,
       EGONN_POSE_STATUS_SINGULAR = 2,
       EGONN_POSE_STATUS_BAD_INDEX = 4 };
int egonn_radius_count(const double* query, int64_t nq, const double* ref, int64_t nm, const double* radii, int n_radius,
                       int exclude_self_mask, int32_t* counts, void* stream);
int egonn_radius_fill(const double* query, int64_t nq, const double* ref, int64_t nm, double radius, int exclude_self,
                      const int64_t* offsets, int32_t* indices, int64_t capacity, int32_t* status, void* stream);
int egonn_pair_masks(const int32_t* labels, int batch_size, const int64_t* pos_offsets, const int32_t* pos_indices, int64_t n_pos,
                     const int64_t* non_offsets, const int32_t* non_indices, int64_t n_non, int64_t n_tuples,
                     uint8_t* positives_mask, uint8_t* negatives_mask, int32_t* status, void* stream);
int egonn_relative_poses(const double* poses, int64_t n_poses, const int32_t* idx_a, const int32_t* idx_b, int64_t n_pairs,
                         int negate_translation, double* out, int32_t* status, void* stream);
int egonn_gather_clouds(const double* bank, int64_t n_bank, const int64_t* bank_offsets, int64_t n_clouds, const int32_t* pick,
                        int n_pick, double* out, int64_t capacity, int64_t* out_offsets, int32_t* status, void* stream);

enum { EGONN_RELOC_NO_CANDIDATE = 1,
       EGONN_RELOC_BAD_INDEX = 2,
       EGONN_RELOC_UNVERIFIED = 4 };
int64_t egonn_match_candidates_scratch_bytes(int n_queries, int k, int n_max);
int egonn_match_candidates(const float* q_feat, const int32_t* q_n, const float* bank_feat, const int32_t* bank_n,
                           const int32_t* nn_index, int n_queries, int k, int n_bank, int n_max, int dim, int32_t* corr,
                           int32_t* n_corr, int32_t* status, void* scratch, int64_t scratch_bytes, void* stream);
int egonn_gather_candidates(const float* q_kp, const int32_t* q_n, const float* bank_kp, const int32_t* bank_n,
                            const int32_t* nn_index, const int32_t* query_id, int n_queries, int k, int n_bank, int n_max,
                            float* kp1, float* kp2, int32_t* n1, int32_t* n2, int32_t* pair_id, void* stream);
int egonn_pick_candidates(const int32_t* nn_index, int n_queries, int k, int n_bank, const double* map_pose, const double* T,
                          const int32_t* inliers, const double* inlier_rmse, const int32_t* reg_status, const double* rte,
                          const double* rre, const int32_t* success, int min_inliers, int32_t* best_rank, int32_t* best_index,
                          int32_t* reranked, double* T_rel, double* pose, int32_t* safe_pick, int32_t* best_inliers,
                          int32_t* status, double* best_rte, double* best_rre, int32_t* best_success, void* stream);

int egonn_profile_enable(egonn_ctx* ctx, int mode, const char* filter);
int egonn_profile_fetch(egonn_ctx* ctx, int cap, int* n, char* names, float* ms, double* bytes, double* flops,
                        void* stream);

#ifdef __cplusplus
}
#endif
#endif
// ... 1 lines not shown
```

Before: 23420.

## Fuse ECA gate computation with gate application and allow multi-chunk global tail

Adds a kernel that computes the ECA channel gate from the grouped partial sums and applies it to the block output in a single launch, chunked across workgroups per scan. A routing function picks this path when the per-scan psum footprint is small and the gate is not shared with a downstream fused consumer. This removes a launch and the gate round-trip through global memory, but each chunk's workgroup recomputes the gate redundantly. The global tail kernel also gains a chunks-per-workgroup template parameter, left at one by default.

```diff
diff --git a/egonn_amd/_lib.py b/egonn_amd/_lib.py
--- a/egonn_amd/_lib.py
+++ b/egonn_amd/_lib.py
@@ -36,6 +36,9 @@
     ("egonn_debug_dense_group3", C.c_int, [_P, _P, _P, _P, _P, _P, _P]),
     ("egonn_debug_global_tail_scratch_bytes", C.c_int64, [C.c_int64]),
     ("egonn_debug_global_tail", C.c_int, [_P, _P, C.c_int, C.c_int64, _P, _P, _P, _P, _P, _P, C.c_int, C.c_int, _P, _P, _P, C.c_int64, _P]),
+    ("egonn_debug_eca_tail", C.c_int, [_P, _P, _P, _P, C.c_int, C.c_int64, C.c_int64, C.c_int, _P, C.c_int, _P, _P, C.c_int, C.c_int,
+                                       C.c_int, _P, _P, _P]),
+    ("egonn_debug_eca_route", C.c_int, [C.c_int64, C.c_int, C.c_int, C.c_int64, C.c_int, C.c_int, C.POINTER(C.c_int32)]),
     ("egonn_voxelize", C.c_int, [_P, _P, C.POINTER(C.c_int64), C.c_int, C.c_int, C.POINTER(C.c_float), _P]),
     ("egonn_ctx_reserve", C.c_int, [_P, C.c_int64, C.c_int, C.POINTER(C.c_int64)]),
     ("egonn_voxelize_device", C.c_int, [_P, _P, C.c_int64, _P, C.c_int, C.c_int, C.POINTER(C.c_float), _P]),
@@ -370,6 +373,24 @@
     return partial, out
 
 
+def debug_eca_tail(psum, gmask, meta, row_offsets, wconv, x, res, out, form: int, chunks: int = 0):
+    lib = load()
+    B = row_offsets.numel() - 1
+    c = x.shape[1]
+    gate = torch.full((B, c), float("nan"), dtype=torch.float32, device=x.device)
+    call(x.device, lib.egonn_debug_eca_tail, psum.data_ptr(), gmask.data_ptr(), meta.data_ptr(), row_offsets.data_ptr(), B,
+         int(gmask.numel()), int(x.shape[0]), int(c), wconv.data_ptr(), int(wconv.numel()), x.data_ptr(), res.data_ptr(),
+         int(x.dtype == torch.bfloat16), int(form), int(chunks), gate.data_ptr(), out.data_ptr())
+    return gate
+
+
+def debug_eca_route(cap_groups: int, batch_size: int, channels: int, rows_capacity: int, bf16: bool = False, gate_shared: bool = False):
+    out = (C.c_int32 * 2)()
+    check(load().egonn_debug_eca_route(int(cap_groups), int(batch_size), int(channels), int(rows_capacity), int(bool(bf16)),
+                                       int(bool(gate_shared)), out))
+    return bool(out[0]), int(out[1])
+
+
 def require_gpu() -> torch.device:
     if not torch.cuda.is_available():
         raise RuntimeError("egonn_amd: no HIP device visible (torch.cuda.is_available() is False); "
diff --git a/egonn_amd/csrc/common.h b/egonn_amd/csrc/common.h
--- a/egonn_amd/csrc/common.h
+++ b/egonn_amd/csrc/common.h
@@ -203,6 +203,7 @@
   bool no_gated_k2s2;
   bool no_fused_ghead;
   bool no_fused_gtail;
+  bool no_fused_eca;
   bool no_packed_laterals;
   bool no_split_heads;
   bool no_tail_split;
@@ -214,6 +215,7 @@
   int split_max_level_k8;
   int split_cfg;
   int rg_first_pass;
+  int gtail_cpw;
   const char* ksplit[5];
 };
 const Switches& switches();
diff --git a/egonn_amd/csrc/coords.hip b/egonn_amd/csrc/coords.hip
--- a/egonn_amd/csrc/coords.hip
+++ b/egonn_amd/csrc/coords.hip
@@ -22,12 +22,14 @@
     return Switches{.debug_sync = ds && ds[0] == '1', .no_presplit = on("EGONN_NO_PRESPLIT"), .no_fused_down = on("EGONN_NO_FUSED_DOWN"),
                     .no_fused_lateral = on("EGONN_NO_FUSED_LATERAL"), .no_gated_k2s2 = on("EGONN_NO_GATED_K2S2"),
                     .no_fused_ghead = on("EGONN_NO_FUSED_GHEAD"), .no_fused_gtail = on("EGONN_NO_FUSED_GTAIL"),
+                    .no_fused_eca = on("EGONN_NO_FUSED_ECA"),
                     .no_packed_laterals = on("EGONN_NO_PACKED_LATERALS"), .no_split_heads = on("EGONN_NO_SPLIT_HEADS"),
                     .no_tail_split = on("EGONN_NO_TAIL_SPLIT"), .no_task_order = on("EGONN_NO_TASK_ORDER"),
                     .flat_sort = on("EGONN_FLAT_SORT"), .sort_pairs = on("EGONN_SORT_PAIRS"), .no_search67 = on("EGONN_NO_SEARCH67"),
                     .no_dense_stream = on("EGONN_NO_DENSE_STREAM"),
                     .split_max_level = num("EGONN_SPLIT_MAX_LEVEL", -1), .split_max_level_k8 = num("EGONN_SPLIT_MAX_LEVEL_K8", -1),
                     .split_cfg = num("EGONN_SPLIT_CFG", 0), .rg_first_pass = num("EGONN_RG_FIRST_PASS", 0),
+                    .gtail_cpw = num("EGONN_GTAIL_CPW", 0),
                     .ksplit = {getenv("EGONN_KSPLIT"), getenv("EGONN_KSPLIT8"), getenv("EGONN_KSPLIT_KW"), getenv("EGONN_KSPLIT_KW8"),
                                getenv("EGONN_KSPLIT_PARTS")}};
   }();
diff --git a/egonn_amd/csrc/global_tail.hip b/egonn_amd/csrc/global_tail.hip
--- a/egonn_amd/csrc/global_tail.hip
+++ b/egonn_amd/csrc/global_tail.hip
@@ -8,21 +8,31 @@
 constexpr int GT_NT0 = GTAIL_MID / 16 / 4, GT_NT1 = GTAIL_OUT / 16 / 4;
 constexpr int GT_HS = GTAIL_MID + 4, GT_OS = GTAIL_OUT + 4;
 
+template <int CPW>
 __global__ __launch_bounds__(256, 2) void global_tail_kernel(const float* __restrict__ g5, int64_t ncap, const int32_t* __restrict__ boff,
                                                              const f32x4* __restrict__ wf0, const float* __restrict__ b0,
                                                              const f32x4* __restrict__ wf1, const float* __restrict__ b1, int pow_mode,
                                                              const float* __restrict__ pexp, float* __restrict__ partial) {
   __shared__ __attribute__((aligned(16))) float s_hid[16 * GT_HS];
   __shared__ __attribute__((aligned(16))) float s_out[16 * GT_OS];
-  const int b = blockIdx.y, ch = blockIdx.x;
+  const int b = blockIdx.y, ch0 = blockIdx.x * CPW;
   const int32_t s = boff[b], e = boff[b + 1];
   const int64_t len = e - s;
-  const int32_t r0 = s + (int32_t)(len * ch / SEG_CHUNKS);
-  const int32_t r1 = ncap > 0 ? s + (int32_t)(len * (ch + 1) / SEG_CHUNKS) : r0;
+  const int32_t r0 = s + (int32_t)(len * ch0 / SEG_CHUNKS);
+  const auto chunk_end = [&](int c) { return ncap > 0 ? s + (int32_t)(len * (c + 1) / SEG_CHUNKS) : r0; };
+  const int32_t r1 = chunk_end(ch0 + CPW - 1);
   const int tid = threadIdx.x, lane = tid & 63, wave = tid >> 6;
   const int l15 = lane & 15, g4 = lane >> 4;
   const float p = pow_mode == 1 ? pexp[0] : 1.f;
   float run = pow_mode == 2 ? -INFINITY : 0.f;
+  const auto flush = [&](int c) {
+    float sum = pow_mode == 2 ? -INFINITY : 0.f;
+    sum = pow_mode == 2 ? fmaxf(sum, run) : sum + run;
+    partial[((int64_t)b * SEG_CHUNKS + c) * GTAIL_OUT + tid] = sum;
+    run = pow_mode == 2 ? -INFINITY : 0.f;
+  };
+  int ch = ch0;
+  int32_t cend = chunk_end(ch0);
 #pragma unroll 1
   for (int32_t base = r0; base < r1; base += 16) {
     int zero = 0;
@@ -82,23 +92,37 @@
     __syncthreads();
     const int nrows = min(16, r1 - base);
     for (int r = 0; r < nrows; ++r) {
+      if constexpr (CPW > 1) {
+        while (base + r >= cend) {
+          flush(ch);
+          cend = chunk_end(++ch);
+        }
+      }
       float v = s_out[r * GT_OS + tid];
       if (pow_mode == 1) v = powf(fmaxf(v, 1e-6f), p);
       run = pow_mode == 2 ? fmaxf(run, v) : run + v;
     }
   }
-  float sum = pow_mode == 2 ? -INFINITY : 0.f;
-  sum = pow_mode == 2 ? fmaxf(sum, run) : sum + run;
-  partial[((int64_t)b * SEG_CHUNKS + ch) * GTAIL_OUT + tid] = sum;
+  for (; ch < ch0 + CPW; ++ch) flush(ch);
 }
 
 int global_tail_fused(const float* g5, int64_t ncap, const int32_t* boff, int B, const float* wf0, const float* b0, const float* wf1,
-                      const float* b1, int pow_mode, const float* p, float* partial, hipStream_t stream) {
+                      const float* b1, int pow_mode, const float* p, float* partial, hipStream_t stream, int cpw) {
   EGONN_REQUIRE(g5 && boff && wf0 && b0 && wf1 && b1 && partial && B >= 1 && ncap >= 0 && pow_mode >= 0 && pow_mode <= 2 &&
                     (pow_mode != 1 || p),
                 EGONN_ERR_INVALID, "global tail: bad arguments");
-  hipLaunchKernelGGL(global_tail_kernel, dim3(SEG_CHUNKS, B), dim3(256), 0, stream, g5, ncap, boff, reinterpret_cast<const f32x4*>(wf0),
-                     b0, reinterpret_cast<const f32x4*>(wf1), b1, pow_mode, p, partial);
+  if (cpw == 0) cpw = GTAIL_CPW;
+  static_assert(SEG_CHUNKS % 4 == 0);
+  const auto launch = [&](auto kernel) {
+    hipLaunchKernelGGL(kernel, dim3(SEG_CHUNKS / cpw, B), dim3(256), 0, stream, g5, ncap, boff, reinterpret_cast<const f32x4*>(wf0), b0,
+                       reinterpret_cast<const f32x4*>(wf1), b1, pow_mode, p, partial);
+  };
+  switch (cpw) {
+    case 1: launch(global_tail_kernel<1>); break;
+    case 2: launch(global_tail_kernel<2>); break;
+    case 4: launch(global_tail_kernel<4>); break;
+    default: EGONN_REQUIRE(false, EGONN_ERR_INVALID, "global tail: %d chunks per workgroup (1, 2 or 4)", cpw);
+  }
   HIP_CHECK(hipGetLastError());
   return EGONN_OK;
 }
diff --git a/egonn_amd/csrc/kernels.h b/egonn_amd/csrc/kernels.h
--- a/egonn_amd/csrc/kernels.h
+++ b/egonn_amd/csrc/kernels.h
@@ -149,8 +149,9 @@
 int dense_pack_frags(const float* W, int w_out_in, int cin, int cout, float* out, hipStream_t stream);
 
 constexpr int GTAIL_CIN = 128, GTAIL_MID = 192, GTAIL_OUT = 256;
+constexpr int GTAIL_CPW = 1;
 int global_tail_fused(const float* g5, int64_t ncap, const int32_t* boff, int B, const float* wf0, const float* b0, const float* wf1,
-                      const float* b1, int pow_mode, const float* p, float* partial, hipStream_t stream);
+                      const float* b1, int pow_mode, const float* p, float* partial, hipStream_t stream, int cpw = 0);
 
 int bn_fold(const float* w, const float* b, const float* rm, const float* rv, float eps, int c, float* scale,
             float* shift, hipStream_t stream);
@@ -165,6 +166,13 @@
                     float* gate, hipStream_t stream);
 int eca_apply_gate(const void* x, const void* res, const float* gate, const int32_t* boff, int B, int64_t n, int c,
                    void* out, int bf16, hipStream_t stream);
+struct EcaRoute {
+  bool fused;
+  int chunks;
+};
+EcaRoute eca_route(int64_t cap_groups, int B, int c, int64_t ncap, int bf16, bool gate_shared);
+int eca_gate_apply(const float* psum, const RowGroups& rg, const int32_t* boff, int B, int64_t n, int c, const float* wconv, int ksize,
+                   const void* x, const void* res, void* out, int bf16, int chunks, float* gate_out, hipStream_t stream);
 int convert_bf16_to_f32(const void* in, int64_t n, float* out, hipStream_t stream);
 int gem_finish(const float* partial, const int32_t* boff, int B, int c, const float* p, float* out,
                hipStream_t stream);
diff --git a/egonn_amd/csrc/model.h b/egonn_amd/csrc/model.h
--- a/egonn_amd/csrc/model.h
+++ b/egonn_amd/csrc/model.h
@@ -127,7 +127,7 @@
                 hipStream_t st);
 bool global_tail_fusable(const MlpRef& r);
 int global_tail(const MlpRef& r, const void* const* pk, const float* g5, int64_t ncap, const int32_t* n_dev, const int32_t* boff, int B,
-                Pooling method, const float* p, bool fused, float* gh, float* gd, float* partial, float* out, hipStream_t st);
+                Pooling method, const float* p, bool fused, float* gh, float* gd, float* partial, float* out, hipStream_t st, int cpw = 0);
 
 bool topdown_split_supported(int C, int Cl);
 int topdown_split_forward(Ctx* ctx, int level_out, const float* x_coarse, const void* sp_tconv, const float* x_lateral,
diff --git a/egonn_amd/csrc/model.hip b/egonn_amd/csrc/model.hip
--- a/egonn_amd/csrc/model.hip
+++ b/egonn_amd/csrc/model.hip
@@ -774,12 +774,12 @@
 
 bool global_tail_fusable(const MlpRef& r) { return r.cin == GTAIL_CIN && r.mid == GTAIL_MID && r.cout == GTAIL_OUT; }
 int global_tail(const MlpRef& r, const void* const* pk, const float* g5, int64_t ncap, const int32_t* n_dev, const int32_t* boff, int B,
-                Pooling method, const float* p, bool fused, float* gh, float* gd, float* partial, float* out, hipStream_t st) {
+                Pooling method, const float* p, bool fused, float* gh, float* gd, float* partial, float* out, hipStream_t st, int cpw) {
   if (fused) {
     EGONN_REQUIRE(global_tail_fusable(r) && pk && pk[0] && pk[1], EGONN_ERR_STATE, "global tail: no fused form for %d->%d->%d", r.cin,
                   r.mid, r.cout);
     EGONN_TRY(global_tail_fused(g5, ncap, boff, B, static_cast<const float*>(pk[0]), r.b0, static_cast<const float*>(pk[1]), r.b1,
-                                pool_pow_mode(method), method == POOL_GEM ? p : nullptr, partial, st));
+                                pool_pow_mode(method), method == POOL_GEM ? p : nullptr, partial, st, cpw));
     return global_pool_finish(method, partial, boff, B, r.cout, p, out, st);
   }
   EGONN_TRY(run_mlp(r, g5, ncap, ACT_NONE, gh, gd, st, n_dev));
@@ -893,11 +893,15 @@
     EGONN_TRY(block_convs(c, st, A, i, b, m->pk_c1[i], m->pk_c2[i], bf16, y, psum, &t2));
     WALLOC(float, gate, (size_t)B * b.cout);
     DBG_SYNC("L%d convs", i);
-    EGONN_TRY(eca_gate_groups(psum, L.rg27, L.boff, B, b.cout, b.eca, b.eca_k, gate, st));
+    const bool gated_k2s2 = i == 1 && !switches().no_gated_k2s2 && !c->keep_level_features && !bf16 && !b.down &&
+                            c->sconv.set.product() && b.cout == 32 && m->blk[2].cin == 32 && sconv_route(c, 1, 2, 32, 32, 0) == ROUTE_SPLIT;
+    const bool gated_down = b.down && !switches().no_fused_down && dense_gate_fusable(n, b.cin, b.cout);
+    EcaRoute er = eca_route(L.rg27.cap_groups, B, b.cout, n, bf16, gated_k2s2 || gated_down);
+    if (switches().no_fused_eca) er.fused = false;
+    if (!er.fused) EGONN_TRY(eca_gate_groups(psum, L.rg27, L.boff, B, b.cout, b.eca, b.eca_k, gate, st));
     DBG_SYNC("L%d eca gate", i);
     const void* res = y;
-    if (i == 1 && !switches().no_gated_k2s2 && !c->keep_level_features && !bf16 && !b.down && c->sconv.set.product() && b.cout == 32 &&
-        m->blk[2].cin == 32 && sconv_route(c, 1, 2, 32, 32, 0) == ROUTE_SPLIT) {
+    if (gated_k2s2) {
       gated_t2 = reinterpret_cast<const float*>(t2);
       gated_res = reinterpret_cast<const float*>(y);
       gated_gate = gate;
@@ -908,7 +912,7 @@
     }
     WALLOC(char, xo, n * b.cout * es);
     const DenseCall down = down_call(b, y, bf16, n, cnt + i, m->pk_down[i]);
-    if (b.down && !switches().no_fused_down && dense_gate_fusable(n, b.cin, b.cout)) {
+    if (gated_down) {
       DenseCall dc = down;
       dc.residual = t2; dc.res_bf16 = bf16;
       dc.gate = gate; dc.boff = L.boff; dc.B = B;
@@ -922,7 +926,10 @@
         EGONN_TRY(dense_forward(dc, st));
         res = rd;
       }
-      EGONN_TRY(eca_apply_gate(t2, res, gate, L.boff, B, n, b.cout, xo, bf16, st));
+      if (er.fused)
+        EGONN_TRY(eca_gate_apply(psum, L.rg27, L.boff, B, n, b.cout, b.eca, b.eca_k, t2, res, xo, bf16, er.chunks, nullptr, st));
+      else
+        EGONN_TRY(eca_apply_gate(t2, res, gate, L.boff, B, n, b.cout, xo, bf16, st));
     }
     DBG_SYNC("L%d eca apply", i);
     x[i] = xo;
@@ -983,7 +990,9 @@
     const Pooling pool = (flags & EGONN_FLAG_POOL_MAC) ? POOL_MAC : (flags & EGONN_FLAG_POOL_SPOC) ? POOL_SPOC : POOL_GEM;
     EGONN_REQUIRE(pool != POOL_GEM || m->gem_p, EGONN_ERR_STATE, "forward: GeM pooling needs the tensor 'global_pooling.pooling.p'");
     const bool fused_tail = !switches().no_fused_gtail && global_tail_fusable(m->gdec) && m->pk_gdec[0] && m->pk_gdec[1];
-    EGONN_TRY(global_tail(m->gdec, m->pk_gdec, g5, P.cap[5], cnt + 5, P.lv[5].boff, B, pool, m->gem_p, fused_tail, gh, gd, gp, out_global, st));
+    const int cpw = switches().gtail_cpw;
+    EGONN_TRY(global_tail(m->gdec, m->pk_gdec, g5, P.cap[5], cnt + 5, P.lv[5].boff, B, pool, m->gem_p, fused_tail, gh, gd, gp, out_global, st,
+                          cpw));
   }
 
   DBG_SYNC("global decoder + pooling");
@@ -1009,7 +1018,8 @@
                 "debug_global_tail: rows_capacity=%lld outside [0, 2^31 / %d)", (long long)rows_capacity, GTAIL_OUT);
   EGONN_REQUIRE(pooling >= POOL_GEM && pooling <= POOL_SPOC && (pooling != POOL_GEM || p), EGONN_ERR_INVALID,
                 "debug_global_tail: pooling=%d (1 GeM with its exponent, 2 MAC, 3 SPoC)", pooling);
-  EGONN_REQUIRE(form == 0 || form == 1, EGONN_ERR_INVALID, "debug_global_tail: form=%d (0 three launches, 1 the fused launch)", form);
+  EGONN_REQUIRE(form >= 0 && form <= 4, EGONN_ERR_INVALID,
+                "debug_global_tail: form=%d (0 three launches, 1 the fused launch, 2 / 3 / 4 fused with 1 / 2 / 4 chunks per workgroup)", form);
   const size_t need = debug_tail_span(rows_capacity);
   EGONN_REQUIRE(scratch_bytes >= (int64_t)need && ((uintptr_t)scratch & 255) == 0, EGONN_ERR_INVALID,
                 "debug_global_tail: scratch needs %lld bytes, 256-byte aligned", (long long)need);
@@ -1022,11 +1032,13 @@
   EGONN_REQUIRE(gh && gd && pk0 && pk1, EGONN_ERR_STATE, "debug_global_tail: scratch span too small");
   const MlpRef r{.w0 = w0, .b0 = b0, .w1 = w1, .b1 = b1, .cin = GTAIL_CIN, .mid = GTAIL_MID, .cout = GTAIL_OUT};
   const void* pk[2] = {pk0, pk1};
-  if (form == 1) {
+  if (form >= 1) {
     EGONN_TRY(dense_pack_frags(w0, 1, r.cin, r.mid, pk0, st));
     EGONN_TRY(dense_pack_frags(w1, 1, r.mid, r.cout, pk1, st));
   }
-  return global_tail(r, pk, g5, rows_capacity, n_dev, row_offsets, batch_size, (Pooling)pooling, p, form == 1, gh, gd, partial, out, st);
+  const int cpw[5] = {0, 0, 1, 2, 4};
+  return global_tail(r, pk, g5, rows_capacity, n_dev, row_offsets, batch_size, (Pooling)pooling, p, form >= 1, gh, gd, partial, out, st,
+                     cpw[form]);
 }
 
 API int egonn_forward_level_features(egonn_ctx* c, int level, float* out, int channels, void* stream) {
diff --git a/egonn_amd/csrc/rowwise.hip b/egonn_amd/csrc/rowwise.hip
--- a/egonn_amd/csrc/rowwise.hip
+++ b/egonn_amd/csrc/rowwise.hip
@@ -1,3 +1,6 @@
+#include <algorithm>
+
+#include "../../include/egonn_hip.h"
 #include "common.h"
 #include "kernels.h"
 #include "rowmath.h"
@@ -98,6 +101,40 @@
 
 
 template <bool BF16>
+__device__ __forceinline__ uint4 eca_piece(const uint4 xh, const uint4 rh, const float* gp) {
+  constexpr int CPT = BF16 ? 8 : 4;
+  const uint32_t xw[4] = {xh.x, xh.y, xh.z, xh.w}, rw[4] = {rh.x, rh.y, rh.z, rh.w};
+  float xv[CPT], rv[CPT], g[CPT];
+  if constexpr (BF16) {
+#pragma unroll
+    for (int i = 0; i < 4; ++i) {
+      xv[2 * i] = bf2f(xw[i] & 0xFFFFu); xv[2 * i + 1] = bf2f(xw[i] >> 16);
+      rv[2 * i] = bf2f(rw[i] & 0xFFFFu); rv[2 * i + 1] = bf2f(rw[i] >> 16);
+    }
+    const float4 g0 = reinterpret_cast<const float4*>(gp)[0], g1 = reinterpret_cast<const float4*>(gp)[1];
+    g[0] = g0.x; g[1] = g0.y; g[2] = g0.z; g[3] = g0.w; g[4] = g1.x; g[5] = g1.y; g[6] = g1.z; g[7] = g1.w;
+  } else {
+    const float4 g0 = reinterpret_cast<const float4*>(gp)[0];
+#pragma unroll
+    for (int i = 0; i < 4; ++i) { xv[i] = __uint_as_float(xw[i]); rv[i] = __uint_as_float(rw[i]); }
+    g[0] = g0.x; g[1] = g0.y; g[2] = g0.z; g[3] = g0.w;
+  }
+  float o[CPT];
+#pragma unroll
+  for (int i = 0; i < CPT; ++i) o[i] = fmaxf(xv[i] * g[i] + rv[i], 0.f);
+  uint4 oh;
+  if constexpr (BF16) {
+    oh.x = f2bf_rn(o[0]) | (f2bf_rn(o[1]) << 16);
+    oh.y = f2bf_rn(o[2]) | (f2bf_rn(o[3]) << 16);
+    oh.z = f2bf_rn(o[4]) | (f2bf_rn(o[5]) << 16);
+    oh.w = f2bf_rn(o[6]) | (f2bf_rn(o[7]) << 16);
+  } else {
+    oh = make_uint4(__float_as_uint(o[0]), __float_as_uint(o[1]), __float_as_uint(o[2]), __float_as_uint(o[3]));
+  }
+  return oh;
+}
+
+template <bool BF16>
 __global__ void eca_apply_kernel(const void* __restrict__ x, const void* __restrict__ res,
                                  const float* __restrict__ gate, const int32_t* __restrict__ boff, int B, int64_t n,
                                  int cq_shift, void* __restrict__ out) {
@@ -109,37 +146,7 @@
   const int q = (int)(t - ((int64_t)r << cq_shift));
   const int b = sample_of_row(boff, B, r);
   const float* gp = gate + (((int64_t)b << cq_shift) + q) * CPT;
-  float xv[CPT], rv[CPT], g[CPT];
-  if constexpr (BF16) {
-    const uint4 xh = reinterpret_cast<const uint4*>(x)[t], rh = reinterpret_cast<const uint4*>(res)[t];
-    const uint32_t xw[4] = {xh.x, xh.y, xh.z, xh.w}, rw[4] = {rh.x, rh.y, rh.z, rh.w};
-#pragma unroll
-    for (int i = 0; i < 4; ++i) {
-      xv[2 * i] = bf2f(xw[i] & 0xFFFFu); xv[2 * i + 1] = bf2f(xw[i] >> 16);
-      rv[2 * i] = bf2f(rw[i] & 0xFFFFu); rv[2 * i + 1] = bf2f(rw[i] >> 16);
-    }
-    const float4 g0 = reinterpret_cast<const float4*>(gp)[0], g1 = reinterpret_cast<const float4*>(gp)[1];
-    g[0] = g0.x; g[1] = g0.y; g[2] = g0.z; g[3] = g0.w; g[4] = g1.x; g[5] = g1.y; g[6] = g1.z; g[7] = g1.w;
-  } else {
-    const float4 xf = reinterpret_cast<const float4*>(x)[t], rf = reinterpret_cast<const float4*>(res)[t];
-    const float4 g0 = reinterpret_cast<const float4*>(gp)[0];
-    xv[0] = xf.x; xv[1] = xf.y; xv[2] = xf.z; xv[3] = xf.w;
-    rv[0] = rf.x; rv[1] = rf.y; rv[2] = rf.z; rv[3] = rf.w;
-    g[0] = g0.x; g[1] = g0.y; g[2] = g0.z; g[3] = g0.w;
-  }
-  float o[CPT];
-#pragma unroll
-  for (int i = 0; i < CPT; ++i) o[i] = fmaxf(xv[i] * g[i] + rv[i], 0.f);
-  if constexpr (BF16) {
-    uint4 oh;
-    oh.x = f2bf_rn(o[0]) | (f2bf_rn(o[1]) << 16);
-    oh.y = f2bf_rn(o[2]) | (f2bf_rn(o[3]) << 16);
-    oh.z = f2bf_rn(o[4]) | (f2bf_rn(o[5]) << 16);
-    oh.w = f2bf_rn(o[6]) | (f2bf_rn(o[7]) << 16);
-    reinterpret_cast<uint4*>(out)[t] = oh;
-  } else {
-    reinterpret_cast<float4*>(out)[t] = make_float4(o[0], o[1], o[2], o[3]);
-  }
+  reinterpret_cast<uint4*>(out)[t] = eca_piece<BF16>(reinterpret_cast<const uint4*>(x)[t], reinterpret_cast<const uint4*>(res)[t], gp);
 }
 __global__ void bf16_to_f32_kernel(const uint16_t* __restrict__ in, int64_t n, float* __restrict__ out) {
   const int64_t t = (int64_t)blockIdx.x * blockDim.x + threadIdx.x;
@@ -168,6 +175,52 @@
   return EGONN_OK;
 }
 
+__device__ __forceinline__ float eca_gate_body(const float* __restrict__ psum, const uint32_t* __restrict__ gmask, int g0, int g1,
+                                               int32_t cntr, int c, const float* __restrict__ wconv, int ksize, float* red,
+                                               float* mean) {
+  const int tid = threadIdx.x;
+  const int nsl = 1024 / c, sl = tid / c, ch = tid - sl * c;
+  float acc = 0.f;
+  {
+    constexpr int U = 8;
+    int g = g0 + sl;
+    for (; g + (U - 1) * nsl < g1; g += U * nsl) {
+      float v[U];
+      uint32_t m[U];
+#pragma unroll
+      for (int u = 0; u < U; ++u) {
+        m[u] = gmask[g + u * nsl];
+        v[u] = psum[(int64_t)(g + u * nsl) * c + ch];
+      }
+#pragma unroll
+      for (int u = 0; u < U; ++u) acc += (m[u] >> 31) ? v[u] : 0.f;
+    }
+    for (; g < g1; g += nsl) {
+      const uint32_t m = gmask[g];
+      const float v = psum[(int64_t)g * c + ch];
+      acc += (m >> 31) ? v : 0.f;
+    }
+  }
+  red[tid] = acc;
+  __syncthreads();
+  if (tid < c) {
+    float s = 0.f;
+    for (int k = 0; k < nsl; ++k) s += red[k * c + tid];
+    mean[tid] = cntr > 0 ? s / (float)cntr : 0.f;
+  }
+  __syncthreads();
+  float gv = 0.f;
+  if (tid < c) {
+    const int pad = (ksize - 1) / 2;
+    float y = 0.f;
+    for (int j = 0; j < ksize; ++j) {
+      const int q = tid + j - pad;
+      if (q >= 0 && q < c) y += wconv[j] * mean[q];
+    }
+    gv = 1.f / (1.f + expf(-y));
+  }
+  return gv;
+}
 __global__ __launch_bounds__(1024) void eca_gate_groups_kernel(const float* __restrict__ psum,
                                                                 const uint32_t* __restrict__ gmask,
                                                                 const int32_t* __restrict__ meta,
@@ -179,46 +232,45 @@
   const int b = blockIdx.x, tid = threadIdx.x;
   const int g0 = meta[1 + b], g1 = meta[2 + b];
   const int32_t cntr = boff[b + 1] - boff[b];
-  const int nsl = 1024 / c, sl = tid / c, ch = tid - sl * c;
-  float acc = 0.f;
-  {
-    constexpr int U = 8;
-    int g = g0 + sl;
-    for (; g + (U - 1) * nsl < g1; g += U * nsl) {
-      float v[U];
-      uint32_t m[U];
-#pragma unroll
-      for (int u = 0; u < U; ++u) {
-        m[u] = gmask[g + u * nsl];
-        v[u] = psum[(int64_t)(g + u * nsl) * c + ch];
-      }
-#pragma unroll
-      for (int u = 0; u < U; ++u) acc += (m[u] >> 31) ? v[u] : 0.f;
-    }
-    for (; g < g1; g += nsl) {
-      const uint32_t m = gmask[g];
-      const float v = psum[(int64_t)g * c + ch];
-      acc += (m >> 31) ? v : 0.f;
-    }
-  }
-  red[tid] = acc;
+  const float gv = eca_gate_body(psum, gmask, g0, g1, cntr, c, wconv, ksize, red, mean);
+  if (tid < c) gate[(int64_t)b * c + tid] = gv;
+}
+
+template <bool BF16>
+__global__ __launch_bounds__(1024) void eca_gate_apply_kernel(const float* __restrict__ psum, const uint32_t* __restrict__ gmask,
+                                                               const int32_t* __restrict__ meta, const int32_t* __restrict__ boff,
+                                                               int B, int64_t n, int c, int cq_shift, const float* __restrict__ wconv,
+                                                               int ksize, const void* __restrict__ x, const void* __restrict__ res,
+                                                               void* __restrict__ out, float* __restrict__ gate_out) {
+  constexpr int CPT = BF16 ? 8 : 4;
+  __shared__ float red[1024];
+  __shared__ float mean[256];
+  __shared__ __attribute__((aligned(16))) float s_gate[256];
+  const int b = blockIdx.y, ch = blockIdx.x, nch = gridDim.x, tid = threadIdx.x;
+  n = min((int64_t)boff[B], n);
+  const int32_t b0 = boff[b], b1 = boff[b + 1];
+  const int64_t s = min((int64_t)b0, n), len = min((int64_t)b1, n) - s;
+  const int64_t t0 = (s + len * ch / nch) << cq_shift, t1 = (s + len * (ch + 1) / nch) << cq_shift;
+  if (t0 >= t1) return;
+  int64_t t = t0 + tid;
+  const int64_t tc = min(t, t1 - 1);
+  uint4 xh = reinterpret_cast<const uint4*>(x)[tc], rh = reinterpret_cast<const uint4*>(res)[tc];
+  const float gv = eca_gate_body(psum, gmask, meta[1 + b], meta[2 + b], b1 - b0, c, wconv, ksize, red, mean);
+  if (tid < c) {
+    s_gate[tid] = gv;
+    if (gate_out && t0 == (s << cq_shift)) gate_out[(int64_t)b * c + tid] = gv;
+  }
   __syncthreads();
-  if (tid < c) {
-    float s = 0.f;
-    for (int k = 0; k < nsl; ++k) s += red[k * c + tid];
-    mean[tid] = cntr > 0 ? s / (float)cntr : 0.f;
-  }
-  __syncthreads();
-  if (tid < c) {
-    const int pad = (ksize - 1) / 2;
-    float y = 0.f;
-    for (int j = 0; j < ksize; ++j) {
-      const int q = tid + j - pad;
-      if (q >= 0 && q < c) y += wconv[j] * mean[q];
-    }
-    gate[(int64_t)b * c + tid] = 1.f / (1.f + expf(-y));
-  }
-}
+  const int qmask = (1 << cq_shift) - 1;
+  while (t < t1) {
+    reinterpret_cast<uint4*>(out)[t] = eca_piece<BF16>(xh, rh, s_gate + ((int)t & qmask) * CPT);
+    t += 1024;
+    const int64_t tn = min(t, t1 - 1);
+    xh = reinterpret_cast<const uint4*>(x)[tn];
+    rh = reinterpret_cast<const uint4*>(res)[tn];
+  }
+}
+
 int eca_gate_groups(const float* psum, const RowGroups& rg, const int32_t* boff, int B, int c, const float* wconv, int ksize,
                     float* gate, hipStream_t stream) {
   EGONN_REQUIRE(c >= 32 && c <= 256 && 256 % c == 0, EGONN_ERR_INVALID, "eca gate: %d channels unsupported", c);
@@ -238,6 +290,36 @@
   else
     hipLaunchKernelGGL(eca_apply_kernel<false>, dim3((unsigned)cdiv(n * cq, 256)), dim3(256), 0, stream, x, res, gate, boff, B, n,
                        __builtin_ctz(cq), out);
+  HIP_CHECK(hipGetLastError());
+  return EGONN_OK;
+}
+
+constexpr int64_t ECA_CHUNK_PIECES = 4 * 1024;
+constexpr int64_t ECA_FUSED_MAX_PSUM_BYTES = (ECA_CHUNK_PIECES * 16 * 3) / 3;
+constexpr int ECA_MIN_WORKGROUPS = 128;
+EcaRoute eca_route(int64_t cap_groups, int B, int c, int64_t ncap, int bf16, bool gate_shared) {
+  EcaRoute r{.fused = false, .chunks = 0};
+  const int cq = bf16 ? c / 8 : c / 4;
+  if (gate_shared || B < 1 || ncap <= 0 || cap_groups < 0 || cq < 1 || (cq & (cq - 1)) || c < 32 || c > 256 || 256 % c) return r;
+  if (cap_groups / B * c * 4 > ECA_FUSED_MAX_PSUM_BYTES) return r;
+  const int64_t pieces = cdiv(ncap, (int64_t)B) * cq;
+  const int64_t most = std::max<int64_t>(pieces / 1024, 1), want = cdiv(ECA_MIN_WORKGROUPS, B);
+  r.chunks = (int)std::min<int64_t>(std::max(cdiv(pieces, ECA_CHUNK_PIECES), std::min(most, want)), 65535);
+  r.fused = true;
+  return r;
+}
+int eca_gate_apply(const float* psum, const RowGroups& rg, const int32_t* boff, int B, int64_t n, int c, const float* wconv, int ksize,
+                   const void* x, const void* res, void* out, int bf16, int chunks, float* gate_out, hipStream_t stream) {
+  EGONN_REQUIRE(c >= 32 && c <= 256 && 256 % c == 0, EGONN_ERR_INVALID, "eca gate: %d channels unsupported", c);
+  EGONN_REQUIRE(chunks >= 1 && chunks <= 65535 && B >= 1 && B <= 65535, EGONN_ERR_INVALID, "eca gate + apply: grid (%d, %d)", chunks, B);
+  if (n == 0) return EGONN_OK;
+  const int cq = bf16 ? c / 8 : c / 4;
+  if (bf16)
+    hipLaunchKernelGGL(eca_gate_apply_kernel<true>, dim3(chunks, B), dim3(1024), 0, stream, psum, rg.gmask, rg.meta, boff, B, n, c,
+                       __builtin_ctz(cq), wconv, ksize, x, res, out, gate_out);
+  else
+    hipLaunchKernelGGL(eca_gate_apply_kernel<false>, dim3(chunks, B), dim3(1024), 0, stream, psum, rg.gmask, rg.meta, boff, B, n, c,
+                       __builtin_ctz(cq), wconv, ksize, x, res, out, gate_out);
   HIP_CHECK(hipGetLastError());
   return EGONN_OK;
 }
@@ -308,3 +390,44 @@
 }
 
 }
+
+using namespace egonn;
+
+API int egonn_debug_eca_route(int64_t cap_groups, int batch_size, int channels, int64_t rows_capacity, int bf16, int gate_shared,
+                              int32_t out[2]) {
+  EGONN_REQUIRE(out && cap_groups >= 0 && batch_size >= 1 && batch_size <= EGONN_MAX_BATCH && rows_capacity >= 0 && channels >= 32 &&
+                    channels <= 256 && 256 % channels == 0,
+                EGONN_ERR_INVALID, "debug_eca_route: bad arguments");
+  const EcaRoute r = eca_route(cap_groups, batch_size, channels, rows_capacity, bf16 ? 1 : 0, gate_shared != 0);
+  out[0] = r.fused ? 1 : 0;
+  out[1] = r.chunks;
+  return EGONN_OK;
+}
+API int egonn_debug_eca_tail(const float* psum, const uint32_t* gmask, const int32_t* meta, const int32_t* row_offsets, int batch_size,
+                             int64_t cap_groups, int64_t rows_capacity, int channels, const float* wconv, int ksize, const void* x,
+                             const void* res, int bf16, int form, int chunks, float* gate, void* out, void* stream) {
+  EGONN_REQUIRE(psum && gmask && meta && row_offsets && wconv && x && res && gate && out, EGONN_ERR_INVALID, "debug_eca_tail: null pointer");
+  EGONN_REQUIRE(batch_size >= 1 && batch_size <= EGONN_MAX_BATCH, EGONN_ERR_INVALID, "debug_eca_tail: batch_size=%d outside [1, %d]",
+                batch_size, EGONN_MAX_BATCH);
+  EGONN_REQUIRE(channels >= 32 && channels <= 256 && 256 % channels == 0 && ksize >= 1 && ksize <= 15 && (ksize & 1), EGONN_ERR_INVALID,
+                "debug_eca_tail: channels=%d ksize=%d (32..256 dividing 256, odd 1..15)", channels, ksize);
+  EGONN_REQUIRE(rows_capacity >= 0 && rows_capacity < (1ll << 31) / channels && cap_groups >= 0 && cap_groups < (1ll << 31) / channels,
+                EGONN_ERR_INVALID, "debug_eca_tail: rows_capacity=%lld cap_groups=%lld outside [0, 2^31 / %d)", (long long)rows_capacity,
+                (long long)cap_groups, channels);
+  EGONN_REQUIRE((form == 0 || form == 1) && chunks >= 0 && chunks <= 65535, EGONN_ERR_INVALID,
+                "debug_eca_tail: form=%d chunks=%d (0 two launches, 1 one launch; 0..65535 chunks, 0 = the route's)", form, chunks);
+  hipStream_t st = (hipStream_t)stream;
+  RowGroups rg;
+  rg.cap_groups = (int)cap_groups;
+  rg.gmask = const_cast<uint32_t*>(gmask);
+  rg.meta = const_cast<int32_t*>(meta);
+  if (form == 0) {
+    EGONN_TRY(eca_gate_groups(psum, rg, row_offsets, batch_size, channels, wconv, ksize, gate, st));
+    return eca_apply_gate(x, res, gate, row_offsets, batch_size, rows_capacity, channels, out, bf16 ? 1 : 0, st);
+  }
+  if (chunks == 0) {
+    const EcaRoute r = eca_route(cap_groups, batch_size, channels, rows_capacity, bf16 ? 1 : 0, false);
+    chunks = r.fused ? r.chunks : 1;
+  }
+  return eca_gate_apply(psum, rg, row_offsets, batch_size, rows_capacity, channels, wconv, ksize, x, res, out, bf16 ? 1 : 0, chunks, gate, st);
+}
diff --git a/include/egonn_hip.h b/include/egonn_hip.h
--- a/include/egonn_hip.h
+++ b/include/egonn_hip.h
@@ -40,6 +40,11 @@
 int egonn_debug_global_tail(const float* g5, const int32_t* row_offsets, int batch_size, int64_t rows_capacity, const int32_t* n_dev,
                             const float* w0, const float* b0, const float* w1, const float* b1, const float* p, int pooling, int form,
                             float* partial, float* out, void* scratch, int64_t scratch_bytes, void* stream);
+int egonn_debug_eca_tail(const float* psum, const uint32_t* gmask, const int32_t* meta, const int32_t* row_offsets, int batch_size,
+                         int64_t cap_groups, int64_t rows_capacity, int channels, const float* wconv, int ksize, const void* x,
+                         const void* res, int bf16, int form, int chunks, float* gate, void* out, void* stream);
+int egonn_debug_eca_route(int64_t cap_groups, int batch_size, int channels, int64_t rows_capacity, int bf16, int gate_shared,
+                          int32_t out[2]);
 
 int egonn_voxelize(egonn_ctx* ctx, const float* points, const int64_t* scan_offsets, int batch_size, int quant_mode,
                    const float* step, void* stream);
```

Result: no change. 23450, median of 4 (+0.1%).
